# Britefury/cutmix-semisup-seg

Hardware: AMD Instinct MI355X
Metric: train images/sec (student+teacher step) (higher is better)
Workload: dtype bf16; 1 GPU; deeplab2-resnet101 cutmix mean-teacher step, 10x3x321x321, 21 classes (BASELINE configs[1]); per_gpu_batch=10, global_batch=10, classes=21, parallelism=dp1, fuse_batches=True, stream_overlap=True, deterministic_wgrad=False

## Files before the change

### cutmix-semisup-seg_amd/_lib.py

```python
import ctypes as C
import os

import torch

_HERE = os.path.dirname(os.path.abspath(__file__))
LIB_PATH = os.path.join(_HERE, 'csrc', 'libcutmixseg_hip.so')

if not os.path.exists(LIB_PATH):
    raise ImportError('libcutmixseg_hip.so not found at {} -- build it with '
                      '`python cutmix-semisup-seg_amd/build.py` (hipcc, gfx950); there is no CPU fallback'.format(LIB_PATH))

lib = C.CDLL(LIB_PATH)

F32, BF16 = 0, 1
(BN_REDUCE, BN_FINALIZE, BN_APPLY, BN_REDUCE_BWD, BN_BWD_APPLY, BN_COUNT, BN_STATS, BN_FINALIZE_TILES,
 BN_BWD_SUMS_TILES) = range(9)
LABEL_U8, LABEL_I64 = 0, 1
LOSS_IDS = {'var': 0, 'logits_var': 1, 'logits_smoothl1': 2, 'bce': 3, 'kld': 4}
MODE_MIX, MODE_CUT = 0, 1
OPT_CHUNK = 2048
AUG_PARAMS = 24

c_void_p, c_int, c_float, c_size_t = C.c_void_p, C.c_int, C.c_float, C.c_size_t

# ... 52 lines not shown
                ('stats_out', c_void_p), ('stats_rows_per_group', c_int), ('mask_gates_res', c_int),
                ('bstats_u', c_void_p), ('bstats_bits', c_void_p), ('bstats_mean', c_void_p), ('bstats_rstd', c_void_p)]


class WgradDesc(C.Structure):
    _fields_ = [('du', c_void_p), ('x', c_void_p), ('dw', c_void_p), ('scale', c_void_p),
                ('n', c_int), ('h', c_int), ('w_in', c_int), ('cin', c_int), ('ho', c_int), ('wo', c_int),
                ('cout', c_int), ('cout_real', c_int), ('ntaps', c_int), ('tap_dy', c_int * 18), ('tap_dx', c_int * 18),
                ('stride', c_int), ('ksplit', c_int), ('w', c_void_p), ('wdot', c_void_p), ('dbeta', c_void_p),
                ('dw_cout', c_int), ('workspace', c_void_p), ('workspace_bytes', C.c_longlong), ('wg_target', c_int)]


class BnOp(C.Structure):
    _fields_ = [('what', c_int), ('dtype', c_int), ('c', c_int), ('relu', c_int),
                ('x', c_void_p), ('res', c_void_p), ('y', c_void_p), ('dy', c_void_p), ('dx', c_void_p), ('dres', c_void_p),
                ('sums', c_void_p), ('gamma', c_void_p), ('beta', c_void_p), ('mean', c_void_p), ('rstd', c_void_p),
                ('scale', c_void_p), ('shift', c_void_p), ('running_mean', c_void_p), ('running_var', c_void_p),
                ('counter', c_void_p), ('clear_a', c_void_p), ('clear_b', c_void_p), ('ws', c_void_p), ('count', C.c_double), ('n_pixels', C.c_ulonglong), ('eps', c_float),
                ('momentum', c_float), ('groups', c_int), ('tile_rows', c_int), ('mask_bits', c_void_p)]


class AugmentDesc(C.Structure):
    _fields_ = [('src', c_void_p), ('src_labels', c_void_p), ('out0', c_void_p), ('out1', c_void_p),
                ('out_labels', c_void_p), ('out_mask', c_void_p), ('params', c_void_p),
                ('mean', c_float * 3), ('std_', c_float * 3),
                ('n', c_int), ('hs', c_int), ('ws', c_int), ('h', c_int), ('w', c_int), ('out_dtype', c_int)]


class StageEntry(C.Structure):
    _fields_ = [('img_off', C.c_longlong), ('lab_off', C.c_longlong), ('hs', c_int), ('ws', c_int)]


class StageDesc(C.Structure):
    _fields_ = [('pool_img', c_void_p), ('pool_labels', c_void_p), ('entries', c_void_p), ('index', c_void_p),
                ('out0', c_void_p), ('out1', c_void_p), ('out_labels', c_void_p), ('out_mask', c_void_p), ('params', c_void_p),
                ('mean', c_float * 3), ('std_', c_float * 3),
                ('n', c_int), ('n_entries', c_int), ('h', c_int), ('w', c_int), ('out_dtype', c_int)]


class PdPatch(C.Structure):
    _fields_ = [('img_off', C.c_longlong), ('hs', c_int), ('ws', c_int), ('cy', c_int), ('cx', c_int)]


TTA_MAX_VIEWS = 16


class TtaDesc(C.Structure):
    _fields_ = [('logits', c_void_p * TTA_MAX_VIEWS), ('h', c_int * TTA_MAX_VIEWS), ('w', c_int * TTA_MAX_VIEWS),
                ('flip', c_int * TTA_MAX_VIEWS),
                ('n', c_int), ('c', c_int), ('H', c_int), ('W', c_int), ('k', c_int), ('align_corners', c_int),
                ('labels', c_void_p), ('label_dtype', c_int), ('ignore_index', c_int), ('cm', c_void_p), ('pred_out', c_void_p)]


class ClassMixDesc(C.Structure):
    _fields_ = [('logits', c_void_p), ('valid', c_void_p), ('keys', c_void_p),
                ('n', c_int), ('c', c_int), ('h', c_int), ('w', c_int), ('H', c_int), ('W', c_int), ('align_corners', c_int),
                ('mask_out', c_void_p), ('pred_out', c_void_p), ('present_out', c_void_p), ('chosen_out', c_void_p),
                ('workspace', c_void_p), ('workspace_bytes', c_size_t)]


class CpsDesc(C.Structure):
    _fields_ = [('l0_a', c_void_p), ('l1_a', c_void_p), ('l0_b', c_void_p), ('l1_b', c_void_p),
                ('ranges', c_void_p), ('mask', c_void_p), ('um0', c_void_p), ('um1', c_void_p),
                ('n', c_int), ('c', c_int), ('h', c_int), ('w', c_int), ('H', c_int), ('W', c_int), ('align_corners', c_int),
                ('n_boxes', c_int), ('invert', c_int), ('conf_thresh', c_float),
                ('label_a', c_void_p), ('label_b', c_void_p), ('stats', c_void_p)]


class BoundaryDesc(C.Structure):
    _fields_ = [('truth', c_void_p), ('pred', c_void_p), ('widths', c_void_p),
                ('n', c_int), ('h', c_int), ('w', c_int), ('num_classes', c_int), ('ignore_index', c_int), ('k', c_int),
                ('bcm', c_void_p), ('tcm', c_void_p), ('dist_truth', c_void_p), ('dist_pred', c_void_p),
                ('workspace', c_void_p), ('workspace_bytes', c_size_t)]


class PackItem(C.Structure):
    _fields_ = [('src', c_void_p), ('dst', c_void_p), ('scale', c_void_p),
                ('ntaps', c_int), ('cout', c_int), ('cin', c_int), ('first_block', c_int)]


class WfinishItem(C.Structure):
    _fields_ = [('scratch', c_void_p), ('grad', c_void_p), ('w', c_void_p), ('scale', c_void_p), ('wdot', c_void_p),
                ('ntaps', c_int), ('cout', c_int), ('cin', c_int), ('first_block', c_int)]


_P = C.POINTER


def _proto(name, restype, argtypes):
    fn = getattr(lib, name)
    fn.restype = restype
    fn.argtypes = argtypes
    return fn


PROTOTYPES = {
    'cms_version': (c_int, []),
    'cms_last_error': (C.c_char_p, []),
    'cms_device_info': (c_int, [_P(c_int), C.c_char_p, c_size_t]),
    'cms_boxmask_rasterize': (c_int, [c_void_p, c_int, c_int, c_int, c_int, c_int, c_void_p, c_void_p]),
    'cms_cutmix_paste': (c_int, [c_void_p, c_void_p, c_void_p, c_int, c_void_p, c_int, c_int, c_int, c_int, c_int,
                                 c_int, c_void_p]),
    'cms_cutmix_paste_mask': (c_int, [c_void_p, c_void_p, c_void_p, c_int, c_void_p, c_int, c_int, c_int, c_int,
                                      c_void_p]),
    'cms_consistency_workspace_bytes': (c_size_t, [_P(ConsistencyDesc)]),
    'cms_consistency_fwd': (c_int, [_P(ConsistencyDesc), c_void_p, c_void_p, c_void_p]),
    'cms_consistency_finalize': (c_int, [c_void_p, c_void_p, c_float, c_int, c_float, c_float, c_void_p, c_void_p]),
    'cms_consistency_bwd': (c_int, [_P(ConsistencyDesc), c_void_p, c_void_p, c_void_p]),
    'cms_consistency_fused_supported': (c_int, [_P(ConsistencyDesc)]),
    'cms_consistency_fwd_bwd': (c_int, [_P(ConsistencyDesc), c_float, c_void_p, c_void_p, c_void_p, c_void_p]),
    'cms_scale_by_scalar': (c_int, [c_void_p, C.c_longlong, c_void_p, c_int, c_float, c_void_p]),
    'cms_ict_blend': (c_int, [c_void_p, c_void_p, c_void_p, c_int, c_void_p, c_int, C.c_longlong, c_void_p]),
    'cms_ict_workspace_bytes': (c_size_t, [_P(IctDesc)]),
    'cms_ict_fwd': (c_int, [_P(IctDesc), c_void_p, c_void_p, c_void_p]),
    'cms_ict_bwd': (c_int, [_P(IctDesc), c_void_p, c_void_p, c_void_p, c_void_p]),
    'cms_aug_workspace_bytes': (c_size_t, [_P(AugDesc)]),
    'cms_aug_fwd': (c_int, [_P(AugDesc), c_void_p, c_void_p, c_void_p]),
    'cms_aug_bwd': (c_int, [_P(AugDesc), c_void_p, c_void_p, c_void_p]),
    'cms_ce_workspace_bytes': (c_size_t, [_P(CeDesc)]),
    'cms_ce_fwd': (c_int, [_P(CeDesc), c_void_p, c_void_p, c_void_p]),
    'cms_ce_finalize': (c_int, [c_void_p, c_float, c_void_p, c_void_p]),
    'cms_ce_bwd': (c_int, [_P(CeDesc), c_void_p, c_void_p, c_void_p]),
    'cms_ce_fused_supported': (c_int, [_P(CeDesc)]),
    'cms_ce_fwd_bwd': (c_int, [_P(CeDesc), c_void_p, c_void_p, c_void_p, c_void_p]),
    'cms_upsample_bilinear_fwd': (c_int, [c_void_p, c_void_p, c_int, c_int, c_int, c_int, c_int, c_int, c_int,
                                          c_void_p]),
    'cms_upsample_bilinear_bwd': (c_int, [c_void_p, c_void_p, c_int, c_int, c_int, c_int, c_int, c_int, c_int,
                                          c_void_p]),
    'cms_ema_flat': (c_int, [c_void_p, c_void_p, c_size_t, c_float, c_float, c_void_p, c_void_p]),
    'cms_adam_ema_step': (c_int, [_P(OptimDesc), c_void_p]),
    'cms_sgd_ema_step': (c_int, [_P(OptimDesc), c_void_p]),
    'cms_increment_counter': (c_int, [c_void_p, c_void_p]),
    'cms_bn_fold': (c_int, [c_void_p, c_void_p, c_void_p, c_void_p, c_void_p, c_int, c_float, c_void_p, c_void_p, c_void_p]),
    'cms_argmax_confusion': (c_int, [c_void_p, c_void_p, c_int, c_int, c_int, c_int, c_int, c_int, c_int, c_int,
                                     c_int, c_void_p, c_void_p, c_void_p]),
    'cms_confusion': (c_int, [c_void_p, c_void_p, c_size_t, c_int, c_int, c_void_p, c_void_p]),
    'cms_fill_holes_workspace_bytes': (c_size_t, [c_int, c_int, c_int]),
    'cms_fill_holes': (c_int, [c_void_p, c_void_p, c_void_p, c_int, c_void_p, c_int, c_int, c_int, c_void_p, c_size_t,
                               c_void_p]),
    'cms_conv_igemm': (c_int, [_P(ConvDesc), c_void_p]),
    'cms_conv_igemm_route': (c_int, [_P(ConvDesc)]),
    'cms_conv_igemm_stats_tile_rows': (c_int, [_P(ConvDesc)]),
    'cms_frozen_bn_act_bwd': (c_int, [c_void_p, c_void_p, c_void_p, c_void_p, c_int, c_void_p, c_size_t, c_int, c_void_p]),
    'cms_conv_set_trace': (c_int, [c_void_p, c_int]),
    'cms_conv_set_wgrad8': (c_int, [c_int]),
    'cms_loss_set_deterministic': (c_int, [c_int]),
    'cms_conv_wgrad_uses_wgrad8': (c_int, [_P(WgradDesc)]),
    'cms_conv_wgrad': (c_int, [_P(WgradDesc), c_void_p]),
    'cms_conv_wgrad_workspace_bytes': (C.c_longlong, [_P(WgradDesc)]),
    'cms_conv_wgrad_group_kind': (c_int, [_P(WgradDesc)]),
    'cms_conv_wgrad_group_bytes': (C.c_longlong, [c_int]),
    'cms_conv_wgrad_group_pack': (c_int, [_P(WgradDesc), c_int, c_int, c_void_p, C.c_longlong, _P(c_int)]),
    'cms_conv_wgrad_group_run': (c_int, [c_void_p, c_int, c_int, c_int, c_void_p]),
    'cms_conv_pack_transpose': (c_int, [c_void_p, c_int, c_void_p, c_void_p, c_int, c_int, c_int, c_int, c_void_p]),
    'cms_conv_pack_transpose_batch': (c_int, [c_void_p, c_int, c_int, c_int, c_void_p]),
    'cms_conv_pack_transpose_batch64': (c_int, [c_void_p, c_int, c_int, c_void_p]),
    'cms_augment_batch': (c_int, [_P(AugmentDesc), c_void_p]),
    'cms_augment_luma': (c_int, [_P(AugmentDesc), c_void_p, c_void_p]),
    'cms_stage_batch': (c_int, [_P(StageDesc), c_void_p]),
    'cms_stage_luma': (c_int, [_P(StageDesc), c_void_p, c_void_p]),
    'cms_bn_workspace_bytes': (c_size_t, [c_size_t, c_int, c_int]),
    'cms_bn_run': (c_int, [_P(BnOp), c_void_p]),
    'cms_channel_copy': (c_int, [c_void_p, c_size_t, c_void_p, c_size_t, c_size_t, c_int, c_int, c_size_t, c_void_p]),
    'cms_add_n': (c_int, [c_void_p, c_int, c_void_p, c_size_t, c_int, c_void_p]),
    'cms_channel_sum': (c_int, [c_void_p, c_int, c_size_t, c_int, c_void_p, c_void_p]),
    'cms_wgrad_finish_pack': (c_int, [_P(WfinishItem), c_int]),
    'cms_wgrad_finish_run': (c_int, [c_void_p, c_int, c_int, c_void_p]),
    'cms_program_add_channel_sum': (c_int, [c_void_p, c_void_p, c_int, c_size_t, c_int, c_void_p, c_int, c_int]),
    'cms_program_add_wgrad_finish': (c_int, [c_void_p, c_void_p, c_int, c_int, c_int, c_int]),
    'cms_rows_reduce': (c_int, [c_void_p, c_size_t, c_int, c_size_t, c_int, c_int, c_void_p, c_float, c_void_p]),
    'cms_upsample_nhwc': (c_int, [c_void_p, c_void_p, c_size_t, c_int, c_int, c_int, c_int, c_int, c_int, c_int, c_int, c_int,
                                  c_void_p]),
    'cms_aspp_gather_fwd': (c_int, [c_void_p, c_void_p, c_void_p, _P(c_int), _P(c_int), c_int, c_int, c_int, c_int, c_int,
                                    c_int, c_void_p]),
    'cms_aspp_spread_bwd': (c_int, [c_void_p, c_void_p, c_int, _P(c_int), _P(c_int), c_int, c_int, c_int, c_int, c_int,
                                    c_int, c_void_p]),
    'cms_stem_pack_weights': (c_int, [c_void_p, c_int, c_void_p, c_void_p]),
    'cms_stem_out_hw': (c_int, [c_int, c_int, _P(c_int), _P(c_int), _P(c_int), _P(c_int)]),
    'cms_stem_fwd': (c_int, [c_void_p, c_int, c_void_p, c_int, c_void_p, c_void_p, c_void_p, c_int, c_int, c_int,
                             c_void_p]),
    'cms_maxpool3x3s2_fwd': (c_int, [c_void_p, c_void_p, c_void_p, c_int, c_int, c_int, c_int, c_int, c_int, c_void_p]),
    'cms_maxpool3x3s2_relu_bwd': (c_int, [c_void_p, c_void_p, c_void_p, c_void_p, c_int, c_int, c_int, c_int, c_int,
                                          c_int, c_void_p]),
    'cms_stem_wgrad': (c_int, [c_void_p, c_int, c_void_p, c_int, c_void_p, c_void_p, c_int, c_int, c_int, c_void_p]),
    'cms_stem_wgrad_workspace_bytes': (C.c_longlong, [c_int, c_int, c_int, c_int, c_int]),
    'cms_stem_wgrad_ws': (c_int, [c_void_p, c_int, c_void_p, c_int, c_void_p, c_void_p, c_int, c_int, c_int, c_void_p,
                          C.c_longlong, c_void_p]),
    'cms_stem_dgrad': (c_int, [c_void_p, c_int, c_void_p, c_void_p, c_void_p, c_int, c_int, c_int, c_void_p]),
    'cms_program_create': (c_int, [_P(c_void_p)]),
    'cms_program_destroy': (c_int, [c_void_p]),
    'cms_program_add_conv': (c_int, [c_void_p, _P(ConvDesc), c_int, c_int, c_int]),
    'cms_program_add_wgrad': (c_int, [c_void_p, _P(WgradDesc), c_int, c_int, c_int]),
    'cms_program_add_wgrad_group': (c_int, [c_void_p, c_void_p, c_int, c_int, c_int, c_int, c_int]),
    'cms_program_add_memset': (c_int, [c_void_p, c_void_p, c_size_t, c_int, c_int]),
# ... 66 lines not shown
```

### cutmix-semisup-seg_amd/backbone_hip.py

```python
import os
import torch

from . import ops
from .arena import ensure_arena


def executors_of(module):
    exs = getattr(module, '_hip_executors', None)
    if exs:
        return list(exs.values())
    ex = getattr(module, '_hip_executor', None)
    return [] if ex is None else [ex]


class _Conv(object):
    __slots__ = ('wkey', 'bn', 'taps', 'ntaps', 'neg_taps', 'stride', 'cin', 'cout', 'scale', 'bias', 'wT', 'ksize',
                 'pad', 'dil', 'wdot', 'dbeta', 'wT_raw')

    def __init__(self, wkey, bn, conv):
        self.wkey, self.bn = wkey, bn
        kh, kw = conv.kernel_size
        self.ksize, self.pad, self.dil = kh, conv.padding[0], conv.dilation[0]
        self.taps = ops.conv_taps(kh, kw, conv.dilation[0], conv.padding[0])
        self.neg_taps = [(-dy, -dx) for dy, dx in self.taps]
        self.stride = conv.stride[0]
        self.cin, self.cout = conv.in_channels, conv.out_channels
        self.scale = self.bias = self.wT = None
        self.wT_raw = None
        self.wdot = self.dbeta = None


class _Block(object):
    __slots__ = ('c1', 'c2', 'c3', 'cd')


class DeepLabHipExecutor(object):
    def __init__(self, net, dtype=torch.bfloat16):
        self._init_common(net, dtype)
        self.num_classes = net.num_classes
        self._add_blocks('', [getattr(net, 'layer{}'.format(li)) for li in range(1, 5)])
        self.stem_wkey, self.stem_bn, self.stem_ceil = 'conv1.weight', 'bn1', True
        self.stem_w147 = None
        self._stem_version = -1
        head = net.layer5.conv2d_list
        self.aspp_keys = ['layer5.conv2d_list.0', 'layer5.conv2d_list.1']
        self.aspp_taps = []
        for i in range(2):
            self.aspp_taps += ops.conv_taps(3, 3, head[i].dilation[0], head[i].padding[0])
        self.aspp_neg_taps = [(-dy, -dx) for dy, dx in self.aspp_taps]
        dev = self.arena.device
        C = self.num_classes
        if C > 32:
            raise NotImplementedError('ASPP head kernel is specialised for <= 32 classes')
        self.aspp_zc = (18 * C + 127) // 128 * 128
        self.aspp_wall = torch.zeros(1, self.aspp_zc, 2048, dtype=self.dtype, device=dev)
        self.aspp_wallT = torch.zeros(1, 2048, self.aspp_zc, dtype=self.dtype, device=dev)
        self._aspp_version = -1
        self.aspp_bias = torch.zeros(C, dtype=torch.float32, device=dev)

    def _init_common(self, net, dtype=torch.bfloat16):
        if dtype not in (torch.bfloat16, torch.float32):
            raise TypeError('executor dtype must be torch.bfloat16 or torch.float32')
        self.net = net
        self.dtype = dtype
        self.trainable = any(p.requires_grad for p in net.parameters())
        self.bn_trainable = any(p.requires_grad for m in net.modules() if 'BatchNorm' in type(m).__name__
                                for p in m.parameters())
        self.arena = ensure_arena(net, with_grad=self.trainable, with_bf16=(dtype == torch.bfloat16))
        self.blocks = []
        self._layer_first = []
        self._affine_ready = False
        self._bn_idx = None
        self._side = None
        self._pack_plan = None
        self._pack_plan_bn = None
        self._wT_raw_version = -1
        self._bn_modules = {}
        self._stem_param = None
        self._sentinel = None
        self._seen_shapes = {}
        self._wscratch_buf = None
        self._wfinish_pending = []
        self._wfinish_ok = {}
        self._pending_keep = None
        self.grad_hook = None
        self.data_grad_only = False
        self.overlap_wgrad = True
        self.wgrad_streams = 2 if os.environ.get('CMS_WGRAD8', '1') != '0' else 1
        self.defer_wgrad_join = False
        self._pending_join = None
        self._sides = []
        self.conv_tile = 0
        self.tile_rules = {}
        self._wT_version = -1
        self.version = 0
        self.use_programs = True
        self._programs = {}
        self._generation = 0
        self.issued = dict(flops=0.0, conv_launches=0, conv_bytes=0.0, head_launches=0, head_bytes=0.0, head_bytes_alg=0.0, floor_s=0.0)
        net.register_load_state_dict_post_hook(lambda module, incompatible: self.invalidate())

    def _add_blocks(self, prefix, layers):
        for li, layer in enumerate(layers):
            self._layer_first.append(len(self.blocks))
            for bi, blk in enumerate(layer):
                pre = '{}layer{}.{}'.format(prefix, li + 1, bi)
                b = _Block()
                b.c1 = _Conv(pre + '.conv1.weight', pre + '.bn1', blk.conv1)
                b.c2 = _Conv(pre + '.conv2.weight', pre + '.bn2', blk.conv2)
                b.c3 = _Conv(pre + '.conv3.weight', pre + '.bn3', blk.conv3)
                b.cd = None
                if blk.downsample is not None:
                    b.cd = _Conv(pre + '.downsample.0.weight', pre + '.downsample.1', blk.downsample[0])
                self.blocks.append(b)

    def invalidate(self):
        self.arena.refresh_bf16()
        self._affine_ready = False
        self.version += 1

    def weights_changed(self, bn_too=False):
        self.version += 1
        if bn_too or self.bn_trainable:
            self._affine_ready = False

    def block_grad_offsets(self):
        return [self.arena.by_key[b.c1.wkey].offset for b in self.blocks]

    def layer_first_blocks(self):
        return list(self._layer_first)

    def _all_convs(self):
        for b in self.blocks:
            for c in (b.c1, b.c2, b.c3, b.cd):
                if c is not None:
                    yield c

    def _build_affine_tables(self):
        a = self.arena
        idx = {k: [] for k in ('weight', 'bias', 'running_mean', 'running_var')}
        off = 0
        spans = []
        for c in self._all_convs():
            for k in idx:
                s = a.by_key[c.bn + '.' + k]
                idx[k].append(torch.arange(s.offset, s.offset + s.count, dtype=torch.int64))
            spans.append((c, off, off + c.cout))
            off += c.cout
        stem_span = None
        if getattr(self, 'stem_bn', None) is not None:
            for k in idx:
                s = a.by_key[self.stem_bn + '.' + k]
                idx[k].append(torch.arange(s.offset, s.offset + s.count, dtype=torch.int64))
            stem_span = (off, off + a.by_key[self.stem_bn + '.weight'].count)
            off = stem_span[1]
        dev = a.device
        self._bn_idx = {k: torch.cat(v).to(dev) for k, v in idx.items()}
        self._scale_all = torch.zeros(off, dtype=torch.float32, device=dev)
        self._bias_all = torch.zeros(off, dtype=torch.float32, device=dev)
        for c, lo, hi in spans:
            c.scale, c.bias = self._scale_all[lo:hi], self._bias_all[lo:hi]
        if stem_span is not None:
            self.stem_scale, self.stem_bias = self._scale_all[stem_span[0]:stem_span[1]], self._bias_all[stem_span[0]:stem_span[1]]
        if self.bn_trainable and self.trainable:
            self._wdot_all = torch.zeros(off, dtype=torch.float32, device=dev)
            self._dbeta_all = torch.zeros(off, dtype=torch.float32, device=dev)
            for c, lo, hi in spans:
                c.wdot, c.dbeta = self._wdot_all[lo:hi], self._dbeta_all[lo:hi]

    def _refresh_affine(self):
        if self._bn_idx is None:
            self._build_affine_tables()
# ... 134 lines not shown
                          sums=fsums[g * 2 * C:(g + 1) * 2 * C], gamma=a.view(c.bn + '.weight'), beta=a.view(c.bn + '.bias'),
                          mean=mean[sl], rstd=rstd[sl], scale=scale[sl], shift=shift[sl],
                          running_mean=a.view(c.bn + '.running_mean'), running_var=a.view(c.bn + '.running_var'),
                          counter=bn.num_batches_tracked)
        else:
            ops.bn_op('stats', c=C, dtype=self.dtype, n_pixels=npix, groups=G, eps=bn.eps, momentum=bn.momentum, x=u, ws=ws,
                      gamma=a.view(c.bn + '.weight'), beta=a.view(c.bn + '.bias'), mean=mean, rstd=rstd, scale=scale, shift=shift,
                      running_mean=a.view(c.bn + '.running_mean'), running_var=a.view(c.bn + '.running_var'),
                      counter=bn.num_batches_tracked)
        y = torch.empty_like(u)
        bits = torch.empty(npix * C // 8, dtype=torch.uint8, device=dev) if (relu and save) else None
        ops.bn_op('apply', c=C, dtype=self.dtype, n_pixels=npix, groups=G, relu=relu, x=u, res=res, y=y, scale=scale,
                  shift=shift, mask_bits=bits)
        return y, (u, bits, mean, rstd, bsums, ws, G)

    def _bstats(self, s3):
        if self.dtype != torch.bfloat16:
            return None
        u, bits, mean, rstd, _sums, _ws, G = s3
        return {'groups': G, 'u': u, 'mean': mean, 'rstd': rstd, 'bits': bits}

    def _bwd_unit_bn(self, dy, saved, c, want_res, dy_bits=None, tile_stats=None):
        u, bits, mean, rstd, sums, ws, G = saved
        C = c.cout
        npix = u.numel() // C
        if dy_bits is not None:
            assert bits is None
            bits = dy_bits
        if tile_stats is not None and tile_stats.get('tile_rows', 0) > 0:
            assert dy_bits is None
            ops.bn_op('sums_tiles', c=C, dtype=self.dtype, n_pixels=npix, groups=G, tile_rows=tile_stats['tile_rows'],
                      ws=tile_stats['tile_sums'], sums=sums)
        else:
            ops.bn_op('reduce_bwd', c=C, dtype=self.dtype, n_pixels=npix, groups=G, x=u, dy=dy, mean=mean, rstd=rstd, sums=sums,
                      ws=ws, mask_bits=bits)
        grp = self._dist_group()
        world = ops._world(grp)
        if world > 1:
            ops.host_call(lambda t=sums, g_=grp: ops._allreduce_sum(t, g_))
        du = torch.empty_like(u)
        dres = torch.empty_like(u) if want_res else None
        ops.bn_op('bwd_apply', c=C, dtype=self.dtype, n_pixels=npix, groups=G, count=(npix // G) * world, x=u, dy=dy, dx=du, dres=dres,
                  mask_bits=bits, mean=mean, rstd=rstd, gamma=self.arena.view(c.bn + '.weight'), sums=sums)
        return du, dres

    def _fwd_block_bn(self, st, bi):
        b, cur = self.blocks[bi], st['cur']
        save, G = st['saved'] is not None, st.get('groups', 1)
        a1, s1 = self._fwd_unit_bn(cur, b.c1, True, save=save, groups=G)
        a2, s2 = self._fwd_unit_bn(a1, b.c2, True, save=save, groups=G)
        sd = None
        if b.cd is None:
            res = cur
        else:
            res, sd = self._fwd_unit_bn(cur, b.cd, False, save=save, groups=G)
        out, s3 = self._fwd_unit_bn(a2, b.c3, True, res=res, save=save, groups=G)
        st['cur'] = out
        if st['saved'] is not None:
            st['saved'].append((cur, a1, a2, s1, s2, s3, sd))

    def _refresh_backward_weights_bn(self):
        if self._pack_plan_bn is None:
            triples = []
            for c in self._all_convs():
                w = self._w(c)
                c.wT_raw = torch.empty((w.shape[0], w.shape[2], w.shape[1]), dtype=self.dtype, device=w.device)
                triples.append((w, c.wT_raw, None))
            triples.append((self.aspp_wall, self.aspp_wallT, None))
            self._pack_plan_bn = ops.PackTransposePlan(triples)
        self._pack_plan_bn.run()

    def _dgrad_raw(self, du, c, res=None, in_hw=None, res_bits=None, bstats=None):
        n, ho, wo, _ = du.shape
        if c.stride == 1:
            return ops.conv_igemm(du, c.wT_raw, c.neg_taps, res=res, mode=1, tile=self._tile(c.cin), mask_bits=res_bits,
                                  mask_gates_res=res_bits is not None, stats=bstats)
        assert res_bits is None and bstats is None
        return ops.conv_igemm(du, c.wT_raw, c.neg_taps, res=res, mode=1, out_hw=(ho, wo), out_stride=c.stride,
                              out_full_hw=in_hw, tile=self._tile(c.cin))

    def _wgrad_raw(self, du, x, c):
        ops.conv_wgrad(du, x, c.taps, self.arena.packed(c.wkey, self.arena.grad), stride=c.stride, wg_target=self._wg_target())

    def _backward_chain_bn(self, saved, dlg, want_w, sides, hook, box=None):
        x4 = saved[-1]
        main = torch.cuda.current_stream()
        d = ops.aspp_spread_bwd(dlg, self.aspp_taps, self.aspp_zc, self.dtype)
        dwall = None
        if want_w:
            dwall = torch.empty((1, self.aspp_zc, 2048), dtype=torch.float32, device=d.device)
            ops.memset_zero(dwall)
            ops.conv_wgrad(d, x4, [(0, 0)], dwall)
            if box is not None:
                box['dwall'] = dwall
        pend = self._bstats(saved[len(self.blocks) - 1][5])
        dOut = ops.conv_igemm(d, self.aspp_wallT, [(0, 0)], mode=1, stats=pend)
        keep = []
        closes = set(self.bucket_starts())
        for bi in range(len(self.blocks) - 1, -1, -1):
            b = self.blocks[bi]
            xin, a1, a2, s1, s2, s3, sd = saved[bi]
            in_hw = (xin.shape[1], xin.shape[2])
            bits3 = s3[1] if (b.cd is not None or (b.c1.stride == 1 and self.dtype == torch.bfloat16)) else None
            du3, dres = self._bwd_unit_bn(dOut, s3, b.c3, bits3 is None, tile_stats=pend)
            da2 = self._dgrad_raw(du3, b.c3)
            du2, _ = self._bwd_unit_bn(da2, s2, b.c2, False)
            da1 = self._dgrad_raw(du2, b.c2)
            du1, _ = self._bwd_unit_bn(da1, s1, b.c1, False)
            dud = None
            if b.cd is not None:
                dud, _ = self._bwd_unit_bn(dres if bits3 is None else dOut, sd, b.cd, False, dy_bits=bits3)
            if want_w:
                self._issue_wgrads(self._block_jobs(b, du3, du2, dud, du1, xin, a1, a2), sides, main, keep, bi in closes,
                                   wgrad=self._wgrad_raw)
                with torch.cuda.stream(sides[0] if sides else main):
                    hook(bi)
            pend = self._bstats(saved[bi - 1][5]) if (bi > 0 and b.c1.stride == 1) else None
            if b.cd is None and bits3 is not None:
                dOut = self._dgrad_raw(du1, b.c1, res=dOut, in_hw=in_hw, res_bits=bits3, bstats=pend)
            else:
                dx = dres if b.cd is None else self._dgrad_raw(dud, b.cd, in_hw=in_hw)
                dOut = self._dgrad_raw(du1, b.c1, res=dx, in_hw=in_hw, bstats=pend)
        if not self.defer_wgrad_join:
            for sd_ in sides:
                ops.stream_wait(main, sd_)
        self._retire_keep(keep)
        return dOut, dwall

    def _stem_prepare(self):
        if not self._affine_ready:
            self._refresh_affine()
        if self._stem_version != self.version:
            self.stem_w147 = ops.stem_pack_weights(self.arena.packed(self.stem_wkey, self._wbuf()), out=self.stem_w147)
            self._stem_version = self.version

    def stem(self, x):
        if self._stem_param is None:
            self._stem_param = dict(self.net.named_parameters())[self.stem_wkey]
        save = (torch.is_grad_enabled() and (self.trainable or x.requires_grad)) if self.use_programs else None
        return _StemFn.apply(x.contiguous(), self._stem_param, self, save)

    def _stem_destination(self, shape, save):
        key = ('fwd', tuple(int(v) for v in shape), bool(save), self._tile_key(), self._bn_key())
        prog = self._programs.get(key)
        return None if prog is None else prog.x_in

    def _prepare_forward(self):
        if not self._affine_ready and not self.batch_statistics():
            self._refresh_affine()
        self._refresh_aspp_fwd()

    def _bn_key(self):
        return self.bn_groups() if self.batch_statistics() else 0

    def _tile_key(self):
        return (self.conv_tile, tuple(sorted(self.tile_rules.items())))

    MAX_PROGRAMS = 8

    def _program_lookup(self, key):
        prog = self._programs.get(key)
        if prog is not None:
            self._programs[key] = self._programs.pop(key)
            return prog
        if len(self._programs) >= self.MAX_PROGRAMS:
            torch.cuda.synchronize()
            self._programs.pop(next(iter(self._programs)))
        return None

    def _eager_this_time(self, kind, shape, save):
# ... 70 lines not shown
                self.fwd_block(st, bi)
            return self.fwd_end(st)
        prog = self.forward_program(x.shape, save)
        self._prepare_forward()
        if x.data_ptr() != prog.x_in.data_ptr():
            prog.x_in.copy_(x)
        prog.run([torch.cuda.current_stream()])
        self._stamp(prog)
        return prog.logits.clone(), ((prog, prog.generation) if save else None)

    def _wgrad(self, du, x, c):
        if c.wdot is not None and self.dtype == torch.float32:
            g = torch.zeros_like(self._w(c))
            ops.conv_wgrad(du, x, c.taps, g, stride=c.stride)
            self.arena.packed(c.wkey, self.arena.grad).add_(g * c.scale.view(1, -1, 1))
            c.wdot.add_((g * self._w(c)).sum(dim=(0, 2)))
            c.dbeta.add_(du.sum(dim=(0, 1, 2)))
        elif c.wdot is not None and self._wfinish_takes(du, x, c):
            ops.conv_wgrad(du, x, c.taps, self.arena.packed(c.wkey, self._wscratch()), stride=c.stride, scale=None,
                           wg_target=self._wg_target())
            ops.channel_sum(du, c.dbeta)
            if all(c is not p for p in self._wfinish_pending):
                self._wfinish_pending.append(c)
        elif c.wdot is not None:
            ops.conv_wgrad(du, x, c.taps, self.arena.packed(c.wkey, self.arena.grad), stride=c.stride, scale=c.scale,
                           w_bf16=self._w(c), wdot=c.wdot, dbeta=c.dbeta)
        else:
            ops.conv_wgrad(du, x, c.taps, self.arena.packed(c.wkey, self.arena.grad), stride=c.stride, scale=c.scale,
                           wg_target=self._wg_target())

    def _wscratch(self):
        if self._wscratch_buf is None:
            self._wscratch_buf = torch.zeros_like(self.arena.grad)
        return self._wscratch_buf

    def _wfinish_takes(self, du, x, c):
        if self.dtype != torch.bfloat16 or ops.deterministic_wgrad():
            return False
        key = (c.wkey, tuple(du.shape), tuple(x.shape))
        hit = self._wfinish_ok.get(key)
        if hit is None:
            hit = self._wfinish_ok[key] = bool(ops.conv_wgrad(du, x, c.taps, self.arena.packed(c.wkey, self._wscratch()),
                                                              stride=c.stride, scale=None, wg_target=self._wg_target(),
                                                              query_kernel=True))
        return hit

    def _wfinish_flush(self):
        pend = self._wfinish_pending
        if not pend:
            return
        a = self.arena
        ops.wgrad_finish([(a.packed(c.wkey, self._wscratch()), a.packed(c.wkey, a.grad), self._w(c), c.scale, c.wdot) for c in pend])
        del pend[:]

    def _wg_target(self):
        if not self.overlap_wgrad:
            return 0
        return 56 if self.wgrad_streams >= 2 else 112

    def _dgrad(self, du, c, res=None, mask=None, in_hw=None):
        n, ho, wo, _ = du.shape
        mb = getattr(mask, '_cms_relu_bits', None) if mask is not None else None
        if mb is not None:
            mask = None
        if c.stride == 1:
            return ops.conv_igemm(du, c.wT, c.neg_taps, res=res, mode=1, mask_src=mask, tile=self._tile(c.cin), mask_bits=mb)
        return ops.conv_igemm(du, c.wT, c.neg_taps, res=res, mode=1, mask_src=mask, out_hw=(ho, wo),
                              out_stride=c.stride, out_full_hw=in_hw, tile=self._tile(c.cin), mask_bits=mb)

    def _grad_sentinel(self):
        if self._sentinel is None:
            self._sentinel = dict(self.net.named_parameters())[self.blocks[-1].c3.wkey]
        return self._sentinel

    def _want_w(self):
        data_only = self.data_grad_only or getattr(self.net, '_data_grad_only', False)
        return self.trainable and not data_only and self.arena.grad is not None

    def _refresh_for_backward(self):
        if self._wT_version != self.version or self.blocks[0].c1.wT is None:
            self._refresh_backward_weights()
            self._wT_version = self.version

    def _head_bias_grads(self, dlogits, want_w, side=None):
        if want_w:
            if side is not None:
                side.wait_stream(torch.cuda.current_stream())
                dlogits.record_stream(side)
            with torch.cuda.stream(side if side is not None else torch.cuda.current_stream()):
                db = dlogits.sum(dim=(0, 2, 3))
                for k in self.aspp_keys:
                    self.arena.view(k + '.bias', self.arena.grad).add_(db)

    def _head_weight_grads(self, dwall, side=None):
        C = self.num_classes
        a = self.arena
        with torch.cuda.stream(side if side is not None else torch.cuda.current_stream()):
            for i, k in enumerate(self.aspp_keys):
                a.packed(k + '.weight', a.grad).add_(dwall[0, 9 * C * i:9 * C * (i + 1)].view(9, C, 2048))

    def _finish_head(self, dwall, side):
        self._head_weight_grads(dwall, side)
        if side is not None and not self.defer_wgrad_join:
            torch.cuda.current_stream().wait_stream(side)

    def bucket_starts(self):
        l2, l3, l4 = self._layer_first[1], self._layer_first[2], self._layer_first[3]
        return sorted(set([0, l2, l3, (l3 + l4 + 1) // 2, l4]))

    def _backward_chain(self, saved, dlg, want_w, sides, hook, box=None):
        x4 = saved[-1]
        main = torch.cuda.current_stream()
        d = ops.aspp_spread_bwd(dlg, self.aspp_taps, self.aspp_zc, self.dtype)
        dwall = None
        keep = []
        if want_w:
            dwall = torch.empty((1, self.aspp_zc, 2048), dtype=torch.float32, device=d.device)
            hs = sides[0] if sides else None
            if hs is not None:
                ops.stream_wait(hs, main)
                keep.append((d, dwall))
            with torch.cuda.stream(hs if hs is not None else main):
                ops.memset_zero(dwall)
                ops.conv_wgrad(d, x4, [(0, 0)], dwall)
            if box is not None:
                box['dwall'] = dwall
        x4b = getattr(x4, '_cms_relu_bits', None)
        dC = ops.conv_igemm(d, self.aspp_wallT, [(0, 0)], mode=1, mask_src=None if x4b is not None else x4, mask_bits=x4b)
        capture = getattr(self, 'debug_capture', None)
        closes = set(self.bucket_starts())
        for bi in range(len(self.blocks) - 1, -1, -1):
            if capture is not None:
                capture[bi] = dC
            b = self.blocks[bi]
            xin, a1, a2 = saved[bi]
            in_hw = (xin.shape[1], xin.shape[2])
            dU2 = self._dgrad(dC, b.c3, mask=a2)
            dU1 = self._dgrad(dU2, b.c2, mask=a1)
            if want_w:
                self._issue_wgrads(self._block_jobs(b, dC, dU2, dC, dU1, xin, a1, a2), sides, main, keep, bi in closes)
                with torch.cuda.stream(sides[0] if sides else main):
                    hook(bi)
            dres = dC if b.cd is None else self._dgrad(dC, b.cd, in_hw=in_hw)
            dC = self._dgrad(dU1, b.c1, res=dres, mask=None if bi == 0 else xin, in_hw=in_hw)
        if not self.defer_wgrad_join:
            for sd in sides:
                ops.stream_wait(main, sd)
        self._retire_keep(keep)
        return dC, dwall

    def backward(self, token, dlogits):
        bn = (token[0].bn if self.use_programs and isinstance(token, tuple) and isinstance(token[0], ops.Program)
              else len(token[0]) == 7)
        chain = self._backward_chain_bn if bn else self._backward_chain
        if bn:
            if self._wT_raw_version != self.version or self.blocks[0].c1.wT_raw is None:
                self._refresh_aspp_fwd()
                self._refresh_backward_weights_bn()
                self._wT_raw_version = self.version
        else:
            self._refresh_for_backward()
        want_w = self._want_w()
        if want_w and self._grad_sentinel().grad is None:
            self.arena.ensure_grads_attached()
        n, _, h, w = dlogits.shape
        main = torch.cuda.current_stream()
        sides = self._side_streams(self.wgrad_streams) if (self.overlap_wgrad and want_w) else []
        hside = sides[0] if (sides and not bn) else None
        if not self.use_programs:
            if self.defer_wgrad_join and sides:
                self._pending_join = list(sides)
            self._head_bias_grads(dlogits, want_w, hside)
            box = {}

            def hook(bi):
                if 'done' not in box and box.get('dwall') is not None:
                    self._head_weight_grads(box['dwall'])
                    box['done'] = True
                if self.grad_hook is not None:
                    self.grad_hook(bi)
            dx, dwall = chain(token, dlogits, want_w, sides, hook, box)
            if dwall is not None and 'done' not in box:
                self._finish_head(dwall, hside)
            return dx
        fprog, gen = token
        if fprog.generation != gen:
            raise RuntimeError('the activations of this forward pass were overwritten by a later forward pass of the '
                               'same shape through the same executor (programs keep ONE set of buffers per shape): '
                               'run backward before the next forward, or set executor.use_programs = False')
        key = (want_w, len(sides), bool(self.defer_wgrad_join))
        if self.defer_wgrad_join and sides:
            self._pending_join = list(sides)
        prog = fprog.bwd.get(key)
        if prog is None:
            prog = ops.Program()
            dlg = torch.empty(tuple(dlogits.shape), dtype=torch.float32, device=dlogits.device)
            streams = [main] + sides
            with ops.recording(prog, streams):
                dx, dwall = chain(fprog.saved, dlg, want_w, sides, prog.mark)
            prog.dlg, prog.dx, prog.dwall = dlg, dx, dwall
            fprog.bwd[key] = prog
        prog.dlg.copy_(dlogits)
        self._head_bias_grads(dlogits, want_w, hside)
        streams = [main] + sides
        if self.grad_hook is None or not want_w:
            prog.run(streams)
            if prog.dwall is not None:
                self._finish_head(prog.dwall, hside)
        else:
            first = 0
            hook_stream = sides[0] if sides else main
            head_done = False
            wanted = getattr(self.grad_hook, 'blocks', None)
            for idx, bi in prog.marks:
                if wanted is not None and bi not in wanted:
                    continue
                prog.run(streams, first, idx)
                first = idx
                with torch.cuda.stream(hook_stream):
                    if not head_done and prog.dwall is not None:
                        self._head_weight_grads(prog.dwall)
                        head_done = True
                    self.grad_hook(bi)
            prog.run(streams, first, -1)
            if prog.dwall is not None and not head_done:
                self._finish_head(prog.dwall, hside)
        self._account(prog)
        return prog.dx.clone()

    def _retire_keep(self, keep):
        if keep and self.defer_wgrad_join and ops._REC is None:
            self._pending_keep = (self._pending_keep or []) + [keep]

    def join_wgrad(self):
        sides, self._pending_join = self._pending_join, None
        if sides:
            main = torch.cuda.current_stream()
            for sd in sides:
                main.wait_stream(sd)
        self._pending_keep = None

    @staticmethod
    def _block_jobs(b, d3, d2, dd, d1, xin, a1, a2):
        return [(d3, a2, b.c3), (d2, a1, b.c2)] + ([(dd, xin, b.cd)] if b.cd is not None else []) + [(d1, xin, b.c1)]

    def _issue_wgrads(self, jobs, sides, main, keep, closes, first=0, wgrad=None):
        wgrad = wgrad or self._wgrad
        for sd in sides:
            ops.stream_wait(sd, main)
        if sides:
            keep.append(jobs)
        for ji, (du_, x_, c_) in enumerate(jobs, first):
            with torch.cuda.stream(sides[ji % len(sides)] if sides else main):
                wgrad(du_, x_, c_)
        if closes:
            for sd in sides[1:]:
                ops.stream_wait(sides[0], sd)
        return first + len(jobs)

    def _side_streams(self, k):
        k = max(1, min(int(k), 3))
        while len(self._sides) < k:
            self._sides.append(ops.pooled_stream(self.arena.device, 'wgrad{}'.format(len(self._sides))))
        return self._sides[:k]

    def _side_stream(self):
        if self._side is None:
            self._side = ops.pooled_stream(self.arena.device, 'side')
        return self._side


class DeepLabV3PlusBackboneExecutor(DeepLabHipExecutor):

    def __init__(self, wrapper, dtype=torch.bfloat16):
        self._init_common(wrapper, dtype)
        self.use_programs = not (dtype == torch.float32 and self.bn_trainable and self.trainable)
        self.stem_wkey, self.stem_bn, self.stem_ceil = 'deeplab.backbone.conv1.weight', 'deeplab.backbone.bn1', False
        self.stem_w147 = None
        self._stem_version = -1
        bb = wrapper.deeplab.backbone
        self._add_blocks('deeplab.backbone.', [bb['layer{}'.format(li)] for li in range(1, 5)])
        self.tap_low = self._layer_first[1] - 1
        self._phase_w = {}

    def _prepare_forward(self):
        if not self._affine_ready:
            self._refresh_affine()

    def _taps_pass(self, x, save):
        st = self.fwd_begin(x, save)
        low = None
        for bi in range(len(self.blocks)):
            if ops._REC is not None:
                ops._REC[0].group = bi
            self.fwd_block(st, bi)
            if bi == self.tap_low:
                low = st['cur']
        if save:
            st['saved'].append(st['cur'])
        return low, st['cur'], st['saved']

    def taps_program(self, shape, save):
        key = ('taps', tuple(int(v) for v in shape), bool(save), self._tile_key())
        prog = self._program_lookup(key)
        if prog is None:
            self._prepare_forward()
            prog = ops.Program()
            x_in = torch.empty(tuple(shape), dtype=self.dtype, device=self.arena.device)
            with ops.recording(prog, [torch.cuda.current_stream()]):
                low, out, saved = self._taps_pass(x_in, save)
            prog.x_in, prog.low, prog.out, prog.saved = x_in, low, out, saved
            prog.bwd = {}
            prog.generation = -1
            self._programs[key] = prog
        return prog

    def forward_taps(self, x, save=False):
        if not self.use_programs or self._eager_this_time('taps', x.shape, save):
            low, out, saved = self._taps_pass(x, save)
            return (low, out, saved) if save else (low, out)
        prog = self.taps_program(x.shape, save)
        self._prepare_forward()
        prog.x_in.copy_(x)
        prog.run([torch.cuda.current_stream()])
        self._stamp(prog)
        if save:
            return prog.low.detach(), prog.out.detach(), (prog, prog.generation)
        return prog.low.detach(), prog.out.detach()

    def _refresh_backward_weights(self):
        super()._refresh_backward_weights()
        for (cid, py, px), (c, idx, buf) in self._phase_w.items():
            torch.index_select(c.wT, 0, idx, out=buf)

    def _dgrad_strided(self, du, c, mask, in_hw):
        if not (c.stride == 2 and c.ksize == 3 and c.pad == 1 and c.dil == 1):
            raise NotImplementedError('phase decomposition is written for the 3x3 / stride 2 / pad 1 convolution')
        n = du.shape[0]
        H, W = int(in_hw[0]), int(in_hw[1])
        dx = torch.empty((n, H, W, c.cin), dtype=du.dtype, device=du.device)
        sel = {0: [1], 1: [0, 2]}
        for py in (0, 1):
            for px in (0, 1):
                ha, wb = (H - py + 1) // 2, (W - px + 1) // 2
                if ha <= 0 or wb <= 0:
                    continue
                ks = [(ky, kx) for ky in sel[py] for kx in sel[px]]
                ent = self._phase_w.get((id(c), py, px))
                if ent is None:
                    idx = _index_tensor(tuple(ky * 3 + kx for ky, kx in ks), du.device)
                    ent = (c, idx, c.wT[idx].contiguous())
                    self._phase_w[(id(c), py, px)] = ent
                taps = [((py + 1 - ky) // 2, (px + 1 - kx) // 2) for ky, kx in ks]
                ops.conv_igemm(du, ent[2], taps, mode=1, mask_src=mask, out=dx, out_hw=(ha, wb), out_stride=2,
                               out_full_hw=(H, W), out_pixel_offset=py * W + px)
# ... 350 lines not shown
        return p

    @staticmethod
    def backward(ctx, dp):
        x, s, idx = ctx.saved_tensors
        ex = ctx.executor
        ds = ops.maxpool3x3s2_relu_backward(dp.to(s.dtype), idx, s, ceil_mode=ex.stem_ceil)
        if ctx.w_grad and ex._want_w():
            if ex.bn_trainable:
                a = ex.arena
                g = torch.zeros((49, 64, 3), dtype=torch.float32, device=ds.device)
                ops.stem_wgrad(x, ds, g, None)
                a.packed(ex.stem_wkey, a.grad).add_(g * ex.stem_scale.view(1, -1, 1))
                wdot = (g * a.packed(ex.stem_wkey, ex._wbuf()).float()).sum(dim=(0, 2))
                dbeta = ds.float().sum(dim=(0, 1, 2))
                mean, var = a.view(ex.stem_bn + '.running_mean'), a.view(ex.stem_bn + '.running_var')
                a.view(ex.stem_bn + '.weight', a.grad).add_((wdot - mean * dbeta) * torch.rsqrt(var + 1e-5))
                a.view(ex.stem_bn + '.bias', a.grad).add_(dbeta)
            else:
                ops.stem_wgrad(x, ds, ex.arena.packed(ex.stem_wkey, ex.arena.grad), ex.stem_scale)
        dx = None
        if ctx.needs_input_grad[0]:
            dx = ops.stem_dgrad(ds, ex.stem_w147, ex.stem_scale, ctx.x_shape).to(ctx.x_dtype)
        return dx, None, None, None


class _BodyFn(torch.autograd.Function):

    @staticmethod
    def forward(ctx, x_nhwc, executor, need_grad):
        logits, token = executor.forward(x_nhwc, save=need_grad)
        ctx.executor = executor
        ctx.saved_acts = token
        return logits

    @staticmethod
    def backward(ctx, dlogits):
        dx = ctx.executor.backward(ctx.saved_acts, dlogits.contiguous().float())
        ctx.saved_acts = None
        return dx, None, None


class _BodyPairFn(torch.autograd.Function):

    @staticmethod
    def forward(ctx, x_stu, x_tea, ex_stu, ex_tea, side, need_grad):
        if ex_stu.use_programs and ex_tea.use_programs:
            main = torch.cuda.current_stream()
            ps = ex_stu.forward_program(x_stu.shape, need_grad)
            ex_stu._prepare_forward()
            if x_stu.data_ptr() != ps.x_in.data_ptr():
                ps.x_in.copy_(x_stu)
            with torch.cuda.stream(side):
                pt = ex_tea.forward_program(x_tea.shape, False)
                ex_tea._prepare_forward()
                if x_tea.data_ptr() != pt.x_in.data_ptr():
                    pt.x_in.copy_(x_tea)
            if ps.host_ops or pt.host_ops:
                with torch.cuda.stream(side):
                    pt.run([side])
                ps.run([main])
            else:
                ops.run_pair(ps, [main], pt, [side])
            ex_stu._stamp(ps)
            ex_tea._stamp(pt)
            logits_s = ps.logits.clone()
            with torch.cuda.stream(side):
                logits_t = pt.logits.clone()
            saved = (ps, ps.generation) if need_grad else None
        else:
            st_s = ex_stu.fwd_begin(x_stu, need_grad)
            with torch.cuda.stream(side):
                st_t = ex_tea.fwd_begin(x_tea, False)
            for bi in range(len(ex_stu.blocks)):
                ex_stu.fwd_block(st_s, bi)
                with torch.cuda.stream(side):
                    ex_tea.fwd_block(st_t, bi)
            logits_s, saved = ex_stu.fwd_end(st_s)
            with torch.cuda.stream(side):
                logits_t, _ = ex_tea.fwd_end(st_t)
        ctx.executor = ex_stu
        ctx.saved_acts = saved
        ctx.mark_non_differentiable(logits_t)
        return logits_s, logits_t

    @staticmethod
    def backward(ctx, dlogits, _unused):
        dx = ctx.executor.backward(ctx.saved_acts, dlogits.contiguous().float())
        ctx.saved_acts = None
        return dx, None, None, None, None, None


def run_body_pair(ex_stu, x_stu, ex_tea, x_tea, side):
    if len(ex_stu.blocks) != len(ex_tea.blocks):
        raise ValueError('student and teacher bodies differ')
    need_grad = torch.is_grad_enabled() and ex_stu.trainable
    if need_grad and not x_stu.requires_grad:
        x_stu = x_stu.detach().requires_grad_(True)
    return _BodyPairFn.apply(x_stu, x_tea, ex_stu, ex_tea, side, need_grad)


def run_body(executor, x_nhwc):
    need_grad = torch.is_grad_enabled() and (executor.trainable or x_nhwc.requires_grad)
    if need_grad and not x_nhwc.requires_grad:
        x_nhwc = x_nhwc.detach().requires_grad_(True)
    return _BodyFn.apply(x_nhwc, executor, need_grad)
```

### cutmix-semisup-seg_amd/csrc/aspp.hip

```cpp
#include "common.hpp"

namespace cms {

struct AsppTaps {
    int n_taps;
    short dy[CMS_CONV_MAX_TAPS], dx[CMS_CONV_MAX_TAPS];
};

__device__ __forceinline__ void taps_to_lds(const AsppTaps& tp, short* sdy, short* sdx) {
#pragma unroll
    for (int i = 0; i < CMS_CONV_MAX_TAPS; ++i)
        if ((int)threadIdx.x == i) {
            sdy[i] = tp.dy[i];
            sdx[i] = tp.dx[i];
        }
    __syncthreads();
}

__global__ __launch_bounds__(256) void aspp_gather_fwd_kernel(const float* __restrict__ z, const float* __restrict__ bias,
                                                              float* __restrict__ logits, AsppTaps tp, int N, int C, int ZC,
                                                              int H, int W) {
    __shared__ short sdy[CMS_CONV_MAX_TAPS], sdx[CMS_CONV_MAX_TAPS];
    taps_to_lds(tp, sdy, sdx);
    const int n_taps = tp.n_taps;
    const size_t total = (size_t)N * C * H * W;
    for (size_t i = (size_t)blockIdx.x * blockDim.x + threadIdx.x; i < total; i += (size_t)gridDim.x * blockDim.x) {
        const unsigned ii = (unsigned)i;
        const int x = (int)(ii % (unsigned)W);
        unsigned t = ii / (unsigned)W;
        const int y = (int)(t % (unsigned)H); t /= (unsigned)H;
        const int c = (int)(t % (unsigned)C);
        const int n = (int)(t / (unsigned)C);
        float acc = bias ? bias[c] : 0.0f;
        const float* zn = z + ((size_t)n * ZC + c) * H * W;
        const size_t tap_stride = (size_t)C * H * W;
        for (int k = 0; k < n_taps; ++k) {
            const int yy = y + sdy[k], xx = x + sdx[k];
            if ((unsigned)yy < (unsigned)H && (unsigned)xx < (unsigned)W) acc += zn[(size_t)k * tap_stride + (size_t)yy * W + xx];
        }
        logits[i] = acc;
    }
}

template <class T>
__global__ __launch_bounds__(256) void aspp_spread_bwd_kernel(const float* __restrict__ dl, T* __restrict__ d, AsppTaps tp,
                                                              int N, int C, int ZC, int H, int W) {
    __shared__ short sdy[CMS_CONV_MAX_TAPS], sdx[CMS_CONV_MAX_TAPS];
    taps_to_lds(tp, sdy, sdx);
    const int n_taps = tp.n_taps;
    const unsigned zc8 = (unsigned)ZC / 8u;
    const size_t total = (size_t)N * H * W * zc8;
    const size_t plane = (size_t)H * W;
    for (size_t i = (size_t)blockIdx.x * blockDim.x + threadIdx.x; i < total; i += (size_t)gridDim.x * blockDim.x) {
        const unsigned ii = (unsigned)i;
        const unsigned ch = ii % zc8;
        unsigned t = ii / zc8;
        const int x = (int)(t % (unsigned)W); t /= (unsigned)W;
        const int y = (int)(t % (unsigned)H);
        const int n = (int)(t / (unsigned)H);
        const float* dn = dl + (size_t)n * C * plane;
        float v[8];
        int k = (int)((ch * 8u) / (unsigned)C), c = (int)(ch * 8u) - k * C;
#pragma unroll
        for (int e = 0; e < 8; ++e) {
            float val = 0.0f;
            if (k < n_taps) {
                const int yy = y - sdy[k], xx = x - sdx[k];
                if ((unsigned)yy < (unsigned)H && (unsigned)xx < (unsigned)W) val = dn[(size_t)c * plane + (size_t)yy * W + xx];
            }
            v[e] = val;
            if (++c == C) { c = 0; ++k; }
        }
        if constexpr (sizeof(T) == 4) {
            float4* o = reinterpret_cast<float4*>(d + i * 8);
            o[0] = float4{v[0], v[1], v[2], v[3]};
            o[1] = float4{v[4], v[5], v[6], v[7]};
        } else {
            uint4 o;
            o.x = (uint32_t)f32_to_bf16(v[0]) | ((uint32_t)f32_to_bf16(v[1]) << 16);
            o.y = (uint32_t)f32_to_bf16(v[2]) | ((uint32_t)f32_to_bf16(v[3]) << 16);
            o.z = (uint32_t)f32_to_bf16(v[4]) | ((uint32_t)f32_to_bf16(v[5]) << 16);
            o.w = (uint32_t)f32_to_bf16(v[6]) | ((uint32_t)f32_to_bf16(v[7]) << 16);
            *reinterpret_cast<uint4*>(d + i * 8) = o;
        }
    }
}

}

using namespace cms;

static int fill_taps(AsppTaps& tp, const int* dy, const int* dx, int n_taps) {
    CMS_REQUIRE(dy && dx && n_taps > 0 && n_taps <= CMS_CONV_MAX_TAPS, "aspp: 1..%d taps", CMS_CONV_MAX_TAPS);
    tp.n_taps = n_taps;
    for (int i = 0; i < CMS_CONV_MAX_TAPS; ++i) {
        tp.dy[i] = (short)(i < n_taps ? dy[i] : 0);
        tp.dx[i] = (short)(i < n_taps ? dx[i] : 0);
    }
    return CMS_OK;
}

extern "C" int cms_aspp_gather_fwd(const float* z, const float* bias, float* logits, const int* tap_dy, const int* tap_dx,
                                   int n_taps, int n, int c, int zc, int h, int w, void* stream) {
    CMS_REQUIRE(z && logits, "aspp_gather_fwd: NULL pointer");
    CMS_REQUIRE(n > 0 && c > 0 && h > 0 && w > 0 && zc >= n_taps * c, "aspp_gather_fwd: bad geometry (zc >= taps * classes)");
    AsppTaps tp;
    const int rc = fill_taps(tp, tap_dy, tap_dx, n_taps);
    if (rc) return rc;
    const size_t total = (size_t)n * c * h * w;
    CMS_REQUIRE(total < (1ull << 32), "aspp_gather_fwd: more than 2^32 logits");
    hipLaunchKernelGGL(aspp_gather_fwd_kernel, dim3(grid_for(total, 256, 256 * 16)), dim3(256), 0, (hipStream_t)stream, z, bias,
                       logits, tp, n, c, zc, h, w);
    return launch_status("cms_aspp_gather_fwd");
}

extern "C" int cms_aspp_spread_bwd(const float* dlogits, void* d_nhwc, int d_dtype, const int* tap_dy, const int* tap_dx,
                                   int n_taps, int n, int c, int zc, int h, int w, void* stream) {
    CMS_REQUIRE(dlogits && d_nhwc, "aspp_spread_bwd: NULL pointer");
    CMS_REQUIRE(d_dtype == CMS_F32 || d_dtype == CMS_BF16, "aspp_spread_bwd: bad dtype");
    CMS_REQUIRE(n > 0 && c > 0 && h > 0 && w > 0 && zc >= n_taps * c, "aspp_spread_bwd: bad geometry (zc >= taps * classes)");
    AsppTaps tp;
    const int rc = fill_taps(tp, tap_dy, tap_dx, n_taps);
    if (rc) return rc;
    CMS_REQUIRE(zc % 8 == 0, "aspp_spread_bwd: the stacked tap x class axis (%d) must be a multiple of 8", zc);
    const size_t total = (size_t)n * h * w * (zc / 8);
    CMS_REQUIRE(total < (1ull << 32), "aspp_spread_bwd: more than 2^32 chunks");
    hipStream_t s = (hipStream_t)stream;
    if (d_dtype == CMS_F32)
        hipLaunchKernelGGL(aspp_spread_bwd_kernel<float>, dim3(grid_for(total, 256, 256 * 16)), dim3(256), 0, s, dlogits,
                           (float*)d_nhwc, tp, n, c, zc, h, w);
    else
        hipLaunchKernelGGL(aspp_spread_bwd_kernel<uint16_t>, dim3(grid_for(total, 256, 256 * 16)), dim3(256), 0, s, dlogits,
                           (uint16_t*)d_nhwc, tp, n, c, zc, h, w);
    return launch_status("cms_aspp_spread_bwd");
}
```

### cutmix-semisup-seg_amd/csrc/common.hpp

```cpp
#pragma once
#include <hip/hip_runtime.h>
#include <stdarg.h>
#include <stdio.h>
#include "../../include/cutmixseg.h"
#include "pixel_math.hpp"

namespace cms {

void set_error(const char* fmt, ...);

inline int launch_status(const char* what) {
    hipError_t e = hipGetLastError();
    if (e != hipSuccess) {
        set_error("%s: %s", what, hipGetErrorString(e));
        return CMS_ELAUNCH;
    }
    return CMS_OK;
}

#define CMS_REQUIRE(cond, ...)         \
    do {                               \
        if (!(cond)) {                 \
            cms::set_error(__VA_ARGS__); \
            return CMS_EINVAL;         \
        }                              \
    } while (0)

constexpr int kWave = 64;

__device__ __forceinline__ float wave_sum(float v) {
#pragma unroll
    for (int off = 32; off > 0; off >>= 1) v += __shfl_down(v, off, 64);
    return v;
}

template <int K>
__device__ __forceinline__ void block_sum(float (&v)[K], float* smem ) {
    const int lane = threadIdx.x & 63, wid = threadIdx.x >> 6, nw = blockDim.x >> 6;
#pragma unroll
    for (int k = 0; k < K; ++k) v[k] = wave_sum(v[k]);
    if (lane == 0) {
#pragma unroll
        for (int k = 0; k < K; ++k) smem[k * 16 + wid] = v[k];
    }
    __syncthreads();
    if (threadIdx.x == 0) {
#pragma unroll
        for (int k = 0; k < K; ++k) {
            float s = 0.0f;
            for (int i = 0; i < nw; ++i) s += smem[k * 16 + i];
            v[k] = s;
        }
    }
}

bool conv8_supported(const cms_conv_desc* d);
int conv8_launch(const cms_conv_desc* d, hipStream_t s, void* trace, int trace_wgs);
bool wgrad8_supported(const cms_wgrad_desc* d);
int wgrad8_plan(const cms_wgrad_desc* d, int* kt_per_slice);
int wgrad8_launch(const cms_wgrad_desc* d, hipStream_t s, void* trace, int trace_wgs);
void wgrad_reduce_launch(const float* slab, float* dw, int ksplit, size_t slice_elems, int ntaps, int cout, int cin, int cout_real,
                         int dw_cout, hipStream_t s);

inline int grid_for(size_t work_items, int block, int max_blocks = 256 * 8) {
    size_t b = (work_items + block - 1) / block;
    if (b > (size_t)max_blocks) b = max_blocks;
    if (b < 1) b = 1;
    return (int)b;
}

__device__ __forceinline__ float bf16_to_f32(uint16_t v) { return __uint_as_float(((uint32_t)v) << 16); }
__device__ __forceinline__ uint16_t f32_to_bf16(float f) {
    uint32_t u = __float_as_uint(f);
    if ((u & 0x7fffffffu) > 0x7f800000u) return (uint16_t)((u >> 16) | 0x40);
    u += 0x7fffu + ((u >> 16) & 1u);
    return (uint16_t)(u >> 16);
}

template <class T>
__device__ __forceinline__ void put_as(void* base, size_t idx, float v) {
    if constexpr (sizeof(T) == 4) reinterpret_cast<float*>(base)[idx] = v;
    else reinterpret_cast<uint16_t*>(base)[idx] = f32_to_bf16(v);
}

}
```

### cutmix-semisup-seg_amd/csrc/loss_tiles.hpp

```cpp
#pragma once
#include <algorithm>
#include <cstdlib>
#include "common.hpp"

namespace cms {

template <bool IDENT>
struct Gather {
    const float* base;
    size_t plane;
    int w_in;
    Tap ty, tx;
    size_t off;
    __device__ __forceinline__ float operator()(int c) const {
        if (IDENT) return base[c * plane + off];
        return bilin_gather(base + c * plane, w_in, ty, tx);
    }
};

template <int CT>
struct RegVec {
    float v[CT > 0 ? CT : 1];
    __device__ __forceinline__ float operator()(int c) const { return v[c]; }
};
// ... 96 lines not shown
        r.off = (size_t)y * g.w + x;
    } else {
        r.ty = bilin_tap(y, g.sy, g.h, g.align != 0);
        r.tx = bilin_tap(x, g.sx, g.w, g.align != 0);
    }
    return r;
}

__device__ __forceinline__ Gather<false> gather_staged(const float* base, const Patch& p, const Tap& ty, const Tap& tx) {
    Gather<false> r;
    r.base = base;
    r.plane = (size_t)p.n_rows * p.n_cols;
    r.w_in = p.n_cols;
    r.ty = ty;
    r.tx = tx;
    return r;
}

struct ScatterTile {
    int n, x0, y0, tw, th;
};

__device__ __forceinline__ ScatterTile fwd_tile(const Geo& g) {
    const int tiles_x = (g.W + TILE_W - 1) / TILE_W, tiles_y = (g.H + FWD_TILE_H - 1) / FWD_TILE_H;
    int b = blockIdx.x;
    const int tx_i = b % tiles_x;
    b /= tiles_x;
    const int ty_i = b % tiles_y;
    ScatterTile t;
    t.n = b / tiles_y;
    t.x0 = tx_i * TILE_W;
    t.y0 = ty_i * FWD_TILE_H;
    t.tw = min(TILE_W, g.W - t.x0);
    t.th = min(FWD_TILE_H, g.H - t.y0);
    return t;
}

template <bool UNROLL, class Stage, class Pixel>
__device__ __forceinline__ void fwd_tile_walk(const Geo& g, float* smem, Stage stage, Pixel pixel) {
    const ScatterTile t = fwd_tile(g);
    const Patch p = tile_patch(g, t.x0, t.y0, t.tw, t.th);
    stage(t.n, p, smem);
    __syncthreads();
    const int col = threadIdx.x & (TILE_W - 1);
    auto rows = [&](int rr) {
        const int row = (threadIdx.x >> 6) + rr * 4;
        if (col < t.tw && row < t.th) {
            const int y = t.y0 + row, x = t.x0 + col;
            Tap ty = bilin_tap(y, g.sy, g.h, g.align != 0), tx = bilin_tap(x, g.sx, g.w, g.align != 0);
            rebase(ty, tx, p);
            pixel(t.n, y, x, ty, tx, p);
        }
    };
    if (UNROLL) {
#pragma unroll
        for (int rr = 0; rr < FWD_TILE_H / 4; ++rr) rows(rr);
    } else {
#pragma unroll 1
        for (int rr = 0; rr < FWD_TILE_H / 4; ++rr) rows(rr);
    }
}

template <class F>
__device__ __forceinline__ void pixel_walk(const Geo& g, F f) {
    const size_t P = (size_t)g.n * g.H * g.W;
    for (size_t idx = (size_t)blockIdx.x * blockDim.x + threadIdx.x; idx < P; idx += (size_t)gridDim.x * blockDim.x) {
        const int x = (int)(idx % g.W);
        const size_t t = idx / g.W;
        const int y = (int)(t % g.H);
        const int n = (int)(t / g.H);
        f(idx, n, y, x);
    }
}

template <int K>
__device__ __forceinline__ void store_partials(float (&acc)[K], float* red, float* __restrict__ partials) {
    block_sum<K>(acc, red);
    if (threadIdx.x == 0) {
#pragma unroll
        for (int k = 0; k < K; ++k) partials[blockIdx.x * K + k] = acc[k];
    }
}

template <int K>
__global__ __launch_bounds__(256) void reduce_partials_kernel(const float* __restrict__ partials, int nblocks,
                                                              double* __restrict__ out, double extra, int extra_slot) {
    __shared__ double sm[K][256];
    double loc[K];
#pragma unroll
    for (int k = 0; k < K; ++k) loc[k] = 0.0;
    for (int i = threadIdx.x; i < nblocks; i += 256) {
#pragma unroll
        for (int k = 0; k < K; ++k) loc[k] += (double)partials[i * K + k];
    }
#pragma unroll
    for (int k = 0; k < K; ++k) sm[k][threadIdx.x] = loc[k];
    __syncthreads();
    for (int s = 128; s > 0; s >>= 1) {
        if ((int)threadIdx.x < s) {
#pragma unroll
            for (int k = 0; k < K; ++k) sm[k][threadIdx.x] += sm[k][threadIdx.x + s];
        }
        __syncthreads();
    }
    if (threadIdx.x == 0) {
#pragma unroll
        for (int k = 0; k < K; ++k) out[k] = sm[k][0];
        if (extra_slot >= 0) out[extra_slot] = extra;
    }
}

#ifndef CMS_LOSS_TILE_H
#define CMS_LOSS_TILE_H 4
#endif
constexpr int TILE_H = CMS_LOSS_TILE_H;
constexpr int G_LD = TILE_W + 1;

struct TileTables {
    int xi0[TILE_W], xi1[TILE_W];
    float xw1[TILE_W];
    int yi0[TILE_H], yi1[TILE_H];
    float yw1[TILE_H];
    int xbeg[TILE_W + 2], xend[TILE_W + 2];
};

inline int tile_max_rows(float sy) { return tile_max_rows_of(sy, TILE_H); }

inline size_t tile_lds_bytes(int C, float sy, float sx, int n_patches) {
    size_t g = (size_t)TILE_H * C * G_LD;
    size_t r = (size_t)TILE_H * C * tile_max_cols(sx);
    return (g + r + (size_t)n_patches * patch_floats(C, sy, sx, TILE_H)) * sizeof(float);
}

__device__ __forceinline__ ScatterTile scatter_tile(const Geo& g) {
    const int tiles_x = (g.W + TILE_W - 1) / TILE_W;
    const int tiles_y = (g.H + TILE_H - 1) / TILE_H;
    const int ctx = (tiles_x - g.col_x + g.col_kx - 1) / g.col_kx;
    const int cty = (tiles_y - g.col_y + g.col_ky - 1) / g.col_ky;
    int b = blockIdx.x;
    const int tx_i = g.col_x + (b % ctx) * g.col_kx;
    b /= ctx;
    const int ty_i = g.col_y + (b % cty) * g.col_ky;
    ScatterTile t;
    t.n = b / cty;
    t.x0 = tx_i * TILE_W;
    t.y0 = ty_i * TILE_H;
    t.tw = min(TILE_W, g.W - t.x0);
    t.th = min(TILE_H, g.H - t.y0);
    return t;
}

template <class Stage, class PixelGrad>
__device__ __forceinline__ void tiled_scatter(const Geo& g, Stage stage, PixelGrad pixel_grad, float* __restrict__ grad_lo,
                                              float* smem) {
    __shared__ TileTables tb;
    const ScatterTile tile = scatter_tile(g);
    const int n = tile.n, x0 = tile.x0, y0 = tile.y0, tw = tile.tw, th = tile.th;
    const int C = g.c;
    const int tid = threadIdx.x;

    if (tid < TILE_W) {
        Tap t = bilin_tap(min(x0 + tid, g.W - 1), g.sx, g.w, g.align != 0);
        tb.xi0[tid] = t.i0;
        tb.xi1[tid] = t.i1;
        tb.xw1[tid] = t.w1;
    } else if (tid < TILE_W + TILE_H) {
        const int r = tid - TILE_W;
        Tap t = bilin_tap(min(y0 + r, g.H - 1), g.sy, g.h, g.align != 0);
        tb.yi0[r] = t.i0;
        tb.yi1[r] = t.i1;
        tb.yw1[r] = t.w1;
    }
    __syncthreads();
    const int r_x_lo = tb.xi0[0], r_n_cols = tb.xi1[tw - 1] - r_x_lo + 1;
    const int r_y_lo = tb.yi0[0], r_n_rows = tb.yi1[th - 1] - r_y_lo + 1;
    if (tid < r_n_cols) {
        tb.xbeg[tid] = tw;
        tb.xend[tid] = 0;
    }
    __syncthreads();
    if (tid < tw) {
        const int j0 = tb.xi0[tid] - r_x_lo, j1 = tb.xi1[tid] - r_x_lo;
        atomicMin(&tb.xbeg[j0], tid);
        atomicMax(&tb.xend[j0], tid + 1);
        atomicMin(&tb.xbeg[j1], tid);
        atomicMax(&tb.xend[j1], tid + 1);
    }

    float* G = smem;
    float* R = smem + (size_t)TILE_H * C * G_LD;
    Patch patch;
    patch.x_lo = r_x_lo; patch.n_cols = r_n_cols; patch.y_lo = r_y_lo; patch.n_rows = r_n_rows;
// ... 194 lines not shown
```

### cutmix-semisup-seg_amd/csrc/losses.hip

```cpp
#include "loss_tiles.hpp"

namespace cms {

struct ConsArgs {
    cms_consistency_desc d;
    Geo g;
    float tau, inv_root_c;
};

struct ConsPixel {
    bool m;
    float um;
    const float* tea;
    int which;
};

__device__ __forceinline__ ConsPixel cons_pixel_inputs(const ConsArgs& a, int n, int y, int x) {
    const cms_consistency_desc& d = a.d;
    const size_t pix = ((size_t)n * d.H + y) * d.W + x;
    ConsPixel p;
    if (d.mask) {
        p.m = d.mask[pix] >= 0.5f;
    } else {
        p.m = box_mask_bit(d.ranges + (size_t)n * d.n_boxes * 4, d.n_boxes, y, x, d.invert != 0);
    }
    const size_t sample = (size_t)n * d.c * d.h * d.w;
    if (d.mode == MODE_MIX) {
        p.tea = (p.m ? d.l_tea1 : d.l_tea0) + sample;
        p.which = p.m ? 1 : 0;
        const float* um = p.m ? d.um1 : d.um0;
        p.um = um ? um[pix] : 1.0f;
    } else {
        p.tea = d.l_tea0 + sample;
        p.which = 0;
        p.um = p.m ? (d.um0 ? d.um0[pix] : 1.0f) : 0.0f;
    }
    return p;
}

__device__ __forceinline__ void cons_stage(const ConsArgs& a, int n, const Patch& p, float* P, int pstride) {
    const Geo& g = a.g;
    const size_t plane = (size_t)g.h * g.w, sample = (size_t)n * g.c * plane;
    stage_patch(P, a.d.l_stu + sample, g.c, plane, g.w, p);
    stage_patch(P + pstride, a.d.l_tea0 + sample, g.c, plane, g.w, p);
    if (a.d.mode == MODE_MIX) stage_patch(P + 2 * pstride, a.d.l_tea1 + sample, g.c, plane, g.w, p);
}

template <int CT, bool IDENT>
__device__ __forceinline__ void cons_fwd_pixel(const ConsArgs& a, const ConsPixel& px, const Gather<IDENT>& gs, const Gather<IDENT>& gt,
                                               float (&acc)[3]) {
    const Geo& g = a.g;
    PixelFwd r;
    if (CT > 0) {
        RegVec<CT> rs, rt;
        fill<CT, IDENT>(rs, gs);
        fill<CT, IDENT>(rt, gt);
        r = consistency_pixel_fwd<CT>(rs, rt, g.c, a.d.loss_fn, a.inv_root_c);
    } else {
        r = consistency_pixel_fwd<0>(gs, gt, g.c, a.d.loss_fn, a.inv_root_c);
    }
    const float lm = r.loss * px.um;
    const float cf = (a.tau > 0.0f && r.conf >= a.tau) ? 1.0f : 0.0f;
    acc[0] += lm;
    acc[1] += lm * cf;
    acc[2] += cf;
}

template <int CT>
__global__ __launch_bounds__(256) void cons_fwd_tiled_kernel(ConsArgs a, float* __restrict__ partials, int patch_stride) {
    extern __shared__ __attribute__((aligned(16))) float smem[];
    float acc[3] = {0.0f, 0.0f, 0.0f};
    fwd_tile_walk<false>(
        a.g, smem, [&](int n, const Patch& p, float* P) { cons_stage(a, n, p, P, patch_stride); },
        [&](int n, int y, int x, const Tap& ty, const Tap& tx, const Patch& p) {
            const ConsPixel px = cons_pixel_inputs(a, n, y, x);
            const Gather<false> gs = gather_staged(smem, p, ty, tx);
            const Gather<false> gt = gather_staged(smem + (px.which ? 2 : 1) * patch_stride, p, ty, tx);
            cons_fwd_pixel<CT, false>(a, px, gs, gt, acc);
        });
    __shared__ float red[3 * 16];
    store_partials<3>(acc, red, partials);
}

template <int CT, bool IDENT>
__global__ __launch_bounds__(256) void cons_fwd_kernel(ConsArgs a, float* __restrict__ partials) {
    const Geo& g = a.g;
    float acc[3] = {0.0f, 0.0f, 0.0f};
    pixel_walk(g, [&](size_t, int n, int y, int x) {
        const ConsPixel px = cons_pixel_inputs(a, n, y, x);
        const Gather<IDENT> gs = gather_at<IDENT>(a.d.l_stu + (size_t)n * g.c * ((size_t)g.h * g.w), g, y, x);
        Gather<IDENT> gt = gs;
        gt.base = px.tea;
        cons_fwd_pixel<CT, IDENT>(a, px, gs, gt, acc);
    });
    __shared__ float red[3 * 16];
    store_partials<3>(acc, red, partials);
}

__global__ void cons_finalize_kernel(const double* __restrict__ sl, const double* __restrict__ sg, float tau,
                                     int per_pixel, float ramp, float weight, float* __restrict__ out) {
    if (threadIdx.x != 0 || blockIdx.x != 0) return;
    const double Pl = sl[3];
    double closs, gs, rate;
    if (tau > 0.0f) {
        rate = sg[2] / sg[3];
        if (per_pixel) {
            closs = sl[1] / Pl;
            gs = 1.0 / Pl;
        } else {
            closs = rate * (sl[0] / Pl);
            gs = rate / Pl;
        }
    } else {
        rate = NAN;
        closs = sl[0] / Pl;
        gs = 1.0 / Pl;
    }
    closs *= (double)ramp;
    out[0] = (float)closs;
    out[1] = (float)rate;
    out[2] = (float)(gs * (double)ramp * (double)weight);
    out[3] = (float)(closs * (double)weight);
}

template <int CT>
__global__ __launch_bounds__(256) void cons_bwd_ident_kernel(ConsArgs a, const float* __restrict__ scalars,
                                                             float* __restrict__ grad) {
    const Geo& g = a.g;
    const size_t plane = (size_t)g.h * g.w;
    const float gscale = scalars[2];
    pixel_walk(g, [&](size_t, int n, int y, int x) {
        const ConsPixel px = cons_pixel_inputs(a, n, y, x);
        const Gather<true> gs = gather_at<true>(a.d.l_stu + (size_t)n * g.c * plane, g, y, x);
        Gather<true> gt = gs;
        gt.base = px.tea;
        float* gp = grad + (size_t)n * g.c * plane + gs.off;
        const float base_f = gscale * px.um;
        const bool pp = a.tau > 0.0f && a.d.conf_per_pixel;
        if (CT > 0) {
            RegVec<CT> rs, rt;
            fill<CT, true>(rs, gs);
            fill<CT, true>(rt, gt);
            float gv[CT > 0 ? CT : 1];
            const float conf = consistency_pixel_bwd<CT>(rs, rt, g.c, a.d.loss_fn, a.inv_root_c,
                                                        [&](int k, float v) { gv[k] = v; });
            const float f = (pp && !(conf >= a.tau)) ? 0.0f : base_f;
#pragma unroll
            for (int k = 0; k < CT; ++k) gp[k * plane] += f * gv[k];
        } else {
            float ms, zs, mt, zt;
            softmax_stats<0>(gt, g.c, mt, zt);
            (void)ms; (void)zs;
            const float conf = 1.0f / zt;
            const float f = (pp && !(conf >= a.tau)) ? 0.0f : base_f;
            consistency_pixel_bwd<0>(gs, gt, g.c, a.d.loss_fn, a.inv_root_c,
                                     [&](int k, float v) { gp[k * plane] += f * v; });
        }
    });
}

template <int CT>
__global__ __launch_bounds__(256) void cons_bwd_tiled_kernel(ConsArgs a, const float* __restrict__ scalars,
                                                             float* __restrict__ grad, int patch_stride) {
    extern __shared__ __attribute__((aligned(16))) float smem[];
    const Geo& g = a.g;
    const float gscale = scalars[2];
    const bool pp = a.tau > 0.0f && a.d.conf_per_pixel;
    const int pstride = patch_stride;
    auto stage = [&](int n, const Patch& p, float* P) { cons_stage(a, n, p, P, pstride); };
    auto pixel_grad = [&](int n, int y, int x, const Tap& ty, const Tap& tx, const Patch& p, const float* P, auto emit) -> bool {
        const ConsPixel px = cons_pixel_inputs(a, n, y, x);
        const float base_f = gscale * px.um;
        const Gather<false> gs = gather_staged(P, p, ty, tx);
        const Gather<false> gt = gather_staged(P + (px.which ? 2 * pstride : pstride), p, ty, tx);
        if (CT > 0) {
            RegVec<CT> rs, rt;
            fill<CT, false>(rs, gs);
            fill<CT, false>(rt, gt);
            float gv[CT > 0 ? CT : 1];
            const float conf = consistency_pixel_bwd<CT>(rs, rt, g.c, a.d.loss_fn, a.inv_root_c,
                                                        [&](int k, float v) { gv[k] = v; });
            const float f = (pp && !(conf >= a.tau)) ? 0.0f : base_f;
#pragma unroll
            for (int k = 0; k < CT; ++k) emit(k, f * gv[k]);
        } else {
            float mt, zt;
            softmax_stats<0>(gt, g.c, mt, zt);
            const float conf = 1.0f / zt;
            const float f = (pp && !(conf >= a.tau)) ? 0.0f : base_f;
            consistency_pixel_bwd<0>(gs, gt, g.c, a.d.loss_fn, a.inv_root_c, [&](int k, float v) { emit(k, f * v); });
        }
        return true;
    };
    tiled_scatter(g, stage, pixel_grad, grad, smem);
}

template <int CT, int LF>
__global__ __launch_bounds__(256, (LF >= 0 && CT > 0) ? 4 : 1) void cons_fused_tiled_kernel(ConsArgs a, float grad_unit, float* __restrict__ grad,
                                                               int patch_stride, float* __restrict__ partials) {
    extern __shared__ __attribute__((aligned(16))) float smem[];
    const Geo& g = a.g;
    const bool pp = a.tau > 0.0f && a.d.conf_per_pixel;
    const int pstride = patch_stride;
    float acc[3] = {0.0f, 0.0f, 0.0f};
    auto stage = [&](int n, const Patch& p, float* P) { cons_stage(a, n, p, P, pstride); };
    auto pixel_grad = [&](int n, int y, int x, const Tap& ty, const Tap& tx, const Patch& p, const float* P, auto emit) -> bool {
        const ConsPixel px = cons_pixel_inputs(a, n, y, x);
        const float base_f = grad_unit * px.um;
        const Gather<false> gs = gather_staged(P, p, ty, tx);
        const Gather<false> gt = gather_staged(P + (px.which ? 2 * pstride : pstride), p, ty, tx);
        PixelFwd r;
        if (CT > 0) {
            RegVec<CT> rs, rt;
            fill<CT, false>(rs, gs);
            fill<CT, false>(rt, gt);
            r = consistency_pixel_fwd_bwd<(CT > 0 ? CT : 1), LF>(
                rs, rt, a.d.loss_fn, a.inv_root_c,
                [&](float conf) -> float { return (pp && !(conf >= a.tau)) ? 0.0f : base_f; },
                [&](int k, float v) { emit(k, v); });
        } else {
            r = consistency_pixel_fwd<0>(gs, gt, g.c, a.d.loss_fn, a.inv_root_c);
            const float f = (pp && !(r.conf >= a.tau)) ? 0.0f : base_f;
            consistency_pixel_bwd<0>(gs, gt, g.c, a.d.loss_fn, a.inv_root_c, [&](int k, float v) { emit(k, f * v); });
        }
        const float lm = r.loss * px.um;
        const float cf = (a.tau > 0.0f && r.conf >= a.tau) ? 1.0f : 0.0f;
        acc[0] += lm;
        acc[1] += lm * cf;
        acc[2] += cf;
        return true;
    };
    tiled_scatter(g, stage, pixel_grad, grad, smem);
    __shared__ float red[3 * 16];
    store_partials<3>(acc, red, partials);
}

__global__ __launch_bounds__(256) void scale_by_scalar_kernel(float* __restrict__ x, size_t n, const float* __restrict__ scalars,
                                                              int idx, float factor) {
    const float f = scalars[idx] * factor;
    for (size_t i = (size_t)blockIdx.x * blockDim.x + threadIdx.x; i < n; i += (size_t)gridDim.x * blockDim.x) x[i] *= f;
}

struct CeArgs {
    cms_ce_desc d;
    Geo g;
};

__device__ __forceinline__ int load_label(const CeArgs& a, size_t pix) {
    if (a.d.label_dtype == CMS_LABEL_U8) return (int)((const uint8_t*)a.d.labels)[pix];
    const int64_t v = ((const int64_t*)a.d.labels)[pix];
    return (v < 0 || v > 0x7fffffff) ? -1 : (int)v;
}

__device__ __forceinline__ bool ce_ignored(const CeArgs& a, int label) {
    return label == a.d.ignore_index || label < 0 || label >= a.g.c;
}

__device__ __forceinline__ void ce_stage(const CeArgs& a, int n, const Patch& p, float* P) {
    const Geo& g = a.g;
    const size_t plane = (size_t)g.h * g.w;
    stage_patch(P, a.d.logits + (size_t)n * g.c * plane, g.c, plane, g.w, p);
}

template <int CT, bool IDENT>
__device__ __forceinline__ void ce_fwd_pixel(const CeArgs& a, const Gather<IDENT>& gl, int label, float (&acc)[2]) {
    float v;
    if (CT > 0) {
        RegVec<CT> r;
        fill<CT, IDENT>(r, gl);
        float mx, z;
        softmax_stats<CT>(r, a.g.c, mx, z);
        v = -((gl(label) - mx) - logf(z));
    } else {
        v = ce_pixel_fwd<0>(gl, a.g.c, label);
    }
    acc[0] += v;
    acc[1] += 1.0f;
}

template <int CT, bool IDENT>
__global__ __launch_bounds__(256) void ce_fwd_kernel(CeArgs a, float* __restrict__ partials) {
    const Geo& g = a.g;
    float acc[2] = {0.0f, 0.0f};
    pixel_walk(g, [&](size_t pix, int n, int y, int x) {
        const int label = load_label(a, pix);
        if (ce_ignored(a, label)) return;
        ce_fwd_pixel<CT, IDENT>(a, gather_at<IDENT>(a.d.logits + (size_t)n * g.c * ((size_t)g.h * g.w), g, y, x), label, acc);
    });
    __shared__ float red[2 * 16];
    store_partials<2>(acc, red, partials);
}

template <int CT>
__global__ __launch_bounds__(256) void ce_fwd_tiled_kernel(CeArgs a, float* __restrict__ partials) {
    extern __shared__ __attribute__((aligned(16))) float smem[];
    const Geo& g = a.g;
    float acc[2] = {0.0f, 0.0f};
    fwd_tile_walk<true>(
        g, smem, [&](int n, const Patch& p, float* P) { ce_stage(a, n, p, P); },
        [&](int n, int y, int x, const Tap& ty, const Tap& tx, const Patch& p) {
            const int label = load_label(a, ((size_t)n * g.H + y) * g.W + x);
            if (ce_ignored(a, label)) return;
            ce_fwd_pixel<CT, false>(a, gather_staged(smem, p, ty, tx), label, acc);
        });
    __shared__ float red[2 * 16];
    store_partials<2>(acc, red, partials);
}

__global__ void ce_finalize_kernel(const double* __restrict__ stats, float weight, float* __restrict__ out) {
    if (threadIdx.x != 0 || blockIdx.x != 0) return;
    out[0] = (float)(stats[0] / stats[1]);
    out[1] = stats[1] > 0.0 ? (float)((double)weight / stats[1]) : 0.0f;
}

template <int CT>
__global__ __launch_bounds__(256) void ce_bwd_ident_kernel(CeArgs a, const float* __restrict__ scalars,
                                                           float* __restrict__ grad) {
    const Geo& g = a.g;
    const size_t plane = (size_t)g.h * g.w;
    const float gscale = scalars[1];
    pixel_walk(g, [&](size_t pix, int n, int y, int x) {
        const int label = load_label(a, pix);
        if (ce_ignored(a, label)) return;
        const Gather<true> gl = gather_at<true>(a.d.logits + (size_t)n * g.c * plane, g, y, x);
        float* gp = grad + (size_t)n * g.c * plane + gl.off;
        if (CT > 0) {
            RegVec<CT> r;
            fill<CT, true>(r, gl);
            ce_pixel_bwd<CT>(r, g.c, label, [&](int k, float v) { gp[k * plane] += gscale * v; });
        } else {
            ce_pixel_bwd<0>(gl, g.c, label, [&](int k, float v) { gp[k * plane] += gscale * v; });
        }
    });
}

template <int CT>
__global__ __launch_bounds__(256) void ce_bwd_tiled_kernel(CeArgs a, const float* __restrict__ scalars,
                                                           float* __restrict__ grad) {
    extern __shared__ __attribute__((aligned(16))) float smem[];
    const Geo& g = a.g;
    const float gscale = scalars[1];
    auto stage = [&](int n, const Patch& p, float* P) { ce_stage(a, n, p, P); };
    auto pixel_grad = [&](int n, int y, int x, const Tap& ty, const Tap& tx, const Patch& p, const float* P, auto emit) -> bool {
        const size_t pix = ((size_t)n * g.H + y) * g.W + x;
        const int label = load_label(a, pix);
        if (ce_ignored(a, label)) return false;
        const Gather<false> gl = gather_staged(P, p, ty, tx);
        if (CT > 0) {
            RegVec<CT> r;
            fill<CT, false>(r, gl);
            ce_pixel_bwd<CT>(r, g.c, label, [&](int k, float v) { emit(k, gscale * v); });
        } else {
            ce_pixel_bwd<0>(gl, g.c, label, [&](int k, float v) { emit(k, gscale * v); });
        }
        return true;
    };
    tiled_scatter(g, stage, pixel_grad, grad, smem);
}

template <int CT>
__global__ __launch_bounds__(256) void ce_fused_tiled_kernel(CeArgs a, float* __restrict__ grad, float* __restrict__ partials) {
    extern __shared__ __attribute__((aligned(16))) float smem[];
    const Geo& g = a.g;
    float acc[2] = {0.0f, 0.0f};
    auto stage = [&](int n, const Patch& p, float* P) { ce_stage(a, n, p, P); };
    auto pixel_grad = [&](int n, int y, int x, const Tap& ty, const Tap& tx, const Patch& p, const float* P, auto emit) -> bool {
        const size_t pix = ((size_t)n * g.H + y) * g.W + x;
        const int label = load_label(a, pix);
        if (ce_ignored(a, label)) return false;
        const Gather<false> gl = gather_staged(P, p, ty, tx);
        float v;
        if (CT > 0) {
            RegVec<CT> r;
            fill<CT, false>(r, gl);
            v = ce_pixel_fwd_bwd<(CT > 0 ? CT : 1)>(r, gl(label), label, [&](int k, float gv) { emit(k, gv); });
        } else {
            v = ce_pixel_fwd<0>(gl, g.c, label);
            ce_pixel_bwd<0>(gl, g.c, label, [&](int k, float gv) { emit(k, gv); });
        }
        acc[0] += v;
        acc[1] += 1.0f;
        return true;
    };
    tiled_scatter(g, stage, pixel_grad, grad, smem);
    __shared__ float red[2 * 16];
    store_partials<2>(acc, red, partials);
}

static int g_loss_deterministic = -1;
bool loss_deterministic() {
    if (g_loss_deterministic < 0) {
        const char* e = getenv("CMS_LOSS_DETERMINISTIC");
        g_loss_deterministic = e ? (atoi(e) != 0) : 0;
    }
    return g_loss_deterministic != 0;
}

int fwd_tiles(const Geo& g, int n_patches, size_t* lds_out, int* stride_out) {
    if (is_ident(g)) return 0;
    static int on = -1;
    if (on < 0) {
        const char* e = getenv("CMS_LOSS_FWD_TILED");
        on = e ? (atoi(e) != 0) : 1;
    }
    if (!on) return 0;
    const size_t pf = patch_floats(g.c, g.sy, g.sx, FWD_TILE_H);
    const size_t lds = pf * n_patches * sizeof(float);
    if (lds > FWD_PATCH_LDS_MAX) return 0;
    if (lds_out) *lds_out = lds;
    if (stride_out) *stride_out = (int)pf;
    return ((g.W + TILE_W - 1) / TILE_W) * ((g.H + FWD_TILE_H - 1) / FWD_TILE_H) * g.n;
}

int fused_tiles(const Geo& g, int n_patches) {
    if (is_ident(g)) return 0;
    if (loss_deterministic()) return 0;
    static int on = -1;
    if (on < 0) {
        const char* e = getenv("CMS_LOSS_FUSED");
        on = e ? (atoi(e) != 0) : 1;
    }
    if (!on) return 0;
    if (tile_lds_bytes(g.c, g.sy, g.sx, n_patches) > TILE_LDS_MAX) return 0;
    return ((g.W + TILE_W - 1) / TILE_W) * ((g.H + TILE_H - 1) / TILE_H) * g.n;
}

static int check_cons(const cms_consistency_desc* d) {
    CMS_REQUIRE(d != nullptr, "consistency: null descriptor");
    CMS_REQUIRE(d->l_stu && d->l_tea0, "consistency: l_stu / l_tea0 must not be NULL");
    CMS_REQUIRE(d->mode == CMS_MODE_MIX || d->mode == CMS_MODE_CUT, "consistency: unknown mode %d", d->mode);
    CMS_REQUIRE(d->mode != CMS_MODE_MIX || d->l_tea1, "consistency: mix mode needs l_tea1");
    CMS_REQUIRE((d->ranges != nullptr) != (d->mask != nullptr), "consistency: give exactly one of ranges / mask");
    CMS_REQUIRE(d->ranges == nullptr || d->n_boxes >= 0, "consistency: n_boxes < 0");
    int rc = check_geometry(d, "consistency");
    return rc ? rc : check_loss_fn(d);
}

static ConsArgs make_cons_args(const cms_consistency_desc* d) {
    ConsArgs a;
    a.d = *d;
    a.g = geo_of(d);
    a.tau = d->conf_thresh;
    a.inv_root_c = (float)(1.0 / sqrt((double)d->c));
    return a;
}

static int check_ce(const cms_ce_desc* d) {
    CMS_REQUIRE(d != nullptr, "ce: null descriptor");
    CMS_REQUIRE(d->logits && d->labels, "ce: logits / labels NULL");
    CMS_REQUIRE(d->label_dtype == CMS_LABEL_U8 || d->label_dtype == CMS_LABEL_I64, "ce: bad label dtype");
    return check_geometry(d, "ce", "label");
}

static CeArgs make_ce_args(const cms_ce_desc* d) {
    CeArgs a;
    a.d = *d;
    a.g = geo_of(d);
    return a;
}

template <int K, class Kern, class... Args>
static void launch_fused(Kern kern, int tiles, size_t lds, hipStream_t s, float* partials, double* stats_out, double extra, int extra_slot,
                         Args... args) {
    allow_lds(kern, lds);
    hipLaunchKernelGGL(kern, dim3(tiles), dim3(256), lds, s, args..., partials);
    hipLaunchKernelGGL((reduce_partials_kernel<K>), dim3(1), dim3(256), 0, s, partials, tiles, stats_out, extra, extra_slot);
}

}

using namespace cms;

extern "C" size_t cms_consistency_workspace_bytes(const cms_consistency_desc* d) {
    if (!d) return 0;
    const Geo g = geo_of(d);
    return (size_t)std::max(fwd_blocks(g, 3), fused_tiles(g, 3)) * 3 * sizeof(float);
}

extern "C" int cms_consistency_fused_supported(const cms_consistency_desc* d) {
    if (check_cons(d)) return 0;
    return fused_tiles(geo_of(d), 3) > 0 ? 1 : 0;
}

extern "C" int cms_consistency_fwd_bwd(const cms_consistency_desc* d, float grad_unit, void* workspace, double* stats_out,
                                       float* grad_l_stu, void* stream) {
    int rc = check_cons(d);
    if (rc) return rc;
    CMS_REQUIRE(workspace && stats_out && grad_l_stu, "consistency_fwd_bwd: workspace / stats_out / grad NULL");
    ConsArgs a = make_cons_args(d);
    const int tiles = fused_tiles(a.g, 3);
    CMS_REQUIRE(tiles > 0, "consistency_fwd_bwd: not available for this geometry / mode (ask cms_consistency_fused_supported)");
    hipStream_t s = (hipStream_t)stream;
    const int pstride = (int)patch_floats(d->c, a.g.sy, a.g.sx, TILE_H);
    CMS_DISPATCH_C(d->c, {
        auto kern = d->loss_fn == CMS_LOSS_VAR ? cons_fused_tiled_kernel<CT, LOSS_VAR> : cons_fused_tiled_kernel<CT, -1>;
        launch_fused<3>(kern, tiles, tile_lds_bytes(d->c, a.g.sy, a.g.sx, 3), s, (float*)workspace, stats_out,
                        (double)((size_t)d->n * d->H * d->W), 3, a, grad_unit, grad_l_stu, pstride);
    });
    return launch_status("cms_consistency_fwd_bwd");
}

extern "C" int cms_scale_by_scalar(float* x, long long n, const float* scalars, int index, float factor, void* stream) {
    CMS_REQUIRE(x && scalars && n >= 0 && index >= 0, "scale_by_scalar: bad argument");
    if (n == 0) return CMS_OK;
    const int grid = (int)std::min<long long>((n + 255) / 256, 1024);
    hipLaunchKernelGGL(scale_by_scalar_kernel, dim3(grid), dim3(256), 0, (hipStream_t)stream, x, (size_t)n, scalars, index, factor);
    return launch_status("cms_scale_by_scalar");
}

extern "C" int cms_consistency_fwd(const cms_consistency_desc* d, void* workspace, double* stats_out, void* stream) {
    int rc = check_cons(d);
    if (rc) return rc;
    CMS_REQUIRE(workspace && stats_out, "consistency_fwd: workspace / stats_out NULL");
    ConsArgs a = make_cons_args(d);
    const FwdPlan p = fwd_plan(a.g, 3);
    CMS_DISPATCH_C(d->c, launch_fwd<3>(cons_fwd_tiled_kernel<CT>, cons_fwd_kernel<CT, true>, cons_fwd_kernel<CT, false>, a, p,
                                       (float*)workspace, stats_out, (double)((size_t)d->n * d->H * d->W), 3,
                                       (hipStream_t)stream, p.pstride));
    return launch_status("cms_consistency_fwd");
}

extern "C" int cms_consistency_finalize(const double* stats_local, const double* stats_global, float conf_thresh,
                                        int conf_per_pixel, float ramp_val, float cons_weight, float* scalars_out,
                                        void* stream) {
    CMS_REQUIRE(stats_local && stats_global && scalars_out, "consistency_finalize: NULL argument");
    hipLaunchKernelGGL(cons_finalize_kernel, dim3(1), dim3(64), 0, (hipStream_t)stream, stats_local, stats_global,
                       conf_thresh, conf_per_pixel, ramp_val, cons_weight, scalars_out);
    return launch_status("cms_consistency_finalize");
}

extern "C" int cms_loss_set_deterministic(int on) {
    cms::g_loss_deterministic = on ? 1 : 0;
    return CMS_OK;
}

extern "C" int cms_consistency_bwd(const cms_consistency_desc* d, const float* scalars, float* grad_l_stu,
                                   void* stream) {
    int rc = check_cons(d);
    if (rc) return rc;
    CMS_REQUIRE(scalars && grad_l_stu, "consistency_bwd: scalars / grad NULL");
    ConsArgs a = make_cons_args(d);
    const int pstride = (int)patch_floats(d->c, a.g.sy, a.g.sx, TILE_H);
    CMS_DISPATCH_C(d->c, rc = launch_bwd("consistency_bwd", cons_bwd_ident_kernel<CT>, cons_bwd_tiled_kernel<CT>, a, 3, 0, scalars,
                                         grad_l_stu, (hipStream_t)stream, pstride));
    return rc ? rc : launch_status("cms_consistency_bwd");
}

extern "C" size_t cms_ce_workspace_bytes(const cms_ce_desc* d) {
    if (!d) return 0;
    const Geo g = geo_of(d);
    return (size_t)std::max(fwd_blocks(g, 1), fused_tiles(g, 1)) * 2 * sizeof(float);
}

extern "C" int cms_ce_fused_supported(const cms_ce_desc* d) {
    if (check_ce(d)) return 0;
    return fused_tiles(geo_of(d), 1) > 0 ? 1 : 0;
}

extern "C" int cms_ce_fwd_bwd(const cms_ce_desc* d, void* workspace, double* stats_out, float* grad_logits, void* stream) {
    int rc = check_ce(d);
    if (rc) return rc;
    CMS_REQUIRE(workspace && stats_out && grad_logits, "ce_fwd_bwd: workspace / stats_out / grad NULL");
    const CeArgs a = make_ce_args(d);
    const int tiles = fused_tiles(a.g, 1);
    CMS_REQUIRE(tiles > 0, "ce_fwd_bwd: not available for this geometry / mode (ask cms_ce_fused_supported)");
    CMS_DISPATCH_C(d->c, launch_fused<2>(ce_fused_tiled_kernel<CT>, tiles, tile_lds_bytes(d->c, a.g.sy, a.g.sx, 1), (hipStream_t)stream,
                                         (float*)workspace, stats_out, 0.0, -1, a, grad_logits));
    return launch_status("cms_ce_fwd_bwd");
}

extern "C" int cms_ce_fwd(const cms_ce_desc* d, void* workspace, double* stats_out, void* stream) {
    int rc = check_ce(d);
    if (rc) return rc;
    CMS_REQUIRE(workspace && stats_out, "ce_fwd: workspace / stats_out NULL");
    const CeArgs a = make_ce_args(d);
    const FwdPlan p = fwd_plan(a.g, 1);
    CMS_DISPATCH_C(d->c, launch_fwd<2>(ce_fwd_tiled_kernel<CT>, ce_fwd_kernel<CT, true>, ce_fwd_kernel<CT, false>, a, p,
                                       (float*)workspace, stats_out, 0.0, -1, (hipStream_t)stream));
    return launch_status("cms_ce_fwd");
}

extern "C" int cms_ce_finalize(const double* stats, float loss_weight, float* scalars_out, void* stream) {
    CMS_REQUIRE(stats && scalars_out, "ce_finalize: NULL argument");
    hipLaunchKernelGGL(ce_finalize_kernel, dim3(1), dim3(64), 0, (hipStream_t)stream, stats, loss_weight, scalars_out);
    return launch_status("cms_ce_finalize");
}

extern "C" int cms_ce_bwd(const cms_ce_desc* d, const float* scalars, float* grad_logits, void* stream) {
    int rc = check_ce(d);
    if (rc) return rc;
    CMS_REQUIRE(scalars && grad_logits, "ce_bwd: scalars / grad NULL");
    const CeArgs a = make_ce_args(d);
    CMS_DISPATCH_C(d->c, rc = launch_bwd("ce_bwd", ce_bwd_ident_kernel<CT>, ce_bwd_tiled_kernel<CT>, a, 1, 0, scalars, grad_logits,
                                         (hipStream_t)stream));
    return rc ? rc : launch_status("cms_ce_bwd");
}
```

### cutmix-semisup-seg_amd/ops.py

```python
import ctypes as C

import numpy as np
import torch

from . import _lib
from ._lib import fn, check


def _stream():
    return C.c_void_p(torch.cuda.current_stream().cuda_stream)


def _ptr(t):
    return None if t is None else C.c_void_p(t.data_ptr())


def _need_cuda(*tensors):
    for t in tensors:
        if t is not None and not t.is_cuda:
            raise RuntimeError('cutmix-semisup-seg_amd ops run on the GPU only (got a {} tensor); there is no CPU '
                               'fallback'.format(t.device))


def _f32c(t):
# ... 69 lines not shown
        d.loss_fn = _lib.LOSS_IDS[self.loss_fn]
        d.conf_thresh = self.conf_thresh
        d.conf_per_pixel = int(self.conf_per_pixel)


class ConsistencyConfig(_LossConfig):

    def __init__(self, mode='mix', loss_fn='var', conf_thresh=0.97, conf_per_pixel=False, align_corners=True,
                 invert=True):
        if mode not in ('mix', 'cut'):
            raise ValueError('Unknown mask_mode {}'.format(mode))
        _LossConfig.__init__(self, loss_fn, conf_thresh, conf_per_pixel, align_corners)
        self.mode = mode
        self.invert = bool(invert)


def _nonempty_ranges(ranges):
    if ranges is not None and ranges.dim() == 3 and ranges.shape[1] == 0:
        return torch.zeros((int(ranges.shape[0]), 1, 4), dtype=torch.int32, device=ranges.device)
    return ranges


def _cons_desc(cfg, l_stu, l_tea0, l_tea1, ranges, mask, um0, um1, out_size):
    n, c, h, w = (int(s) for s in l_stu.shape)
    d = _lib.ConsistencyDesc()
    d.l_stu, d.l_tea0, d.l_tea1 = l_stu.data_ptr(), l_tea0.data_ptr(), (l_tea1.data_ptr() if l_tea1 is not None else None)
    d.ranges = ranges.data_ptr() if ranges is not None else None
    d.mask = mask.data_ptr() if mask is not None else None
    d.um0 = um0.data_ptr() if um0 is not None else None
    d.um1 = um1.data_ptr() if um1 is not None else None
    d.n, d.c, d.h, d.w = n, c, h, w
    d.H, d.W = int(out_size[0]), int(out_size[1])
    cfg.fill(d)
    d.n_boxes = int(ranges.shape[1]) if ranges is not None else 0
    d.invert = int(cfg.invert)
    d.mode = _lib.MODE_MIX if cfg.mode == 'mix' else _lib.MODE_CUT
    return d


def _workspace(name, d, device):
    return _workspace_bytes(int(fn['cms_{}_workspace_bytes'.format(name)](C.byref(d))), device)


def _workspace_bytes(nbytes, device):
    return torch.empty(max(int(nbytes), 16), dtype=torch.uint8, device=device)


def _check_grad_out(who, grad_out, like):
    if grad_out.dtype != torch.float32 or tuple(grad_out.shape) != tuple(like.shape) or not grad_out.is_contiguous():
        raise ValueError('{}: grad_out must be a contiguous f32 tensor of the logits\' shape'.format(who))


def _finalized_scalars(stats, stats_g, cfg, ramp_val, cons_weight):
    scalars = torch.empty(4, dtype=torch.float32, device=stats.device)
    check(fn['cms_consistency_finalize'](_ptr(stats), _ptr(stats_g), cfg.conf_thresh, int(cfg.conf_per_pixel),
                                         float(ramp_val), float(cons_weight), _ptr(scalars), _stream()),
          'cms_consistency_finalize')
    return scalars


def _allreduce_sum(t, group):
    import torch.distributed as dist
    if dist.is_available() and dist.is_initialized() and dist.get_world_size(group) > 1:
        dist.all_reduce(t, op=dist.ReduceOp.SUM, group=group)
        return True
    return False


def _cons_prepare(who, cfg, l_stu, l_tea0, l_tea1, out_size, ranges, mask, um0, um1, grad_out=None):
    _need_cuda(l_stu, l_tea0, l_tea1, ranges, mask, um0, um1, grad_out)
    l_stu, l_tea0, l_tea1 = _f32c(l_stu), _f32c(l_tea0), _f32c(l_tea1)
    mask, um0, um1 = _f32c(mask), _f32c(um0), _f32c(um1)
    ranges = _nonempty_ranges(ranges)
    if l_tea0.shape != l_stu.shape or (l_tea1 is not None and l_tea1.shape != l_stu.shape):
        raise ValueError('consistency: student / teacher logits shapes differ')
    if grad_out is not None:
        _check_grad_out(who, grad_out, l_stu)
    d = _cons_desc(cfg, l_stu, l_tea0, l_tea1, ranges, mask, um0, um1, out_size)
    return d, (l_stu, l_tea0, l_tea1, ranges, mask, um0, um1, cfg, tuple(int(v) for v in out_size))


def _cons_scalars(stats, cfg, ramp_val, cons_weight, group, sync_conf_rate):
    stats_g = stats
    if sync_conf_rate and cfg.conf_thresh > 0.0:
        g = stats.clone()
        if _allreduce_sum(g, group):
            stats_g = g
    return _finalized_scalars(stats, stats_g, cfg, ramp_val, cons_weight)


def consistency_forward(cfg, l_stu, l_tea0, l_tea1, out_size, ranges=None, mask=None, um0=None, um1=None,
                        ramp_val=1.0, cons_weight=1.0, group=None, sync_conf_rate=True):
    d, keep = _cons_prepare('consistency_forward', cfg, l_stu, l_tea0, l_tea1, out_size, ranges, mask, um0, um1)
    dev = keep[0].device
    ws = _workspace('consistency', d, dev)
    stats = torch.empty(4, dtype=torch.float64, device=dev)
    check(fn['cms_consistency_fwd'](C.byref(d), _ptr(ws), _ptr(stats), _stream()), 'cms_consistency_fwd')
    return _cons_scalars(stats, cfg, ramp_val, cons_weight, group, sync_conf_rate), (d, keep, stats)


def consistency_backward(ctx, scalars, grad_out=None, samples=None):
    d, keep, _ = ctx
    l_stu = keep[0]
    if grad_out is None:
        grad_out = torch.zeros_like(l_stu)
    if samples is not None:
        s0, s1 = int(samples[0]), int(samples[1])
        if not (0 <= s0 < s1 <= int(l_stu.shape[0])):
            raise ValueError('consistency_backward: bad sample range')
        sl = lambda t: None if t is None else t[s0:s1]
        l_s, l_t0, l_t1, ranges, mask, um0, um1, cfg, out_size = keep
        d = _cons_desc(cfg, sl(l_s), sl(l_t0), sl(l_t1), sl(ranges), sl(mask), sl(um0), sl(um1), out_size)
        check(fn['cms_consistency_bwd'](C.byref(d), _ptr(scalars), _ptr(grad_out[s0:s1]), _stream()), 'cms_consistency_bwd')
        return grad_out
    check(fn['cms_consistency_bwd'](C.byref(d), _ptr(scalars), _ptr(grad_out), _stream()), 'cms_consistency_bwd')
    return grad_out


def consistency_fused(cfg, l_stu, l_tea0, l_tea1, out_size, grad_out, ranges=None, mask=None, um0=None, um1=None,
                      ramp_val=1.0, cons_weight=1.0, group=None, sync_conf_rate=True):
    d, keep = _cons_prepare('consistency_fused', cfg, l_stu, l_tea0, l_tea1, out_size, ranges, mask, um0, um1, grad_out)
    l_stu, l_tea0, l_tea1, ranges, mask, um0, um1 = keep[:7]
    if not fn['cms_consistency_fused_supported'](C.byref(d)):
        sc, cctx = consistency_forward(cfg, l_stu, l_tea0, l_tea1, out_size, ranges, mask, um0, um1, ramp_val, cons_weight, group,
                                       sync_conf_rate)
        consistency_backward(cctx, sc, grad_out)
        return sc
    dev = l_stu.device
    ws = _workspace('consistency', d, dev)
    stats = torch.empty(4, dtype=torch.float64, device=dev)
    P = float(d.n) * float(d.H) * float(d.W)
    grad_unit = float(ramp_val) * float(cons_weight) / P
    check(fn['cms_consistency_fwd_bwd'](C.byref(d), grad_unit, _ptr(ws), _ptr(stats), _ptr(grad_out), _stream()),
          'cms_consistency_fwd_bwd')
    scalars = _cons_scalars(stats, cfg, ramp_val, cons_weight, group, sync_conf_rate)
    if cfg.conf_thresh > 0.0 and not cfg.conf_per_pixel:
        check(fn['cms_scale_by_scalar'](_ptr(grad_out), grad_out.numel(), _ptr(scalars), 1, 1.0, _stream()), 'cms_scale_by_scalar')
    return scalars


class _ConsistencyFn(torch.autograd.Function):
    @staticmethod
    def forward(ctx, l_stu, l_tea0, l_tea1, ranges, mask, um0, um1, cfg, out_size, ramp_val, cons_weight, group):
        scalars, c = consistency_forward(cfg, l_stu.detach(), l_tea0, l_tea1, out_size, ranges, mask, um0, um1,
                                         ramp_val, cons_weight, group)
        ctx.c = c
        ctx.scalars = scalars
        ctx.in_dtype = l_stu.dtype
        closs, rate, unsup = scalars[0], scalars[1], scalars[3]
        ctx.mark_non_differentiable(closs, rate)
        return unsup, closs, rate

    @staticmethod
    def backward(ctx, g_unsup, g_closs, g_rate):
        sc = ctx.scalars.clone()
        sc[2] = sc[2] * g_unsup
        grad = consistency_backward(ctx.c, sc)
        return (grad.to(ctx.in_dtype),) + (None,) * 11


def consistency_loss(l_stu, l_tea0, l_tea1, out_size, cfg, ranges=None, mask=None, um0=None, um1=None, ramp_val=1.0,
                     cons_weight=1.0, group=None):
    return _ConsistencyFn.apply(l_stu, l_tea0, l_tea1, ranges, mask, um0, um1, cfg, tuple(out_size), ramp_val,
                                cons_weight, group)


def _lam_vector(lam, n):
    lam = _f32c(lam).reshape(-1)
    if int(lam.numel()) != int(n):
        raise ValueError('ict: {} mix factors for {} samples'.format(int(lam.numel()), int(n)))
    return lam


def ict_blend(x0, x1, lam, out=None):
    _need_cuda(x0, x1, lam, out)
    if x0.shape != x1.shape or x0.dtype != x1.dtype:
        raise ValueError('ict_blend: x0/x1 shape or dtype mismatch')
    x0, x1 = x0.contiguous(), x1.contiguous()
    n = int(x0.shape[0])
    lam = _lam_vector(lam, n)
    if out is None:
        out = torch.empty_like(x0)
    elif out.shape != x0.shape or out.dtype != x0.dtype or not out.is_contiguous():
        raise ValueError('ict_blend: out must be a contiguous tensor of the inputs\' shape and dtype')
    if x0.numel() == 0:
        return out
    check(fn['cms_ict_blend'](_ptr(x0), _ptr(x1), _ptr(out), _dtype_code(x0), _ptr(lam), n, int(x0.numel()) // n, _stream()),
          'cms_ict_blend')
    return out


class ICTConsistencyConfig(_LossConfig):

    def __init__(self, loss_fn='var', conf_thresh=0.97, conf_per_pixel=False, align_corners=True):
        _LossConfig.__init__(self, loss_fn, conf_thresh, conf_per_pixel, align_corners)


def ict_consistency_forward(cfg, l_stu, l_tea0, l_tea1, lam, out_size, um0=None, um1=None, ramp_val=1.0, cons_weight=1.0):
    _need_cuda(l_stu, l_tea0, l_tea1, lam, um0, um1)
    l_stu, l_tea0, l_tea1 = _f32c(l_stu), _f32c(l_tea0), _f32c(l_tea1)
    um0, um1 = _f32c(um0), _f32c(um1)
    if l_tea0.shape != l_stu.shape or l_tea1.shape != l_stu.shape:
        raise ValueError('ict: student / teacher logits shapes differ')
    n, c, h, w = (int(s) for s in l_stu.shape)
    H, W = int(out_size[0]), int(out_size[1])
    for um in (um0, um1):
        if um is not None and int(um.numel()) != n * H * W:
            raise ValueError('ict: validity masks must be (N,1,H,W) of the loss geometry')
    lam = _lam_vector(lam, n)
    d = _lib.IctDesc()
    d.l_stu, d.l_tea0, d.l_tea1, d.lam = l_stu.data_ptr(), l_tea0.data_ptr(), l_tea1.data_ptr(), lam.data_ptr()
    d.um0 = um0.data_ptr() if um0 is not None else None
    d.um1 = um1.data_ptr() if um1 is not None else None
    d.n, d.c, d.h, d.w, d.H, d.W = n, c, h, w, H, W
    cfg.fill(d)
    dev = l_stu.device
    ws = _workspace('ict', d, dev)
    stats = torch.empty(4, dtype=torch.float64, device=dev)
    check(fn['cms_ict_fwd'](C.byref(d), _ptr(ws), _ptr(stats), _stream()), 'cms_ict_fwd')
    keep = (l_stu, l_tea0, l_tea1, lam, um0, um1)
    return _finalized_scalars(stats, stats, cfg, ramp_val, cons_weight), (d, keep, ws, stats)
# ... 51 lines not shown
    xf = aug_pixel_matrices(xf0_to_1, (H, W), l_stu.device)
    if int(xf.shape[0]) != n:
        raise ValueError('aug: {} warp matrices for {} samples'.format(int(xf.shape[0]), n))
    d = _lib.AugDesc()
    d.l_stu, d.l_tea, d.xf = l_stu.data_ptr(), l_tea.data_ptr(), xf.data_ptr()
    d.um0 = um0.data_ptr() if um0 is not None else None
    d.um1 = um1.data_ptr() if um1 is not None else None
    d.n, d.c, d.h, d.w, d.H, d.W = n, c, h, w, H, W
    cfg.fill(d)
    d.force_global = int(cfg.force_global)
    dev = l_stu.device
    ws = _workspace('aug', d, dev)
    stats = torch.empty(4, dtype=torch.float64, device=dev)
    check(fn['cms_aug_fwd'](C.byref(d), _ptr(ws), _ptr(stats), _stream()), 'cms_aug_fwd')
    keep = (l_stu, l_tea, xf, um0, um1)
    return _finalized_scalars(stats, stats, cfg, ramp_val, cons_weight), (d, keep, ws, stats)


def aug_consistency_backward(ctx, scalars, grad_out=None):
    d, keep, _, _ = ctx
    if grad_out is None:
        grad_out = torch.zeros_like(keep[0])
    else:
        _check_grad_out('aug_consistency_backward', grad_out, keep[0])
    check(fn['cms_aug_bwd'](C.byref(d), _ptr(scalars), _ptr(grad_out), _stream()), 'cms_aug_bwd')
    return grad_out


def _ce_desc(logits, labels, ignore_index, out_size, align_corners):
    n, c, h, w = (int(s) for s in logits.shape)
    d = _lib.CeDesc()
    d.logits, d.labels = logits.data_ptr(), labels.data_ptr()
    if labels.dtype == torch.uint8:
        d.label_dtype = _lib.LABEL_U8
    elif labels.dtype == torch.int64:
        d.label_dtype = _lib.LABEL_I64
    else:
        raise TypeError('labels must be uint8 or int64, got {}'.format(labels.dtype))
    d.ignore_index = int(ignore_index)
    d.n, d.c, d.h, d.w = n, c, h, w
    d.H, d.W = int(out_size[0]), int(out_size[1])
    d.align_corners = int(bool(align_corners))
    return d


def _ce_prepare(logits, labels, out_size, ignore_index, align_corners, grad_out=None):
    _need_cuda(logits, labels, grad_out)
    logits = _f32c(logits)
    labels = labels.contiguous()
    if labels.dim() == 4:
        labels = labels[:, 0].contiguous()
    if out_size is None:
        out_size = labels.shape[1:3]
    if tuple(labels.shape) != (logits.shape[0], int(out_size[0]), int(out_size[1])):
        raise ValueError('ce: labels shape {} does not match (N,H,W)=({}, {}, {})'.format(
            tuple(labels.shape), logits.shape[0], out_size[0], out_size[1]))
    if grad_out is not None:
        _check_grad_out('ce_fused', grad_out, logits)
    return _ce_desc(logits, labels, ignore_index, out_size, align_corners), logits, labels


def _ce_scalars(stats, loss_weight, group, sync_count):
    if sync_count:
        import torch.distributed as dist
        cnt = stats[1:2].clone()
        if _allreduce_sum(cnt, group):
            stats = torch.stack([stats[0], cnt[0] / dist.get_world_size(group)])
    scalars = torch.empty(2, dtype=torch.float32, device=stats.device)
    check(fn['cms_ce_finalize'](_ptr(stats), float(loss_weight), _ptr(scalars), _stream()), 'cms_ce_finalize')
    return scalars, stats


def ce_forward(logits, labels, out_size=None, ignore_index=255, align_corners=True, loss_weight=1.0, group=None,
               sync_count=False):
    d, logits, labels = _ce_prepare(logits, labels, out_size, ignore_index, align_corners)
    ws = _workspace('ce', d, logits.device)
    stats = torch.empty(2, dtype=torch.float64, device=logits.device)
    check(fn['cms_ce_fwd'](C.byref(d), _ptr(ws), _ptr(stats), _stream()), 'cms_ce_fwd')
    scalars, stats = _ce_scalars(stats, loss_weight, group, sync_count)
    return scalars, (d, (logits, labels), stats)


def ce_fused(logits, labels, grad_out, out_size=None, ignore_index=255, align_corners=True, loss_weight=1.0, group=None,
             sync_count=False):
    d, logits, labels = _ce_prepare(logits, labels, out_size, ignore_index, align_corners, grad_out)
    if not fn['cms_ce_fused_supported'](C.byref(d)):
        sc, cctx = ce_forward(logits, labels, out_size, ignore_index, align_corners, loss_weight, group, sync_count)
        ce_backward(cctx, sc, grad_out)
        return sc
    ws = _workspace('ce', d, logits.device)
    stats = torch.empty(2, dtype=torch.float64, device=logits.device)
    check(fn['cms_ce_fwd_bwd'](C.byref(d), _ptr(ws), _ptr(stats), _ptr(grad_out), _stream()), 'cms_ce_fwd_bwd')
    scalars, _ = _ce_scalars(stats, loss_weight, group, sync_count)
    check(fn['cms_scale_by_scalar'](_ptr(grad_out), grad_out.numel(), _ptr(scalars), 1, 1.0, _stream()), 'cms_scale_by_scalar')
    return scalars


def ce_backward(ctx, scalars, grad_out=None):
    d, keep, _ = ctx
    if grad_out is None:
        grad_out = torch.zeros_like(keep[0])
    check(fn['cms_ce_bwd'](C.byref(d), _ptr(scalars), _ptr(grad_out), _stream()), 'cms_ce_bwd')
    return grad_out


class _CeFn(torch.autograd.Function):
    @staticmethod
    def forward(ctx, logits, labels, out_size, ignore_index, align_corners):
        scalars, c = ce_forward(logits.detach(), labels, out_size, ignore_index, align_corners)
        ctx.c = c
        ctx.scalars = scalars
        ctx.in_dtype = logits.dtype
        return scalars[0]

    @staticmethod
    def backward(ctx, g):
        sc = ctx.scalars.clone()
        sc[1] = sc[1] * g
        return ce_backward(ctx.c, sc).to(ctx.in_dtype), None, None, None, None


def cross_entropy(logits, labels, out_size=None, ignore_index=255, align_corners=True):
    return _CeFn.apply(logits, labels, None if out_size is None else tuple(out_size), ignore_index, align_corners)


class _UpsampleFn(torch.autograd.Function):
    @staticmethod
    def forward(ctx, x, size, align_corners):
        _need_cuda(x)
        xin = _f32c(x)
        n, c, h, w = (int(s) for s in xin.shape)
        H, W = int(size[0]), int(size[1])
        out = torch.empty((n, c, H, W), dtype=torch.float32, device=x.device)
        check(fn['cms_upsample_bilinear_fwd'](_ptr(xin), _ptr(out), n, c, h, w, H, W, int(bool(align_corners)),
                                              _stream()), 'cms_upsample_bilinear_fwd')
        ctx.geo = (n, c, h, w, H, W, int(bool(align_corners)))
        ctx.in_dtype = x.dtype
        return out

    @staticmethod
    def backward(ctx, g):
        n, c, h, w, H, W, ac = ctx.geo
        g = _f32c(g)
        gi = torch.empty((n, c, h, w), dtype=torch.float32, device=g.device)
        check(fn['cms_upsample_bilinear_bwd'](_ptr(g), _ptr(gi), n, c, h, w, H, W, ac, _stream()),
              'cms_upsample_bilinear_bwd')
        return gi.to(ctx.in_dtype), None, None


def upsample_bilinear(x, size, align_corners=True):
    return _UpsampleFn.apply(x, tuple(size), align_corners)


_STREAM_POOL = {}


_ROLE_ALIASES = {'optimizer': 'wgrad1'}
_GOOD_STREAMS = {}
_STREAM_PROBE_LOG = []


def _probe_side_streams(dev):
    good = _GOOD_STREAMS.get(dev.index)
    if good is not None:
        return good
    n_cand = 6
    cands = [torch.cuda.Stream(device=dev) for _ in range(n_cand)]
    if _os.environ.get('CMS_STREAM_PROBE', '1') == '0' or not hasattr(torch.cuda, '_sleep'):
        good = _GOOD_STREAMS[dev.index] = cands
        return good
    cur = torch.cuda.current_stream(dev)
    spin = 200000
    streams = [cur] + cands

    def pair_ms(a, b):
        torch.cuda.synchronize(dev)
        e0, e1 = torch.cuda.Event(enable_timing=True), torch.cuda.Event(enable_timing=True)
        e0.record(a)
# ... 1283 lines not shown


def host_call(call):
    if _REC is None:
        call()
        return
    prog = _REC[0]
    prog.host_ops.append((prog.size(), _rec_stream_index(), call))


def memset_zero(t):
    _need_cuda(t)
    if _REC is None:
        t.zero_()
        return t
    if not t.is_contiguous():
        raise TypeError('memset_zero: contiguous tensor required')
    prog = _REC[0]
    idx = fn['cms_program_add_memset'](prog.h, _ptr(t), t.numel() * t.element_size(), _rec_stream_index(), prog.group)
    if idx < 0:
        check(idx, 'cms_program_add_memset')
    prog.keep.append(t)
    return t


def stream_wait(waiter, waited):
    if _REC is None:
        waiter.wait_stream(waited)
        return
    prog = _REC[0]
    idx = fn['cms_program_add_sync'](prog.h, _rec_stream_index(waited), _rec_stream_index(waiter), prog.group)
    if idx < 0:
        check(idx, 'cms_program_add_sync')


def _tap_arrays(taps):
    n = len(taps)
    dy = (C.c_int * n)(*[int(t[0]) for t in taps])
    dx = (C.c_int * n)(*[int(t[1]) for t in taps])
    return dy, dx, n


def aspp_gather_fwd(z, bias, taps, num_classes, out=None):
    _need_cuda(z, bias, out)
    if z.dtype != torch.float32 or not z.is_contiguous():
        raise TypeError('aspp_gather_fwd: contiguous fp32 (N, ZC, h, w) input required')
    n, zc, h, w = (int(v) for v in z.shape)
    if out is None:
        out = torch.empty((n, int(num_classes), h, w), dtype=torch.float32, device=z.device)
    dy, dx, nt = _tap_arrays(taps)
    if _REC is not None:
        prog = _REC[0]
        idx = fn['cms_program_add_aspp_gather'](prog.h, _ptr(z), _ptr(bias), _ptr(out), dy, dx, nt, n, int(num_classes), zc,
                                                h, w, _rec_stream_index(), prog.group)
        if idx < 0:
            check(idx, 'cms_program_add_aspp_gather')
        prog.keep += [t for t in (z, bias, out) if t is not None]
        prog.head_bytes += 4.0 * nt * int(num_classes) * n * h * w + 4.0 * out.numel()
        prog.head_bytes_alg += 4.0 * out.numel()
        return out
    check(fn['cms_aspp_gather_fwd'](_ptr(z), _ptr(bias), _ptr(out), dy, dx, nt, n, int(num_classes), zc, h, w, _stream()),
          'cms_aspp_gather_fwd')
    return out


def aspp_spread_bwd(dlogits, taps, zc, dtype, out=None):
    _need_cuda(dlogits, out)
    if dlogits.dtype != torch.float32 or not dlogits.is_contiguous():
        raise TypeError('aspp_spread_bwd: contiguous fp32 (N, C, h, w) gradient required')
    n, c, h, w = (int(v) for v in dlogits.shape)
    if out is None:
        out = torch.empty((n, h, w, int(zc)), dtype=dtype, device=dlogits.device)
    dy, dx, nt = _tap_arrays(taps)
    if _REC is not None:
        prog = _REC[0]
        idx = fn['cms_program_add_aspp_spread'](prog.h, _ptr(dlogits), _ptr(out), _dtype_code(out), dy, dx, nt, n, c,
                                                int(zc), h, w, _rec_stream_index(), prog.group)
        if idx < 0:
            check(idx, 'cms_program_add_aspp_spread')
        prog.keep += [dlogits, out]
        return out
    check(fn['cms_aspp_spread_bwd'](_ptr(dlogits), _ptr(out), _dtype_code(out), dy, dx, nt, n, c, int(zc), h, w, _stream()),
          'cms_aspp_spread_bwd')
    return out


_ZERO_PAGES = {}


def _zero_page(device):
    z = _ZERO_PAGES.get(device)
    if z is None:
        z = torch.zeros(32768, dtype=torch.bfloat16, device=device)
        _ZERO_PAGES[device] = z
    return z


_ROUTE_NAMES = {8: 'conv8_kernel', 2: 'conv_igemm_mixed_kernel', 1: 'conv_igemm_kernel<2, 2, 2, 2', 3: 'conv_igemm_kernel<1, 4, 2, 1',
                4: 'conv_igemm_kernel<1, 4, 1, 1', 0: 'other'}


def conv_taps(kh, kw, dilation, padding):
    return [(ky * dilation - padding, kx * dilation - padding) for ky in range(kh) for kx in range(kw)]


def conv_igemm(x, w_packed, taps, stride=1, out_hw=None, scale=None, bias=None, res=None, relu=False, mode=0,
               mask_src=None, out=None, out_f32_nchw=None, cout_real=None, out_stride=1, out_full_hw=None, tile=0,
               ksplit=1, variant=0, out_pixel_offset=0, mask_bits_out=None, mask_bits=None, stats=None,
               mask_gates_res=False):
    _need_cuda(x, w_packed, scale, bias, res, mask_src, out, out_f32_nchw, mask_bits_out, mask_bits)
    for t in (mask_bits_out, mask_bits):
        if t is not None and (t.dtype != torch.uint8 or not t.is_contiguous() or x.dtype != torch.bfloat16):
            raise TypeError('conv_igemm: ReLU mask bits are contiguous uint8 tensors of the bf16 entry point')
    if mask_bits is not None and mask_src is not None:
        raise ValueError('conv_igemm: mask_bits replaces mask_src')
    if mask_gates_res and (mask_bits is None or res is None or int(mode) != 1):
        raise ValueError('conv_igemm: mask_gates_res needs a data-gradient launch with res and mask_bits')
    if x.dtype not in (torch.bfloat16, torch.float32) or w_packed.dtype != x.dtype or not x.is_contiguous() \
            or not w_packed.is_contiguous():
        raise TypeError('conv_igemm: contiguous NHWC input and packed weights of one dtype (bf16 or fp32) required')
    for t in (res, mask_src, out):
        if t is not None and (t.dtype != x.dtype or not t.is_contiguous()):
            raise TypeError('conv_igemm: residual / mask / output tensors must be contiguous and of the input dtype')
    f32 = x.dtype == torch.float32
    n, h, w_in, cin = (int(s) for s in x.shape)
    ntaps, cout, cin_w = (int(s) for s in w_packed.shape)
    if cin_w != cin or ntaps != len(taps):
        raise ValueError('conv_igemm: weight / tap table does not match the input')
    ho, wo = (int(out_hw[0]), int(out_hw[1])) if out_hw is not None else (h, w_in)
    oh, ow = (int(out_full_hw[0]), int(out_full_hw[1])) if out_full_hw is not None else (ho, wo)
    d = _lib.ConvDesc()
    d.x, d.w = x.data_ptr(), w_packed.data_ptr()
    if out_f32_nchw is None:
        if out is None:
            out = torch.empty((n, oh, ow, cout), dtype=x.dtype, device=x.device)
            if out_stride > 1:
                memset_zero(out)
        shift = int(out_pixel_offset) * cout * x.element_size()
        if shift and (out_stride <= 1 or out is None):
            raise ValueError('conv_igemm: out_pixel_offset needs a caller-owned `out` and out_stride > 1')
        d.y, d.y32 = out.data_ptr() + shift, None
    else:
        d.y, d.y32 = None, out_f32_nchw.data_ptr()
    d.scale = scale.data_ptr() if scale is not None else None
    d.bias = bias.data_ptr() if bias is not None else None
    shift = int(out_pixel_offset) * cout * x.element_size() if out_f32_nchw is None else 0
    d.res = res.data_ptr() + shift if res is not None else None
    d.mask_src = mask_src.data_ptr() + shift if mask_src is not None else None
    d.n, d.h, d.w_in, d.cin = n, h, w_in, cin
    bshift = int(out_pixel_offset) * (int(w_packed.shape[1]) // 8) if out_f32_nchw is None else 0
    d.mask_bits_out = mask_bits_out.data_ptr() + bshift if mask_bits_out is not None else None
    d.mask_bits = mask_bits.data_ptr() + bshift if mask_bits is not None else None
    d.mask_gates_res = int(bool(mask_gates_res))
    d.ho, d.wo, d.cout = ho, wo, cout
    d.cout_real = cout if cout_real is None else int(cout_real)
    d.ntaps = ntaps
    for i, (dy, dx) in enumerate(taps):
        d.tap_dy[i], d.tap_dx[i] = int(dy), int(dx)
    d.stride = int(stride)
    d.out_h, d.out_w, d.out_stride = oh, ow, int(out_stride)
    d.relu, d.mode, d.tile = int(bool(relu)), int(mode), int(tile)
    d.ksplit = int(ksplit)
    zp = _zero_page(x.device)
    d.zeros, d.zeros_bytes = zp.data_ptr(), zp.numel() * 2
    d.variant = int(variant)
    tile_sums = None
# ... 331 lines not shown
```

### cutmix-semisup-seg_amd/step.py

```python
import os
import torch

from . import ops
from .graph_replay import GraphReplay


class StepConfig(object):
    def __init__(self, mask_mode='mix', cons_loss_fn='var', cons_weight=1.0, conf_thresh=0.97, conf_per_pixel=False,
                 rampup=-1, unsup_batch_ratio=1, invert=True, fuse_batches=True, compute_dtype=torch.bfloat16,
                 overlap_teacher=True, bucketed_allreduce=True, allreduce_dtype='fp32', deterministic=False,
                 early_optimizer=False):
        if mask_mode not in ('mix', 'zero', 'cut'):
            raise ValueError('Unknown mask_mode {}'.format(mask_mode))
        self.mix = mask_mode == 'mix'
        self.cons_weight = float(cons_weight)
        self.rampup = rampup
        self.unsup_batch_ratio = int(unsup_batch_ratio)
        self.fuse_batches = bool(fuse_batches)
        self.overlap_teacher = bool(overlap_teacher)
        self.bucketed_allreduce = bool(bucketed_allreduce)
        if allreduce_dtype not in ('fp32', 'bf16'):
            raise ValueError('allreduce_dtype must be fp32 or bf16')
        self.allreduce_dtype = allreduce_dtype
        self.deterministic = bool(deterministic)
# ... 286 lines not shown
            for bi, ub in enumerate(unsup_batches):
                x_stu = self._student_inputs(ub)
                if overlap:
                    l0, l1 = tea_out[bi]
                else:
                    with torch.no_grad():
                        l0 = self.teacher.forward_lowres(ub.x0_tea)
                        l1 = self.teacher.forward_lowres(ub.x1_tea) if cfg.mix else None
                ls = self.student.forward_lowres(x_stu)
                if overlap and bi == 0:
                    main.wait_stream(side)
                sc, cctx = ops.consistency_forward(cfg.cons, ls.detach(), l0, l1, out_size, ranges=ub.ranges, mask=ub.mask,
                                                   um0=ub.um0, um1=ub.um1, ramp_val=ramp,
                                                   cons_weight=cfg.cons_weight, group=self.group)
                ls.backward(ops.consistency_backward(cctx, sc).to(ls.dtype))
                cons_vals.append(sc)
        return ce_sc, cons_vals

    def _graph_wanted(self):
        env = os.environ.get('CMS_STEP_GRAPH', 'auto')
        if env in ('0', '1'):
            return env == '1' and self.world == 1
        layerwise = not any(hasattr(n, a) for n in (self.student, self.teacher) for a in ('_use_hip_body', '_use_hip_backbone'))
        return layerwise and self.world == 1

    def _separate_or_graphed(self, sup_x, sup_y, unsup_batches, ramp, out_size, use_unsup):
        cfg = self.cfg
        if not (sup_x.is_cuda and self._graph_wanted() and (cfg.rampup <= 0 or float(ramp) >= 1.0)):
            return self._separate_passes(sup_x, sup_y, unsup_batches, ramp, out_size, use_unsup)
        flat = [sup_x, sup_y]
        for u in (unsup_batches if use_unsup else ()):
            flat += [u.x0_tea, u.x1_tea, u.x0_stu, u.x1_stu, u.ranges, u.um0, u.um1, u.mask]
        extra = (float(ramp), tuple(out_size), bool(use_unsup), self.student.training, self.teacher.training,
                 getattr(self.student, 'compute_dtype', None), getattr(self.teacher, 'compute_dtype', None))

        def passes(ts, capturing):
            ubs = [UnsupBatch(x0t, rg, um0=m0, x1_tea=x1t, um1=m1, x0_stu=x0s, x1_stu=x1s, mask=mk)
                   for x0t, x1t, x0s, x1s, rg, m0, m1, mk in (ts[i:i + 8] for i in range(2, len(ts), 8))]
            overlap = not capturing or os.environ.get('CMS_STEP_GRAPH_OVERLAP', '1') != '0'
            return self._separate_passes(ts[0], ts[1], ubs, ramp, out_size, use_unsup, allow_overlap=overlap)

        return self._graphs.run(flat, extra, passes, nets=(self.student, self.teacher), device=sup_x.device)

    def _fused_passes(self, sup_x, sup_y, unsup_batches, ramp, out_size, use_unsup, independent, groups):
        cfg = self.cfg
        n_sup = sup_x.shape[0]
        stu_in = [sup_x]
        tea_in = []
        zev = None
        if use_unsup:
            main = torch.cuda.current_stream()
            side = self._teacher_stream() if (cfg.overlap_teacher and self.teacher is not self.student) else main
            if side is not main:
                side.wait_stream(main)
            zev = self._zero_grad(main)
            for ub in unsup_batches:
                tea_in.append(ub.x0_tea)
                if cfg.mix:
                    tea_in.append(ub.x1_tea)
            with torch.cuda.stream(side):
                x_tea = torch.cat(tea_in, dim=0) if len(tea_in) > 1 else tea_in[0]
            for ub in unsup_batches:
                stu_in.append(self._student_inputs(ub))
        else:
            self.student_optim.zero_grad()
        x_stu = torch.cat(stu_in, dim=0) if len(stu_in) > 1 else stu_in[0]
        if use_unsup and side is not main and self._both_on_executor():
            from .backbone_hip import run_body_pair
            with torch.cuda.stream(side), torch.no_grad():
                xt = self.teacher.stem_nhwc(x_tea)
            xs = self.student.stem_nhwc(x_stu)
            stu_lo, tea_lo = run_body_pair(self.student.hip_executor(), xs, self.teacher.hip_executor(), xt, side)
        else:
            if use_unsup:
                with torch.cuda.stream(side), torch.no_grad():
                    tea_lo = self.teacher.forward_lowres(x_tea)
            stu_lo = self.student.forward_lowres(x_stu)
        grad_lo = torch.zeros(stu_lo.shape, dtype=torch.float32, device=stu_lo.device)
        lo_det = stu_lo.detach()
        split = use_unsup and side is not main
        if split:
            side.wait_stream(main)
        cons_vals = []

        def consistency_branch():
            s_off, t_off = n_sup, 0
            for ub in unsup_batches:
                n = ub.x0_tea.shape[0]
                l0 = tea_lo[t_off:t_off + n]
                l1 = tea_lo[t_off + n:t_off + 2 * n] if cfg.mix else None
                t_off += 2 * n if cfg.mix else n
                sc = ops.consistency_fused(cfg.cons, lo_det[s_off:s_off + n], l0, l1, out_size, grad_lo[s_off:s_off + n],
                                           ranges=ub.ranges, mask=ub.mask, um0=ub.um0, um1=ub.um1, ramp_val=ramp,
                                           cons_weight=cfg.cons_weight, group=self.group)
                s_off += n
                if split and isinstance(sc, torch.Tensor):
                    sc.record_stream(main)
                cons_vals.append(sc)
        if split:
            with torch.cuda.stream(side):
                consistency_branch()
        ce_sc = ops.ce_fused(lo_det[:n_sup], sup_y, grad_lo[:n_sup], out_size, 255, self.align_corners, group=self.group)
        sex = self._student_executor()
        if split:
            if independent and groups is None and sex is not None and hasattr(sex, '_refresh_for_backward'):
                sex._refresh_for_backward()
            main.wait_stream(side)
        elif use_unsup:
            consistency_branch()
        ex = self._arm_buckets() or self._arm_early_optimizer()
        dex = sex if sex is not None and hasattr(sex, 'join_wgrad') else None
        if dex is not None:
            dex.defer_wgrad_join = True
        if zev is not None:
            main.wait_event(zev)
        try:
            stu_lo.backward(grad_lo.to(stu_lo.dtype))
        finally:
            if ex is not None:
                ex.grad_hook = None
            if dex is not None:
                dex.defer_wgrad_join = False
                dex.join_wgrad()
        return ce_sc, cons_vals

    def __call__(self, sup_x, sup_y, unsup_batches, ramp_val=1.0):
        cfg = self.cfg
        out_size = sup_x.shape[2:4]
        use_unsup = cfg.cons_weight > 0.0 and len(unsup_batches) > 0
        ramp = ramp_val if cfg.rampup > 0 else 1.0

        independent = self._samples_independent()
        groups = None if (independent or not cfg.fuse_batches) else self._sample_groups(sup_x.shape[0], unsup_batches, use_unsup)
        if groups is not None:
            self.student.set_sample_groups(groups[0])
            if use_unsup:
                self.teacher.set_sample_groups(groups[1])
        try:
            if cfg.fuse_batches and (independent or groups is not None):
                ce_sc, cons_vals = self._fused_passes(sup_x, sup_y, unsup_batches, ramp, out_size, use_unsup, independent, groups)
            else:
                ce_sc, cons_vals = self._separate_or_graphed(sup_x, sup_y, unsup_batches, ramp, out_size, use_unsup)

            ops.join_side_streams()
            self._allreduce_grads()
            if self._early_armed:
                self._early_armed = False
                torch.cuda.current_stream().wait_stream(self._opt_stream)
            self.student_optim.step()
            if self.teacher_optim is not None:
                self.teacher_optim.step()
            self._post_nan_probe(ce_sc[0])
            return step_result(ce_sc, cons_vals)
        finally:
            if groups is not None:
                self.student.set_sample_groups(1)
                self.teacher.set_sample_groups(1)
```

### include/cutmixseg.h

```cpp
#ifndef CUTMIXSEG_H
#define CUTMIXSEG_H

#include <stddef.h>
#include <stdint.h>

#ifdef __cplusplus
extern "C" {
#endif

#define CMS_VERSION 101

#define CMS_OK 0
#define CMS_EINVAL (-1)
#define CMS_ELAUNCH (-2)
#define CMS_EUNSUPPORTED (-3)

#define CMS_F32 0
#define CMS_BF16 1

#define CMS_LABEL_U8 0
#define CMS_LABEL_I64 1

#define CMS_LOSS_VAR 0
#define CMS_LOSS_LOGITS_VAR 1
#define CMS_LOSS_LOGITS_SMOOTHL1 2
#define CMS_LOSS_BCE 3
#define CMS_LOSS_KLD 4

#define CMS_MODE_MIX 0
#define CMS_MODE_CUT 1

int cms_version(void);
const char* cms_last_error(void);
int cms_device_info(int* n_cu, char* name_out, size_t name_cap);


int cms_boxmask_rasterize(const int32_t* ranges, int n, int n_boxes, int h, int w, int invert,
                          float* mask_out, void* stream);

int cms_cutmix_paste(const void* x0, const void* x1, void* out, int dtype, const int32_t* ranges, int n,
                     int n_boxes, int c, int h, int w, int invert, void* stream);

int cms_cutmix_paste_mask(const void* x0, const void* x1, void* out, int dtype, const float* mask, int n, int c,
                          int h, int w, void* stream);

typedef struct cms_consistency_desc {
    const float* l_stu;
    const float* l_tea0;
    const float* l_tea1;
    const int32_t* ranges;
    const float* mask;
    const float* um0;
    const float* um1;
    int n, c, h, w;
    int H, W;
    int align_corners;
    int n_boxes, invert;
    int mode;
    int loss_fn;
    float conf_thresh;
    int conf_per_pixel;
} cms_consistency_desc;

size_t cms_consistency_workspace_bytes(const cms_consistency_desc* d);

int cms_consistency_fwd(const cms_consistency_desc* d, void* workspace, double* stats_out, void* stream);

int cms_consistency_finalize(const double* stats_local, const double* stats_global, float conf_thresh,
                             int conf_per_pixel, float ramp_val, float cons_weight, float* scalars_out,
                             void* stream);

int cms_consistency_bwd(const cms_consistency_desc* d, const float* scalars, float* grad_l_stu, void* stream);

int cms_consistency_fused_supported(const cms_consistency_desc* d);
int cms_consistency_fwd_bwd(const cms_consistency_desc* d, float grad_unit, void* workspace, double* stats_out,
                            float* grad_l_stu, void* stream);
int cms_scale_by_scalar(float* x, long long n, const float* scalars, int index, float factor, void* stream);

typedef struct cms_ce_desc {
    const float* logits;
    const void* labels;
    int label_dtype;
    int ignore_index;
    int n, c, h, w, H, W, align_corners;
} cms_ce_desc;

size_t cms_ce_workspace_bytes(const cms_ce_desc* d);
int cms_ce_fwd(const cms_ce_desc* d, void* workspace, double* stats_out, void* stream);
int cms_ce_finalize(const double* stats, float loss_weight, float* scalars_out, void* stream);
int cms_ce_bwd(const cms_ce_desc* d, const float* scalars, float* grad_logits, void* stream);
int cms_ce_fused_supported(const cms_ce_desc* d);
int cms_ce_fwd_bwd(const cms_ce_desc* d, void* workspace, double* stats_out, float* grad_logits, void* stream);
int cms_loss_set_deterministic(int on);


int cms_ict_blend(const void* x0, const void* x1, void* out, int dtype, const float* lam, int n, long long chw, void* stream);

typedef struct cms_ict_desc {
    const float* l_stu;
    const float* l_tea0;
    const float* l_tea1;
    const float* lam;
    const float* um0;
    const float* um1;
    int n, c, h, w;
    int H, W;
    int align_corners;
    int loss_fn;
    float conf_thresh;
    int conf_per_pixel;
} cms_ict_desc;

size_t cms_ict_workspace_bytes(const cms_ict_desc* d);

int cms_ict_fwd(const cms_ict_desc* d, void* workspace, double* stats_out, void* stream);

int cms_ict_bwd(const cms_ict_desc* d, const void* workspace, const float* scalars, float* grad_l_stu, void* stream);


typedef struct cms_aug_desc {
    const float* l_stu;
    const float* l_tea;
    const float* xf;
    const float* um0;
    const float* um1;
    int n, c, h, w;
    int H, W;
    int align_corners;
    int loss_fn;
    float conf_thresh;
    int conf_per_pixel;
    int force_global;
} cms_aug_desc;

size_t cms_aug_workspace_bytes(const cms_aug_desc* d);

int cms_aug_fwd(const cms_aug_desc* d, void* workspace, double* stats_out, void* stream);

int cms_aug_bwd(const cms_aug_desc* d, const float* scalars, float* grad_l_stu, void* stream);

int cms_upsample_bilinear_fwd(const float* lo, float* hi, int n, int c, int h, int w, int H, int W,
                              int align_corners, void* stream);
int cms_upsample_bilinear_bwd(const float* grad_hi, float* grad_lo, int n, int c, int h, int w, int H, int W,
                              int align_corners, void* stream);


int cms_ema_flat(float* tgt, const float* src, size_t count, float alpha, float one_minus_alpha,
                 uint16_t* tgt_bf16_out, void* stream);

typedef struct cms_param_segment {
    uint64_t offset;
    uint64_t count;
    int32_t k_updates;
    int32_t lr_group;
} cms_param_segment;

typedef struct cms_optim_desc {
    float* param;
    const float* grad;
    float* slot0;
    float* slot1;
    float* ema_param;
    uint16_t* param_bf16;
    uint16_t* ema_bf16;
    const cms_param_segment* segments;
    const uint32_t* chunk_seg;
    const uint32_t* chunk_off;
    uint32_t n_chunks;
    const double* lrs;
    const int64_t* step_count;
    float grad_scale;
    float ema_alpha;
    float ema_one_minus_alpha;
    double beta1, beta2, eps;
    float momentum, weight_decay;
// ... 127 lines not shown
    void* out1;
    uint8_t* out_labels;
    float* out_mask;
    const float* params;
    float mean[3], std_[3];
    int n, hs, ws, h, w;
    int out_dtype;
} cms_augment_desc;
int cms_augment_batch(const cms_augment_desc* d, void* stream);
int cms_augment_luma(const cms_augment_desc* d, float* luma, void* stream);

typedef struct cms_stage_entry {
    long long img_off;
    long long lab_off;
    int hs, ws;
} cms_stage_entry;
typedef struct cms_stage_desc {
    const uint8_t* pool_img;
    const uint8_t* pool_labels;
    const cms_stage_entry* entries;
    const int* index;
    void* out0;
    void* out1;
    uint8_t* out_labels;
    float* out_mask;
    const float* params;
    float mean[3], std_[3];
    int n, n_entries, h, w;
    int out_dtype;
} cms_stage_desc;
int cms_stage_batch(const cms_stage_desc* d, void* stream);
int cms_stage_luma(const cms_stage_desc* d, float* luma, void* stream);

enum cms_bn_what { CMS_BN_REDUCE = 0, CMS_BN_FINALIZE, CMS_BN_APPLY, CMS_BN_REDUCE_BWD, CMS_BN_BWD_APPLY, CMS_BN_COUNT,
                   CMS_BN_STATS, CMS_BN_FINALIZE_TILES, CMS_BN_BWD_SUMS_TILES };

typedef struct cms_bn_op {
    int what;
    int dtype, c, relu;
    const void* x;
    const void* res;
    void* y;
    const void* dy;
    void* dx;
    void* dres;
    double* sums;
    const float* gamma;
    const float* beta;
    float* mean;
    float* rstd;
    float* scale;
    float* shift;
    float* running_mean;
    float* running_var;
    long long* counter;
    double* clear_a;
    double* clear_b;
    void* ws;
    double count;
    unsigned long long n_pixels;
    float eps, momentum;
    int groups;
    int tile_rows;
    void* mask_bits;
} cms_bn_op;

size_t cms_bn_workspace_bytes(size_t n_pixels, int c, int groups);
int cms_bn_run(const cms_bn_op* op, void* stream);
int cms_frozen_bn_act_bwd(const void* dy, const void* y, void* dx, void* dres, int dtype, const float* scale, size_t n_pixels, int c,
                          void* stream);

int cms_channel_copy(const void* src, size_t src_pitch, void* dst, size_t dst_pitch, size_t rows, int channels, int dtype,
                     size_t row_div, void* stream);
int cms_add_n(const void* const* srcs, int k, void* dst, size_t n, int dtype, void* stream);
int cms_rows_reduce(const void* src, size_t pitch, int n, size_t rows_per_sample, int channels, int dtype, float* dst,
                    float scale, void* stream);
int cms_upsample_nhwc(const void* src, void* dst, size_t dst_pitch, int n, int h, int w, int H, int W, int channels, int dtype,
                      int align_corners, int backward, void* stream);

int cms_aspp_gather_fwd(const float* z, const float* bias, float* logits, const int* tap_dy, const int* tap_dx, int n_taps,
                        int n, int c, int zc, int h, int w, void* stream);
int cms_aspp_spread_bwd(const float* dlogits, void* d_nhwc, int d_dtype, const int* tap_dy, const int* tap_dx, int n_taps,
                        int n, int c, int zc, int h, int w, void* stream);

int cms_stem_pack_weights(const void* w_khkwcoci, int w_dtype, float* w_packed, void* stream);
int cms_stem_out_hw(int h, int w, int* ho, int* wo, int* hp, int* wp);
int cms_stem_fwd(const void* x_nchw, int x_dtype, void* y_nhwc, int y_dtype, const float* w_packed, const float* scale,
                 const float* bias, int n, int h, int w, void* stream);
int cms_maxpool3x3s2_fwd(const void* s_nhwc, void* p_nhwc, uint8_t* argmax, int dtype, int n, int hs, int ws, int c,
                         int ceil_mode, void* stream);
int cms_maxpool3x3s2_relu_bwd(const void* dp_nhwc, const uint8_t* argmax, const void* s_nhwc, void* ds_nhwc, int dtype,
                              int n, int hs, int ws, int c, int ceil_mode, void* stream);
int cms_stem_wgrad(const void* x_nchw, int x_dtype, const void* ds_nhwc, int ds_dtype, float* dw_khkwcoci,
                   const float* scale, int n, int h, int w, void* stream);
long long cms_stem_wgrad_workspace_bytes(int x_dtype, int ds_dtype, int n, int h, int w);
int cms_stem_wgrad_ws(const void* x_nchw, int x_dtype, const void* ds_nhwc, int ds_dtype, float* dw_khkwcoci,
                      const float* scale, int n, int h, int w, void* workspace, long long workspace_bytes, void* stream);
int cms_stem_dgrad(const void* ds_nhwc, int ds_dtype, const float* w_packed, const float* scale, float* dx_nchw, int n,
                   int h, int w, void* stream);

#define CMS_PROGRAM_MAX_STREAMS 4
typedef struct cms_program cms_program;
int cms_program_create(cms_program** out);
int cms_program_destroy(cms_program* p);
int cms_program_add_conv(cms_program* p, const cms_conv_desc* d, int f32, int stream_idx, int group);
int cms_program_add_wgrad(cms_program* p, const cms_wgrad_desc* d, int f32, int stream_idx, int group);
int cms_program_add_wgrad_group(cms_program* p, const void* table_dev, int n_items, int total_blocks, int kind, int stream_idx,
                                int group);
int cms_program_add_memset(cms_program* p, void* ptr, size_t bytes, int stream_idx, int group);
int cms_program_add_aspp_gather(cms_program* p, const float* z, const float* bias, float* logits, const int* tap_dy,
                                const int* tap_dx, int n_taps, int n, int c, int zc, int h, int w, int stream_idx, int group);
int cms_program_add_aspp_spread(cms_program* p, const float* dlogits, void* d_nhwc, int d_dtype, const int* tap_dy,
                                const int* tap_dx, int n_taps, int n, int c, int zc, int h, int w, int stream_idx, int group);
int cms_program_add_sync(cms_program* p, int from_stream, int to_stream, int group);
typedef struct cms_wfinish_item {
    float* scratch;
    float* grad;
    const uint16_t* w;
    const float* scale;
    float* wdot;
    int ntaps, cout, cin;
    int first_block;
} cms_wfinish_item;
int cms_channel_sum(const void* src, int dtype, size_t rows, int channels, float* dst, void* stream);
int cms_wgrad_finish_pack(cms_wfinish_item* items, int n_items);
int cms_wgrad_finish_run(const void* items_dev, int n_items, int total_blocks, void* stream);
int cms_program_add_channel_sum(cms_program* p, const void* src, int dtype, size_t rows, int channels, float* dst, int stream_idx,
                                int group);
int cms_program_add_wgrad_finish(cms_program* p, const void* items_dev, int n_items, int total_blocks, int stream_idx, int group);

int cms_program_add_bn(cms_program* p, const cms_bn_op* op, int stream_idx, int group);
int cms_program_size(const cms_program* p);
int cms_program_run(cms_program* p, int first, int last, void* const* streams, int n_streams);
int cms_program_run_pair(cms_program* a, void* const* streams_a, int na, cms_program* b, void* const* streams_b, int nb);
int cms_program_set_timing(cms_program* p, int every_k);
int cms_program_read_timing(cms_program* p, double* sum_ms, double* sum_flops, long* launches, double* head_ms,
                            long* head_launches);

int cms_fft2(void* data, int batch, int fh, int fw, int inverse, const void* tw_h, const void* tw_w, void* stream);

typedef struct cms_pd_patch {
    long long img_off;
    int hs, ws;
    int cy, cx;
} cms_pd_patch;
int cms_pd_load_image(const uint8_t* pool_img, const cms_stage_entry* entry_host, int ph, int pw, int fh, int fw, void* planes,
                      int64_t* sq, void* stream);
int cms_pd_load_patches(const uint8_t* pool_img, const cms_pd_patch* patches, int n, int ph, int pw, int fh, int fw, void* planes,
                        void* stream);
int cms_pd_patch_sqdiff(const uint8_t* pool_img, const cms_pd_patch* a, const cms_pd_patch* b, int n, int ph, int pw, int64_t* out,
                        void* stream);
int cms_pd_spectrum_product(const void* f_img, const void* f_pairs, int n_pairs, int fh, int fw, void* out, void* stream);
int cms_pd_finish(const void* corr, const int64_t* p2, const int64_t* q2, int n, int h, int w, int fh, int fw, int64_t* d2,
                  int64_t* keys, uint64_t* residual_bits, void* stream);
size_t cms_select_workspace_bytes(int n);
int cms_select_k_smallest(const int64_t* keys, const uint8_t* mask, const uint8_t* labels, const int32_t* cls, int mode, int n,
                          long long m, int k, int64_t* out, int32_t* count, void* workspace, size_t workspace_bytes, void* stream);

int cms_pd_box_sum(const void* in, int in_is_int64, int hp, int wp, int ph, int pw, void* work, int64_t* out, void* stream);
size_t cms_pd_neighbour_workspace_bytes(int hs, int ws, int ph, int pw);
int cms_pd_neighbour_maps(const uint8_t* pool_img, const cms_stage_entry* entry_host, int ph, int pw, void* work, int64_t* out_d2,
                          void* stream);

int cms_downsample_image_u8(const uint8_t* src, int n, int h, int w, int d, uint8_t* dst, void* stream);
int cms_downsample_labels_u8(const uint8_t* src, int n, int h, int w, int d, uint8_t* dst, void* stream);

// ... 73 lines not shown
```

Baseline: 641.7 images/sec.

## Defer loss-gradient scaling into ASPP spread and reorder head wgrad behind dgrad

The CE and consistency fused losses no longer launch a separate scale-by-scalar pass over the logit gradient. A per-sample scale table is passed down so the ASPP spread-backward kernel, and the bias-gradient reduction via scale_by_table, apply the loss scalars inline. The backward program now records from the spread output instead of copying dlogits into a program buffer. The head weight-gradient is launched after the head dgrad so the dgrad chain starts sooner. This adds new kernels, ticket-based finalisation and more stream bookkeeping, and applies only to single-GPU runs with fp32 logits.

```diff
diff --git a/cutmix-semisup-seg_amd/_lib.py b/cutmix-semisup-seg_amd/_lib.py
--- a/cutmix-semisup-seg_amd/_lib.py
+++ b/cutmix-semisup-seg_amd/_lib.py
@@ -158,6 +158,17 @@
 class WfinishItem(C.Structure):
     _fields_ = [('scratch', c_void_p), ('grad', c_void_p), ('w', c_void_p), ('scale', c_void_p), ('wdot', c_void_p),
                 ('ntaps', c_int), ('cout', c_int), ('cin', c_int), ('first_block', c_int)]
+
+
+SCALE_ENTRIES = 4
+
+
+class ScaleEntry(C.Structure):
+    _fields_ = [('first_sample', c_int), ('index', c_int), ('scalars', c_void_p)]
+
+
+class ScaleTable(C.Structure):
+    _fields_ = [('n', c_int), ('e', ScaleEntry * SCALE_ENTRIES)]
 
 
 _P = C.POINTER
@@ -186,6 +197,12 @@
     'cms_consistency_fused_supported': (c_int, [_P(ConsistencyDesc)]),
     'cms_consistency_fwd_bwd': (c_int, [_P(ConsistencyDesc), c_float, c_void_p, c_void_p, c_void_p, c_void_p]),
     'cms_scale_by_scalar': (c_int, [c_void_p, C.c_longlong, c_void_p, c_int, c_float, c_void_p]),
+    'cms_consistency_fwd_bwd_final': (c_int, [_P(ConsistencyDesc), c_float, c_float, c_float, c_void_p, c_void_p, c_void_p, c_void_p,
+                                              c_void_p, c_void_p]),
+    'cms_scale_by_table': (c_int, [c_void_p, c_void_p, c_int, C.c_longlong, _P(ScaleTable), c_void_p]),
+    'cms_ce_fwd_bwd_final': (c_int, [_P(CeDesc), c_float, c_void_p, c_void_p, c_void_p, c_void_p, c_void_p, c_void_p]),
+    'cms_aspp_spread_bwd_scaled': (c_int, [c_void_p, _P(ScaleTable), c_void_p, c_int, _P(c_int), _P(c_int), c_int, c_int, c_int, c_int,
+                                           c_int, c_int, c_void_p]),
     'cms_ict_blend': (c_int, [c_void_p, c_void_p, c_void_p, c_int, c_void_p, c_int, C.c_longlong, c_void_p]),
     'cms_ict_workspace_bytes': (c_size_t, [_P(IctDesc)]),
     'cms_ict_fwd': (c_int, [_P(IctDesc), c_void_p, c_void_p, c_void_p]),
diff --git a/cutmix-semisup-seg_amd/backbone_hip.py b/cutmix-semisup-seg_amd/backbone_hip.py
--- a/cutmix-semisup-seg_amd/backbone_hip.py
+++ b/cutmix-semisup-seg_amd/backbone_hip.py
@@ -35,6 +35,8 @@
 
 
 class DeepLabHipExecutor(object):
+    takes_dlogits_scale = True
+
     def __init__(self, net, dtype=torch.bfloat16):
         self._init_common(net, dtype)
         self.num_classes = net.num_classes
@@ -88,6 +90,8 @@
         self.overlap_wgrad = True
         self.wgrad_streams = 2 if os.environ.get('CMS_WGRAD8', '1') != '0' else 1
         self.defer_wgrad_join = False
+        self.head_wgrad_behind_dgrad = True
+        self.dlogits_scale = None
         self._pending_join = None
         self._sides = []
         self.conv_tile = 0
@@ -388,10 +392,11 @@
     def _wgrad_raw(self, du, x, c):
         ops.conv_wgrad(du, x, c.taps, self.arena.packed(c.wkey, self.arena.grad), stride=c.stride, wg_target=self._wg_target())
 
-    def _backward_chain_bn(self, saved, dlg, want_w, sides, hook, box=None):
+    def _backward_chain_bn(self, saved, dlg, want_w, sides, hook, box=None, d=None, scale=None):
         x4 = saved[-1]
         main = torch.cuda.current_stream()
-        d = ops.aspp_spread_bwd(dlg, self.aspp_taps, self.aspp_zc, self.dtype)
+        if d is None:
+            d = self._spread(dlg, scale)
         dwall = None
         if want_w:
             dwall = torch.empty((1, self.aspp_zc, 2048), dtype=torch.float32, device=d.device)
@@ -628,15 +633,21 @@
             self._refresh_backward_weights()
             self._wT_version = self.version
 
-    def _head_bias_grads(self, dlogits, want_w, side=None):
-        if want_w:
-            if side is not None:
-                side.wait_stream(torch.cuda.current_stream())
-                dlogits.record_stream(side)
-            with torch.cuda.stream(side if side is not None else torch.cuda.current_stream()):
-                db = dlogits.sum(dim=(0, 2, 3))
-                for k in self.aspp_keys:
-                    self.arena.view(k + '.bias', self.arena.grad).add_(db)
+    def _head_bias_grads(self, dlogits, want_w, side=None, scale=None):
+        if not want_w:
+            return dlogits if not scale else None
+        if side is not None:
+            side.wait_stream(torch.cuda.current_stream())
+            dlogits.record_stream(side)
+            for _, sc, _ in (scale or ()):
+                if sc is not None:
+                    sc.record_stream(side)
+        with torch.cuda.stream(side if side is not None else torch.cuda.current_stream()):
+            src = ops.scale_by_table(dlogits, ops.scale_table(scale)) if scale else dlogits
+            db = src.sum(dim=(0, 2, 3))
+            for k in self.aspp_keys:
+                self.arena.view(k + '.bias', self.arena.grad).add_(db)
+        return src
 
     def _head_weight_grads(self, dwall, side=None):
         C = self.num_classes
@@ -654,25 +665,40 @@
         l2, l3, l4 = self._layer_first[1], self._layer_first[2], self._layer_first[3]
         return sorted(set([0, l2, l3, (l3 + l4 + 1) // 2, l4]))
 
-    def _backward_chain(self, saved, dlg, want_w, sides, hook, box=None):
+    def _spread(self, dlg, scale, out=None):
+        if scale:
+            return ops.aspp_spread_bwd_scaled(dlg, ops.scale_table(scale), self.aspp_taps, self.aspp_zc, self.dtype, out=out)
+        return ops.aspp_spread_bwd(dlg, self.aspp_taps, self.aspp_zc, self.dtype, out=out)
+
+    def _backward_chain(self, saved, dlg, want_w, sides, hook, box=None, d=None, scale=None):
         x4 = saved[-1]
         main = torch.cuda.current_stream()
-        d = ops.aspp_spread_bwd(dlg, self.aspp_taps, self.aspp_zc, self.dtype)
+        if d is None:
+            d = self._spread(dlg, scale)
         dwall = None
         keep = []
-        if want_w:
-            dwall = torch.empty((1, self.aspp_zc, 2048), dtype=torch.float32, device=d.device)
+
+        def head_wgrad():
+            dw = torch.empty((1, self.aspp_zc, 2048), dtype=torch.float32, device=d.device)
             hs = sides[0] if sides else None
             if hs is not None:
                 ops.stream_wait(hs, main)
-                keep.append((d, dwall))
+                keep.append((d, dw))
             with torch.cuda.stream(hs if hs is not None else main):
-                ops.memset_zero(dwall)
-                ops.conv_wgrad(d, x4, [(0, 0)], dwall)
+                ops.memset_zero(dw)
+                ops.conv_wgrad(d, x4, [(0, 0)], dw)
             if box is not None:
-                box['dwall'] = dwall
+                box['dwall'] = dw
+            return dw
+        behind = self.head_wgrad_behind_dgrad and bool(sides)
+        if want_w and not behind:
+            dwall = head_wgrad()
         x4b = getattr(x4, '_cms_relu_bits', None)
         dC = ops.conv_igemm(d, self.aspp_wallT, [(0, 0)], mode=1, mask_src=None if x4b is not None else x4, mask_bits=x4b)
+        if ops._REC is not None:
+            ops._REC[0].head_end = ops._REC[0].size()
+        if want_w and behind:
+            dwall = head_wgrad()
         capture = getattr(self, 'debug_capture', None)
         closes = set(self.bucket_starts())
         for bi in range(len(self.blocks) - 1, -1, -1):
@@ -713,10 +739,11 @@
         main = torch.cuda.current_stream()
         sides = self._side_streams(self.wgrad_streams) if (self.overlap_wgrad and want_w) else []
         hside = sides[0] if (sides and not bn) else None
+        scale, self.dlogits_scale = self.dlogits_scale, None
         if not self.use_programs:
             if self.defer_wgrad_join and sides:
                 self._pending_join = list(sides)
-            self._head_bias_grads(dlogits, want_w, hside)
+            self._head_bias_grads(dlogits, want_w, hside, scale)
             box = {}
 
             def hook(bi):
@@ -725,7 +752,7 @@
                     box['done'] = True
                 if self.grad_hook is not None:
                     self.grad_hook(bi)
-            dx, dwall = chain(token, dlogits, want_w, sides, hook, box)
+            dx, dwall = chain(token, dlogits, want_w, sides, hook, box, scale=scale)
             if dwall is not None and 'done' not in box:
                 self._finish_head(dwall, hside)
             return dx
@@ -734,27 +761,31 @@
             raise RuntimeError('the activations of this forward pass were overwritten by a later forward pass of the '
                                'same shape through the same executor (programs keep ONE set of buffers per shape): '
                                'run backward before the next forward, or set executor.use_programs = False')
-        key = (want_w, len(sides), bool(self.defer_wgrad_join))
+        key = (want_w, len(sides), bool(self.defer_wgrad_join), bool(self.head_wgrad_behind_dgrad))
         if self.defer_wgrad_join and sides:
             self._pending_join = list(sides)
         prog = fprog.bwd.get(key)
         if prog is None:
             prog = ops.Program()
-            dlg = torch.empty(tuple(dlogits.shape), dtype=torch.float32, device=dlogits.device)
+            d_in = torch.empty((n, h, w, self.aspp_zc), dtype=self.dtype, device=dlogits.device)
             streams = [main] + sides
+            prog.head_end = None
             with ops.recording(prog, streams):
-                dx, dwall = chain(fprog.saved, dlg, want_w, sides, prog.mark)
-            prog.dlg, prog.dx, prog.dwall = dlg, dx, dwall
+                dx, dwall = chain(fprog.saved, None, want_w, sides, prog.mark, d=d_in)
+            prog.d_in, prog.dx, prog.dwall = d_in, dx, dwall
             fprog.bwd[key] = prog
-        prog.dlg.copy_(dlogits)
-        self._head_bias_grads(dlogits, want_w, hside)
+        self._spread(dlogits, scale, out=prog.d_in)
         streams = [main] + sides
+        first = 0
+        if hside is not None and want_w and self.head_wgrad_behind_dgrad and prog.head_end:
+            prog.run(streams, 0, prog.head_end)
+            first = prog.head_end
+        prog.dlg = self._head_bias_grads(dlogits, want_w, hside, scale)
         if self.grad_hook is None or not want_w:
-            prog.run(streams)
+            prog.run(streams, first, -1)
             if prog.dwall is not None:
                 self._finish_head(prog.dwall, hside)
         else:
-            first = 0
             hook_stream = sides[0] if sides else main
             head_done = False
             wanted = getattr(self.grad_hook, 'blocks', None)
@@ -817,6 +848,7 @@
 
 
 class DeepLabV3PlusBackboneExecutor(DeepLabHipExecutor):
+    takes_dlogits_scale = False
 
     def __init__(self, wrapper, dtype=torch.bfloat16):
         self._init_common(wrapper, dtype)
@@ -1333,10 +1365,13 @@
         ctx.executor = ex_stu
         ctx.saved_acts = saved
         ctx.mark_non_differentiable(logits_t)
+        ctx.set_materialize_grads(False)
         return logits_s, logits_t
 
     @staticmethod
     def backward(ctx, dlogits, _unused):
+        if dlogits is None:
+            return None, None, None, None, None, None
         dx = ctx.executor.backward(ctx.saved_acts, dlogits.contiguous().float())
         ctx.saved_acts = None
         return dx, None, None, None, None, None
diff --git a/cutmix-semisup-seg_amd/csrc/aspp.hip b/cutmix-semisup-seg_amd/csrc/aspp.hip
--- a/cutmix-semisup-seg_amd/csrc/aspp.hip
+++ b/cutmix-semisup-seg_amd/csrc/aspp.hip
@@ -42,12 +42,12 @@
     }
 }
 
-template <class T>
-__global__ __launch_bounds__(256) void aspp_spread_bwd_kernel(const float* __restrict__ dl, T* __restrict__ d, AsppTaps tp,
-                                                              int N, int C, int ZC, int H, int W) {
-    __shared__ short sdy[CMS_CONV_MAX_TAPS], sdx[CMS_CONV_MAX_TAPS];
-    taps_to_lds(tp, sdy, sdx);
+template <class T, bool SCALED>
+__device__ __forceinline__ void aspp_spread_body(const float* __restrict__ dl, T* __restrict__ d, const AsppTaps& tp, const short* sdy,
+                                                 const short* sdx, int N, int C, int ZC, int H, int W, const cms_scale_table& tb) {
     const int n_taps = tp.n_taps;
+    ScaleFactors sf;
+    if constexpr (SCALED) sf = scale_table_load(tb);
     const unsigned zc8 = (unsigned)ZC / 8u;
     const size_t total = (size_t)N * H * W * zc8;
     const size_t plane = (size_t)H * W;
@@ -59,6 +59,9 @@
         const int y = (int)(t % (unsigned)H);
         const int n = (int)(t / (unsigned)H);
         const float* dn = dl + (size_t)n * C * plane;
+        float f = 1.0f;
+        bool scaled = false;
+        if constexpr (SCALED) scaled = scale_table_pick(tb, sf, n, f);
         float v[8];
         int k = (int)((ch * 8u) / (unsigned)C), c = (int)(ch * 8u) - k * C;
 #pragma unroll
@@ -66,7 +69,10 @@
             float val = 0.0f;
             if (k < n_taps) {
                 const int yy = y - sdy[k], xx = x - sdx[k];
-                if ((unsigned)yy < (unsigned)H && (unsigned)xx < (unsigned)W) val = dn[(size_t)c * plane + (size_t)yy * W + xx];
+                if ((unsigned)yy < (unsigned)H && (unsigned)xx < (unsigned)W) {
+                    val = dn[(size_t)c * plane + (size_t)yy * W + xx];
+                    if (SCALED && scaled) val *= f;
+                }
             }
             v[e] = val;
             if (++c == C) { c = 0; ++k; }
@@ -84,6 +90,22 @@
             *reinterpret_cast<uint4*>(d + i * 8) = o;
         }
     }
+}
+
+template <class T>
+__global__ __launch_bounds__(256) void aspp_spread_bwd_kernel(const float* __restrict__ dl, T* __restrict__ d, AsppTaps tp,
+                                                              int N, int C, int ZC, int H, int W) {
+    __shared__ short sdy[CMS_CONV_MAX_TAPS], sdx[CMS_CONV_MAX_TAPS];
+    taps_to_lds(tp, sdy, sdx);
+    aspp_spread_body<T, false>(dl, d, tp, sdy, sdx, N, C, ZC, H, W, cms_scale_table{});
+}
+
+template <class T>
+__global__ __launch_bounds__(256) void aspp_spread_bwd_scaled_kernel(const float* __restrict__ dl, T* __restrict__ d, AsppTaps tp,
+                                                                     int N, int C, int ZC, int H, int W, cms_scale_table tb) {
+    __shared__ short sdy[CMS_CONV_MAX_TAPS], sdx[CMS_CONV_MAX_TAPS];
+    taps_to_lds(tp, sdy, sdx);
+    aspp_spread_body<T, true>(dl, d, tp, sdy, sdx, N, C, ZC, H, W, tb);
 }
 
 }
@@ -114,8 +136,8 @@
     return launch_status("cms_aspp_gather_fwd");
 }
 
-extern "C" int cms_aspp_spread_bwd(const float* dlogits, void* d_nhwc, int d_dtype, const int* tap_dy, const int* tap_dx,
-                                   int n_taps, int n, int c, int zc, int h, int w, void* stream) {
+static int spread_launch(const float* dlogits, void* d_nhwc, int d_dtype, const int* tap_dy, const int* tap_dx, int n_taps, int n,
+                         int c, int zc, int h, int w, const cms_scale_table* table, void* stream) {
     CMS_REQUIRE(dlogits && d_nhwc, "aspp_spread_bwd: NULL pointer");
     CMS_REQUIRE(d_dtype == CMS_F32 || d_dtype == CMS_BF16, "aspp_spread_bwd: bad dtype");
     CMS_REQUIRE(n > 0 && c > 0 && h > 0 && w > 0 && zc >= n_taps * c, "aspp_spread_bwd: bad geometry (zc >= taps * classes)");
@@ -126,11 +148,32 @@
     const size_t total = (size_t)n * h * w * (zc / 8);
     CMS_REQUIRE(total < (1ull << 32), "aspp_spread_bwd: more than 2^32 chunks");
     hipStream_t s = (hipStream_t)stream;
+    const dim3 grid(grid_for(total, 256, 256 * 16));
+    if (table) {
+        if (d_dtype == CMS_F32)
+            hipLaunchKernelGGL(aspp_spread_bwd_scaled_kernel<float>, grid, dim3(256), 0, s, dlogits, (float*)d_nhwc, tp, n, c, zc, h, w,
+                               *table);
+        else
+            hipLaunchKernelGGL(aspp_spread_bwd_scaled_kernel<uint16_t>, grid, dim3(256), 0, s, dlogits, (uint16_t*)d_nhwc, tp, n, c, zc,
+                               h, w, *table);
+        return launch_status("cms_aspp_spread_bwd_scaled");
+    }
     if (d_dtype == CMS_F32)
-        hipLaunchKernelGGL(aspp_spread_bwd_kernel<float>, dim3(grid_for(total, 256, 256 * 16)), dim3(256), 0, s, dlogits,
-                           (float*)d_nhwc, tp, n, c, zc, h, w);
+        hipLaunchKernelGGL(aspp_spread_bwd_kernel<float>, grid, dim3(256), 0, s, dlogits, (float*)d_nhwc, tp, n, c, zc, h, w);
     else
-        hipLaunchKernelGGL(aspp_spread_bwd_kernel<uint16_t>, dim3(grid_for(total, 256, 256 * 16)), dim3(256), 0, s, dlogits,
-                           (uint16_t*)d_nhwc, tp, n, c, zc, h, w);
+        hipLaunchKernelGGL(aspp_spread_bwd_kernel<uint16_t>, grid, dim3(256), 0, s, dlogits, (uint16_t*)d_nhwc, tp, n, c, zc, h, w);
     return launch_status("cms_aspp_spread_bwd");
 }
+
+extern "C" int cms_aspp_spread_bwd(const float* dlogits, void* d_nhwc, int d_dtype, const int* tap_dy, const int* tap_dx,
+                                   int n_taps, int n, int c, int zc, int h, int w, void* stream) {
+    return spread_launch(dlogits, d_nhwc, d_dtype, tap_dy, tap_dx, n_taps, n, c, zc, h, w, nullptr, stream);
+}
+
+extern "C" int cms_aspp_spread_bwd_scaled(const float* dlogits, const cms_scale_table* table, void* d_nhwc, int d_dtype,
+                                          const int* tap_dy, const int* tap_dx, int n_taps, int n, int c, int zc, int h, int w,
+                                          void* stream) {
+    const int rc = check_scale_table(table, "aspp_spread_bwd_scaled");
+    if (rc) return rc;
+    return spread_launch(dlogits, d_nhwc, d_dtype, tap_dy, tap_dx, n_taps, n, c, zc, h, w, table, stream);
+}
diff --git a/cutmix-semisup-seg_amd/csrc/common.hpp b/cutmix-semisup-seg_amd/csrc/common.hpp
--- a/cutmix-semisup-seg_amd/csrc/common.hpp
+++ b/cutmix-semisup-seg_amd/csrc/common.hpp
@@ -54,6 +54,35 @@
     }
 }
 
+struct ScaleFactors {
+    float f[CMS_SCALE_ENTRIES];
+    bool has[CMS_SCALE_ENTRIES];
+};
+
+__device__ __forceinline__ ScaleFactors scale_table_load(const cms_scale_table& tb) {
+    ScaleFactors s;
+#pragma unroll
+    for (int e = 0; e < CMS_SCALE_ENTRIES; ++e) {
+        s.has[e] = e < tb.n && tb.e[e].scalars != nullptr;
+        s.f[e] = s.has[e] ? tb.e[e].scalars[tb.e[e].index] : 1.0f;
+    }
+    return s;
+}
+
+__device__ __forceinline__ bool scale_table_pick(const cms_scale_table& tb, const ScaleFactors& s, int sample, float& f) {
+    bool has = false;
+    f = 1.0f;
+#pragma unroll
+    for (int e = 0; e < CMS_SCALE_ENTRIES; ++e)
+        if (e < tb.n && sample >= tb.e[e].first_sample) {
+            has = s.has[e];
+            f = s.f[e];
+        }
+    return has;
+}
+
+int check_scale_table(const cms_scale_table* tb, const char* who);
+
 bool conv8_supported(const cms_conv_desc* d);
 int conv8_launch(const cms_conv_desc* d, hipStream_t s, void* trace, int trace_wgs);
 bool wgrad8_supported(const cms_wgrad_desc* d);
diff --git a/cutmix-semisup-seg_amd/csrc/loss_tiles.hpp b/cutmix-semisup-seg_amd/csrc/loss_tiles.hpp
--- a/cutmix-semisup-seg_amd/csrc/loss_tiles.hpp
+++ b/cutmix-semisup-seg_amd/csrc/loss_tiles.hpp
@@ -202,32 +202,68 @@
     }
 }
 
+template <int K, bool IN_LAUNCH>
+__device__ __forceinline__ void reduce_partials_block(const float* partials, int nblocks, double* sm, double (&res)[K]) {
+    double loc[K];
+#pragma unroll
+    for (int k = 0; k < K; ++k) loc[k] = 0.0;
+    for (int i = threadIdx.x; i < nblocks; i += 256) {
+#pragma unroll
+        for (int k = 0; k < K; ++k) {
+            float v;
+            if constexpr (IN_LAUNCH) v = __hip_atomic_load(partials + i * K + k, __ATOMIC_RELAXED, __HIP_MEMORY_SCOPE_AGENT);
+            else v = partials[i * K + k];
+            loc[k] += (double)v;
+        }
+    }
+#pragma unroll
+    for (int k = 0; k < K; ++k) sm[k * 256 + threadIdx.x] = loc[k];
+    __syncthreads();
+    for (int s = 128; s > 0; s >>= 1) {
+        if ((int)threadIdx.x < s) {
+#pragma unroll
+            for (int k = 0; k < K; ++k) sm[k * 256 + threadIdx.x] += sm[k * 256 + threadIdx.x + s];
+        }
+        __syncthreads();
+    }
+#pragma unroll
+    for (int k = 0; k < K; ++k) res[k] = sm[k * 256];
+}
+
 template <int K>
 __global__ __launch_bounds__(256) void reduce_partials_kernel(const float* __restrict__ partials, int nblocks,
                                                               double* __restrict__ out, double extra, int extra_slot) {
-    __shared__ double sm[K][256];
-    double loc[K];
-#pragma unroll
-    for (int k = 0; k < K; ++k) loc[k] = 0.0;
-    for (int i = threadIdx.x; i < nblocks; i += 256) {
-#pragma unroll
-        for (int k = 0; k < K; ++k) loc[k] += (double)partials[i * K + k];
-    }
-#pragma unroll
-    for (int k = 0; k < K; ++k) sm[k][threadIdx.x] = loc[k];
-    __syncthreads();
-    for (int s = 128; s > 0; s >>= 1) {
-        if ((int)threadIdx.x < s) {
-#pragma unroll
-            for (int k = 0; k < K; ++k) sm[k][threadIdx.x] += sm[k][threadIdx.x + s];
-        }
-        __syncthreads();
-    }
+    __shared__ double sm[K * 256];
+    double res[K];
+    reduce_partials_block<K, false>(partials, nblocks, sm, res);
     if (threadIdx.x == 0) {
 #pragma unroll
-        for (int k = 0; k < K; ++k) out[k] = sm[k][0];
+        for (int k = 0; k < K; ++k) out[k] = res[k];
         if (extra_slot >= 0) out[extra_slot] = extra;
     }
+}
+
+template <int K>
+__device__ __forceinline__ bool store_partials_ticket(float (&acc)[K], float* red, float* partials, unsigned* ticket) {
+    block_sum<K>(acc, red);
+    if (threadIdx.x == 0) {
+#pragma unroll
+        for (int k = 0; k < K; ++k) __hip_atomic_store(partials + blockIdx.x * K + k, acc[k], __ATOMIC_RELAXED, __HIP_MEMORY_SCOPE_AGENT);
+        asm volatile("s_waitcnt vmcnt(0)" ::: "memory");
+        const unsigned prev = __hip_atomic_fetch_add(ticket, 1u, __ATOMIC_RELAXED, __HIP_MEMORY_SCOPE_AGENT);
+        const bool last = prev == gridDim.x - 1;
+        if (last) {
+            __builtin_amdgcn_fence(__ATOMIC_ACQUIRE, "agent");
+            asm volatile("s_waitcnt vmcnt(0)" ::: "memory");
+        }
+        red[15] = last ? 1.0f : 0.0f;
+    }
+    __syncthreads();
+    return red[15] != 0.0f;
+}
+
+__device__ __forceinline__ void ticket_reset(unsigned* ticket) {
+    __hip_atomic_store(ticket, 0u, __ATOMIC_RELAXED, __HIP_MEMORY_SCOPE_AGENT);
 }
 
 #ifndef CMS_LOSS_TILE_H
diff --git a/cutmix-semisup-seg_amd/csrc/losses.hip b/cutmix-semisup-seg_amd/csrc/losses.hip
--- a/cutmix-semisup-seg_amd/csrc/losses.hip
+++ b/cutmix-semisup-seg_amd/csrc/losses.hip
@@ -97,9 +97,8 @@
     store_partials<3>(acc, red, partials);
 }
 
-__global__ void cons_finalize_kernel(const double* __restrict__ sl, const double* __restrict__ sg, float tau,
-                                     int per_pixel, float ramp, float weight, float* __restrict__ out) {
-    if (threadIdx.x != 0 || blockIdx.x != 0) return;
+__device__ __forceinline__ void cons_finalize(const double* sl, const double* sg, float tau, int per_pixel, float ramp, float weight,
+                                              float* out) {
     const double Pl = sl[3];
     double closs, gs, rate;
     if (tau > 0.0f) {
@@ -121,6 +120,12 @@
     out[1] = (float)rate;
     out[2] = (float)(gs * (double)ramp * (double)weight);
     out[3] = (float)(closs * (double)weight);
+}
+
+__global__ void cons_finalize_kernel(const double* __restrict__ sl, const double* __restrict__ sg, float tau,
+                                     int per_pixel, float ramp, float weight, float* __restrict__ out) {
+    if (threadIdx.x != 0 || blockIdx.x != 0) return;
+    cons_finalize(sl, sg, tau, per_pixel, ramp, weight, out);
 }
 
 template <int CT>
@@ -196,13 +201,11 @@
 }
 
 template <int CT, int LF>
-__global__ __launch_bounds__(256, (LF >= 0 && CT > 0) ? 4 : 1) void cons_fused_tiled_kernel(ConsArgs a, float grad_unit, float* __restrict__ grad,
-                                                               int patch_stride, float* __restrict__ partials) {
-    extern __shared__ __attribute__((aligned(16))) float smem[];
+__device__ __forceinline__ void cons_fused_tile(const ConsArgs& a, float grad_unit, float* __restrict__ grad, int patch_stride, float* smem,
+                                                float (&acc)[3]) {
     const Geo& g = a.g;
     const bool pp = a.tau > 0.0f && a.d.conf_per_pixel;
     const int pstride = patch_stride;
-    float acc[3] = {0.0f, 0.0f, 0.0f};
     auto stage = [&](int n, const Patch& p, float* P) { cons_stage(a, n, p, P, pstride); };
     auto pixel_grad = [&](int n, int y, int x, const Tap& ty, const Tap& tx, const Patch& p, const float* P, auto emit) -> bool {
         const ConsPixel px = cons_pixel_inputs(a, n, y, x);
@@ -231,14 +234,61 @@
         return true;
     };
     tiled_scatter(g, stage, pixel_grad, grad, smem);
+}
+
+template <int CT, int LF>
+__global__ __launch_bounds__(256, (LF >= 0 && CT > 0) ? 4 : 1) void cons_fused_tiled_kernel(ConsArgs a, float grad_unit, float* __restrict__ grad,
+                                                               int patch_stride, float* __restrict__ partials) {
+    extern __shared__ __attribute__((aligned(16))) float smem[];
+    float acc[3] = {0.0f, 0.0f, 0.0f};
+    cons_fused_tile<CT, LF>(a, grad_unit, grad, patch_stride, smem, acc);
     __shared__ float red[3 * 16];
     store_partials<3>(acc, red, partials);
 }
+
+struct ConsFin {
+    unsigned* ticket;
+    double* stats;
+    float* scalars;
+    double pixels;
+    float ramp, weight;
+};
+
+template <int CT, int LF>
+__global__ __launch_bounds__(256, (LF >= 0 && CT > 0) ? 4 : 1) void cons_fused_final_kernel(ConsArgs a, float grad_unit, float* __restrict__ grad,
+                                                               int patch_stride, float* partials, ConsFin fin) {
+    extern __shared__ __attribute__((aligned(16))) float smem[];
+    float acc[3] = {0.0f, 0.0f, 0.0f};
+    cons_fused_tile<CT, LF>(a, grad_unit, grad, patch_stride, smem, acc);
+    __shared__ float red[3 * 16];
+    if (!store_partials_ticket<3>(acc, red, partials, fin.ticket)) return;
+    double sums[3];
+    reduce_partials_block<3, true>(partials, (int)gridDim.x, reinterpret_cast<double*>(smem), sums);
+    if (threadIdx.x == 0) {
+        const double st[4] = {sums[0], sums[1], sums[2], fin.pixels};
+#pragma unroll
+        for (int k = 0; k < 4; ++k) fin.stats[k] = st[k];
+        cons_finalize(st, st, a.tau, a.d.conf_per_pixel, fin.ramp, fin.weight, fin.scalars);
+        ticket_reset(fin.ticket);
+    }
+}
+
 
 __global__ __launch_bounds__(256) void scale_by_scalar_kernel(float* __restrict__ x, size_t n, const float* __restrict__ scalars,
                                                               int idx, float factor) {
     const float f = scalars[idx] * factor;
     for (size_t i = (size_t)blockIdx.x * blockDim.x + threadIdx.x; i < n; i += (size_t)gridDim.x * blockDim.x) x[i] *= f;
+}
+
+__global__ __launch_bounds__(256) void scale_by_table_kernel(const float* __restrict__ src, float* __restrict__ dst, size_t per_sample,
+                                                             size_t n, cms_scale_table tb) {
+    const ScaleFactors sf = scale_table_load(tb);
+    for (size_t i = (size_t)blockIdx.x * blockDim.x + threadIdx.x; i < n; i += (size_t)gridDim.x * blockDim.x) {
+        float f;
+        const bool has = scale_table_pick(tb, sf, (int)(i / per_sample), f);
+        const float v = src[i];
+        dst[i] = has ? v * f : v;
+    }
 }
 
 struct CeArgs {
@@ -307,10 +357,14 @@
     store_partials<2>(acc, red, partials);
 }
 
+__device__ __forceinline__ void ce_finalize(const double* stats, float weight, float* out) {
+    out[0] = (float)(stats[0] / stats[1]);
+    out[1] = stats[1] > 0.0 ? (float)((double)weight / stats[1]) : 0.0f;
+}
+
 __global__ void ce_finalize_kernel(const double* __restrict__ stats, float weight, float* __restrict__ out) {
     if (threadIdx.x != 0 || blockIdx.x != 0) return;
-    out[0] = (float)(stats[0] / stats[1]);
-    out[1] = stats[1] > 0.0 ? (float)((double)weight / stats[1]) : 0.0f;
+    ce_finalize(stats, weight, out);
 }
 
 template <int CT>
@@ -359,10 +413,8 @@
 }
 
 template <int CT>
-__global__ __launch_bounds__(256) void ce_fused_tiled_kernel(CeArgs a, float* __restrict__ grad, float* __restrict__ partials) {
-    extern __shared__ __attribute__((aligned(16))) float smem[];
-    const Geo& g = a.g;
-    float acc[2] = {0.0f, 0.0f};
+__device__ __forceinline__ void ce_fused_tile(const CeArgs& a, float* __restrict__ grad, float* smem, float (&acc)[2]) {
+    const Geo& g = a.g;
     auto stage = [&](int n, const Patch& p, float* P) { ce_stage(a, n, p, P); };
     auto pixel_grad = [&](int n, int y, int x, const Tap& ty, const Tap& tx, const Patch& p, const float* P, auto emit) -> bool {
         const size_t pix = ((size_t)n * g.H + y) * g.W + x;
@@ -383,9 +435,41 @@
         return true;
     };
     tiled_scatter(g, stage, pixel_grad, grad, smem);
+}
+
+template <int CT>
+__global__ __launch_bounds__(256) void ce_fused_tiled_kernel(CeArgs a, float* __restrict__ grad, float* __restrict__ partials) {
+    extern __shared__ __attribute__((aligned(16))) float smem[];
+    float acc[2] = {0.0f, 0.0f};
+    ce_fused_tile<CT>(a, grad, smem, acc);
     __shared__ float red[2 * 16];
     store_partials<2>(acc, red, partials);
 }
+
+struct CeFin {
+    unsigned* ticket;
+    double* stats;
+    float* scalars;
+    float weight;
+};
+
+template <int CT>
+__global__ __launch_bounds__(256) void ce_fused_final_kernel(CeArgs a, float* __restrict__ grad, float* partials, CeFin fin) {
+    extern __shared__ __attribute__((aligned(16))) float smem[];
+    float acc[2] = {0.0f, 0.0f};
+    ce_fused_tile<CT>(a, grad, smem, acc);
+    __shared__ float red[2 * 16];
+    if (!store_partials_ticket<2>(acc, red, partials, fin.ticket)) return;
+    double st[2];
+    reduce_partials_block<2, true>(partials, (int)gridDim.x, reinterpret_cast<double*>(smem), st);
+    if (threadIdx.x == 0) {
+        fin.stats[0] = st[0];
+        fin.stats[1] = st[1];
+        ce_finalize(st, fin.weight, fin.scalars);
+        ticket_reset(fin.ticket);
+    }
+}
+
 
 static int g_loss_deterministic = -1;
 bool loss_deterministic() {
@@ -508,6 +592,58 @@
     return launch_status("cms_scale_by_scalar");
 }
 
+extern "C" int cms_consistency_fwd_bwd_final(const cms_consistency_desc* d, float grad_unit, float ramp_val, float cons_weight,
+                                             void* workspace, unsigned* ticket, double* stats_out, float* scalars_out,
+                                             float* grad_l_stu, void* stream) {
+    int rc = check_cons(d);
+    if (rc) return rc;
+    CMS_REQUIRE(workspace && ticket && stats_out && scalars_out && grad_l_stu,
+                "consistency_fwd_bwd_final: workspace / ticket / stats_out / scalars_out / grad NULL");
+    ConsArgs a = make_cons_args(d);
+    const int tiles = fused_tiles(a.g, 3);
+    CMS_REQUIRE(tiles > 0, "consistency_fwd_bwd_final: not available for this geometry / mode (ask cms_consistency_fused_supported)");
+    const int pstride = (int)patch_floats(d->c, a.g.sy, a.g.sx, TILE_H);
+    ConsFin fin;
+    fin.ticket = ticket;
+    fin.stats = stats_out;
+    fin.scalars = scalars_out;
+    fin.pixels = (double)((size_t)d->n * d->H * d->W);
+    fin.ramp = ramp_val;
+    fin.weight = cons_weight;
+    const size_t lds = std::max(tile_lds_bytes(d->c, a.g.sy, a.g.sx, 3), (size_t)3 * 256 * sizeof(double));
+    CMS_DISPATCH_C(d->c, {
+        auto kern = d->loss_fn == CMS_LOSS_VAR ? cons_fused_final_kernel<CT, LOSS_VAR> : cons_fused_final_kernel<CT, -1>;
+        allow_lds(kern, lds);
+        hipLaunchKernelGGL(kern, dim3(tiles), dim3(256), lds, (hipStream_t)stream, a, grad_unit, grad_l_stu, pstride,
+                           (float*)workspace, fin);
+    });
+    return launch_status("cms_consistency_fwd_bwd_final");
+}
+
+int cms::check_scale_table(const cms_scale_table* tb, const char* who) {
+    CMS_REQUIRE(tb != nullptr, "%s: NULL scale table", who);
+    CMS_REQUIRE(tb->n >= 0 && tb->n <= CMS_SCALE_ENTRIES, "%s: a scale table holds 0..%d entries", who, CMS_SCALE_ENTRIES);
+    for (int e = 0; e < tb->n; ++e) {
+        CMS_REQUIRE(tb->e[e].index >= 0, "%s: scale table entry %d: negative index", who, e);
+        CMS_REQUIRE(tb->e[e].first_sample >= (e ? tb->e[e - 1].first_sample : 0) && (e || tb->e[e].first_sample == 0),
+                    "%s: scale table entries start at sample 0 and ascend", who);
+    }
+    return CMS_OK;
+}
+
+extern "C" int cms_scale_by_table(const float* src, float* dst, int n, long long per_sample, const cms_scale_table* table,
+                                  void* stream) {
+    CMS_REQUIRE(src && dst && n >= 0 && per_sample > 0, "scale_by_table: bad argument");
+    const int rc = check_scale_table(table, "scale_by_table");
+    if (rc) return rc;
+    const long long total = (long long)n * per_sample;
+    if (total == 0) return CMS_OK;
+    const int grid = (int)std::min<long long>((total + 255) / 256, 1024);
+    hipLaunchKernelGGL(scale_by_table_kernel, dim3(grid), dim3(256), 0, (hipStream_t)stream, src, dst, (size_t)per_sample,
+                       (size_t)total, *table);
+    return launch_status("cms_scale_by_table");
+}
+
 extern "C" int cms_consistency_fwd(const cms_consistency_desc* d, void* workspace, double* stats_out, void* stream) {
     int rc = check_cons(d);
     if (rc) return rc;
@@ -569,6 +705,29 @@
     return launch_status("cms_ce_fwd_bwd");
 }
 
+extern "C" int cms_ce_fwd_bwd_final(const cms_ce_desc* d, float loss_weight, void* workspace, unsigned* ticket, double* stats_out,
+                                    float* scalars_out, float* grad_logits, void* stream) {
+    int rc = check_ce(d);
+    if (rc) return rc;
+    CMS_REQUIRE(workspace && ticket && stats_out && scalars_out && grad_logits,
+                "ce_fwd_bwd_final: workspace / ticket / stats_out / scalars_out / grad NULL");
+    const CeArgs a = make_ce_args(d);
+    const int tiles = fused_tiles(a.g, 1);
+    CMS_REQUIRE(tiles > 0, "ce_fwd_bwd_final: not available for this geometry / mode (ask cms_ce_fused_supported)");
+    CeFin fin;
+    fin.ticket = ticket;
+    fin.stats = stats_out;
+    fin.scalars = scalars_out;
+    fin.weight = loss_weight;
+    const size_t lds = std::max(tile_lds_bytes(d->c, a.g.sy, a.g.sx, 1), (size_t)2 * 256 * sizeof(double));
+    CMS_DISPATCH_C(d->c, {
+        allow_lds(ce_fused_final_kernel<CT>, lds);
+        hipLaunchKernelGGL(ce_fused_final_kernel<CT>, dim3(tiles), dim3(256), lds, (hipStream_t)stream, a, grad_logits,
+                           (float*)workspace, fin);
+    });
+    return launch_status("cms_ce_fwd_bwd_final");
+}
+
 extern "C" int cms_ce_fwd(const cms_ce_desc* d, void* workspace, double* stats_out, void* stream) {
     int rc = check_ce(d);
     if (rc) return rc;
diff --git a/cutmix-semisup-seg_amd/ops.py b/cutmix-semisup-seg_amd/ops.py
--- a/cutmix-semisup-seg_amd/ops.py
+++ b/cutmix-semisup-seg_amd/ops.py
@@ -175,7 +175,7 @@
 
 def _cons_scalars(stats, cfg, ramp_val, cons_weight, group, sync_conf_rate):
     stats_g = stats
-    if sync_conf_rate and cfg.conf_thresh > 0.0:
+    if sync_conf_rate and cfg.conf_thresh > 0.0 and _world(group) > 1:
         g = stats.clone()
         if _allreduce_sum(g, group):
             stats_g = g
@@ -211,14 +211,14 @@
 
 
 def consistency_fused(cfg, l_stu, l_tea0, l_tea1, out_size, grad_out, ranges=None, mask=None, um0=None, um1=None,
-                      ramp_val=1.0, cons_weight=1.0, group=None, sync_conf_rate=True):
+                      ramp_val=1.0, cons_weight=1.0, group=None, sync_conf_rate=True, defer_scale=False):
     d, keep = _cons_prepare('consistency_fused', cfg, l_stu, l_tea0, l_tea1, out_size, ranges, mask, um0, um1, grad_out)
     l_stu, l_tea0, l_tea1, ranges, mask, um0, um1 = keep[:7]
     if not fn['cms_consistency_fused_supported'](C.byref(d)):
         sc, cctx = consistency_forward(cfg, l_stu, l_tea0, l_tea1, out_size, ranges, mask, um0, um1, ramp_val, cons_weight, group,
                                        sync_conf_rate)
         consistency_backward(cctx, sc, grad_out)
-        return sc
+        return (sc, None) if defer_scale else sc
     dev = l_stu.device
     ws = _workspace('consistency', d, dev)
     stats = torch.empty(4, dtype=torch.float64, device=dev)
@@ -228,8 +228,68 @@
           'cms_consistency_fwd_bwd')
     scalars = _cons_scalars(stats, cfg, ramp_val, cons_weight, group, sync_conf_rate)
     if cfg.conf_thresh > 0.0 and not cfg.conf_per_pixel:
+        if defer_scale:
+            return scalars, (scalars, 1)
         check(fn['cms_scale_by_scalar'](_ptr(grad_out), grad_out.numel(), _ptr(scalars), 1, 1.0, _stream()), 'cms_scale_by_scalar')
-    return scalars
+    return (scalars, None) if defer_scale else scalars
+
+
+_TICKETS = {}
+
+
+def _ticket(kind, device):
+    key = (kind, str(device), torch.cuda.current_stream().cuda_stream)
+    t = _TICKETS.get(key)
+    if t is None:
+        t = _TICKETS[key] = torch.zeros(4, dtype=torch.int32, device=device)
+    return t
+
+
+def scale_table(entries):
+    if len(entries) > _lib.SCALE_ENTRIES:
+        raise ValueError('scale_table: at most {} ranges'.format(_lib.SCALE_ENTRIES))
+    tb = _lib.ScaleTable()
+    tb.n = len(entries)
+    for i, (first, scalars, index) in enumerate(entries):
+        if scalars is not None:
+            _need_cuda(scalars)
+            if scalars.dtype != torch.float32 or not 0 <= int(index) < scalars.numel():
+                raise ValueError('scale_table: fp32 scalars and an index inside them required')
+        tb.e[i].first_sample, tb.e[i].index = int(first), int(index)
+        tb.e[i].scalars = scalars.data_ptr() if scalars is not None else None
+    return tb
+
+
+def scale_by_table(src, table, out=None):
+    _need_cuda(src, out)
+    if src.dtype != torch.float32 or not src.is_contiguous():
+        raise TypeError('scale_by_table: contiguous fp32 tensor required')
+    if out is None:
+        out = torch.empty_like(src)
+    n = int(src.shape[0])
+    check(fn['cms_scale_by_table'](_ptr(src), _ptr(out), n, src.numel() // max(n, 1), C.byref(table), _stream()), 'cms_scale_by_table')
+    return out
+
+
+def consistency_fused_final(cfg, l_stu, l_tea0, l_tea1, out_size, grad_out, ranges=None, mask=None, um0=None, um1=None,
+                            ramp_val=1.0, cons_weight=1.0):
+    d, keep = _cons_prepare('consistency_fused_final', cfg, l_stu, l_tea0, l_tea1, out_size, ranges, mask, um0, um1, grad_out)
+    l_stu, l_tea0, l_tea1, ranges, mask, um0, um1 = keep[:7]
+    if not fn['cms_consistency_fused_supported'](C.byref(d)):
+        sc, cctx = consistency_forward(cfg, l_stu, l_tea0, l_tea1, out_size, ranges, mask, um0, um1, ramp_val, cons_weight, None, False)
+        consistency_backward(cctx, sc, grad_out)
+        return sc, None
+    dev = l_stu.device
+    ws = _workspace('consistency', d, dev)
+    stats = torch.empty(4, dtype=torch.float64, device=dev)
+    scalars = torch.empty(4, dtype=torch.float32, device=dev)
+    P = float(d.n) * float(d.H) * float(d.W)
+    grad_unit = float(ramp_val) * float(cons_weight) / P
+    check(fn['cms_consistency_fwd_bwd_final'](C.byref(d), grad_unit, float(ramp_val), float(cons_weight), _ptr(ws),
+                                              _ptr(_ticket('consistency', dev)), _ptr(stats), _ptr(scalars), _ptr(grad_out), _stream()),
+          'cms_consistency_fwd_bwd_final')
+    deferred = (scalars, 1) if (cfg.conf_thresh > 0.0 and not cfg.conf_per_pixel) else None
+    return scalars, deferred
 
 
 class _ConsistencyFn(torch.autograd.Function):
@@ -447,18 +507,35 @@
 
 
 def ce_fused(logits, labels, grad_out, out_size=None, ignore_index=255, align_corners=True, loss_weight=1.0, group=None,
-             sync_count=False):
+             sync_count=False, defer_scale=False):
     d, logits, labels = _ce_prepare(logits, labels, out_size, ignore_index, align_corners, grad_out)
     if not fn['cms_ce_fused_supported'](C.byref(d)):
         sc, cctx = ce_forward(logits, labels, out_size, ignore_index, align_corners, loss_weight, group, sync_count)
         ce_backward(cctx, sc, grad_out)
-        return sc
+        return (sc, None) if defer_scale else sc
     ws = _workspace('ce', d, logits.device)
     stats = torch.empty(2, dtype=torch.float64, device=logits.device)
     check(fn['cms_ce_fwd_bwd'](C.byref(d), _ptr(ws), _ptr(stats), _ptr(grad_out), _stream()), 'cms_ce_fwd_bwd')
     scalars, _ = _ce_scalars(stats, loss_weight, group, sync_count)
+    if defer_scale:
+        return scalars, (scalars, 1)
     check(fn['cms_scale_by_scalar'](_ptr(grad_out), grad_out.numel(), _ptr(scalars), 1, 1.0, _stream()), 'cms_scale_by_scalar')
     return scalars
+
+
+def ce_fused_final(logits, labels, grad_out, out_size=None, ignore_index=255, align_corners=True, loss_weight=1.0):
+    d, logits, labels = _ce_prepare(logits, labels, out_size, ignore_index, align_corners, grad_out)
+    if not fn['cms_ce_fused_supported'](C.byref(d)):
+        sc, cctx = ce_forward(logits, labels, out_size, ignore_index, align_corners, loss_weight)
+        ce_backward(cctx, sc, grad_out)
+        return sc, None
+    dev = logits.device
+    ws = _workspace('ce', d, dev)
+    stats = torch.empty(2, dtype=torch.float64, device=dev)
+    scalars = torch.empty(2, dtype=torch.float32, device=dev)
+    check(fn['cms_ce_fwd_bwd_final'](C.byref(d), float(loss_weight), _ptr(ws), _ptr(_ticket('ce', dev)), _ptr(stats), _ptr(scalars),
+                                     _ptr(grad_out), _stream()), 'cms_ce_fwd_bwd_final')
+    return scalars, (scalars, 1)
 
 
 def ce_backward(ctx, scalars, grad_out=None):
@@ -1908,6 +1985,23 @@
         return out
     check(fn['cms_aspp_spread_bwd'](_ptr(dlogits), _ptr(out), _dtype_code(out), dy, dx, nt, n, c, int(zc), h, w, _stream()),
           'cms_aspp_spread_bwd')
+    return out
+
+
+def aspp_spread_bwd_scaled(dlogits, table, taps, zc, dtype, out=None):
+    _need_cuda(dlogits, out)
+    if dlogits.dtype != torch.float32 or not dlogits.is_contiguous():
+        raise TypeError('aspp_spread_bwd_scaled: contiguous fp32 (N, C, h, w) gradient required')
+    if _REC is not None:
+        raise RuntimeError('aspp_spread_bwd_scaled: not a program op')
+    n, c, h, w = (int(v) for v in dlogits.shape)
+    if out is None:
+        out = torch.empty((n, h, w, int(zc)), dtype=dtype, device=dlogits.device)
+    elif tuple(out.shape) != (n, h, w, int(zc)) or not out.is_contiguous():
+        raise ValueError('aspp_spread_bwd_scaled: out must be a contiguous (N, h, w, zc) tensor')
+    dy, dx, nt = _tap_arrays(taps)
+    check(fn['cms_aspp_spread_bwd_scaled'](_ptr(dlogits), C.byref(table), _ptr(out), _dtype_code(out), dy, dx, nt, n, c, int(zc), h, w,
+                                           _stream()), 'cms_aspp_spread_bwd_scaled')
     return out
 
 
diff --git a/cutmix-semisup-seg_amd/step.py b/cutmix-semisup-seg_amd/step.py
--- a/cutmix-semisup-seg_amd/step.py
+++ b/cutmix-semisup-seg_amd/step.py
@@ -392,6 +392,10 @@
         if split:
             side.wait_stream(main)
         cons_vals = []
+        sex = self._student_executor()
+        final = (self.world <= 1 and sex is not None and getattr(sex, 'takes_dlogits_scale', False)
+                 and stu_lo.dtype == torch.float32 and len(unsup_batches) < ops._lib.SCALE_ENTRIES)
+        scale = []
 
         def consistency_branch():
             s_off, t_off = n_sup, 0
@@ -400,9 +404,15 @@
                 l0 = tea_lo[t_off:t_off + n]
                 l1 = tea_lo[t_off + n:t_off + 2 * n] if cfg.mix else None
                 t_off += 2 * n if cfg.mix else n
-                sc = ops.consistency_fused(cfg.cons, lo_det[s_off:s_off + n], l0, l1, out_size, grad_lo[s_off:s_off + n],
-                                           ranges=ub.ranges, mask=ub.mask, um0=ub.um0, um1=ub.um1, ramp_val=ramp,
-                                           cons_weight=cfg.cons_weight, group=self.group)
+                if final:
+                    sc, deferred = ops.consistency_fused(cfg.cons, lo_det[s_off:s_off + n], l0, l1, out_size,
+                                                         grad_lo[s_off:s_off + n], ranges=ub.ranges, mask=ub.mask, um0=ub.um0,
+                                                         um1=ub.um1, ramp_val=ramp, cons_weight=cfg.cons_weight, defer_scale=True)
+                    scale.append((s_off,) + (deferred or (None, 0)))
+                else:
+                    sc = ops.consistency_fused(cfg.cons, lo_det[s_off:s_off + n], l0, l1, out_size, grad_lo[s_off:s_off + n],
+                                               ranges=ub.ranges, mask=ub.mask, um0=ub.um0, um1=ub.um1, ramp_val=ramp,
+                                               cons_weight=cfg.cons_weight, group=self.group)
                 s_off += n
                 if split and isinstance(sc, torch.Tensor):
                     sc.record_stream(main)
@@ -410,8 +420,11 @@
         if split:
             with torch.cuda.stream(side):
                 consistency_branch()
-        ce_sc = ops.ce_fused(lo_det[:n_sup], sup_y, grad_lo[:n_sup], out_size, 255, self.align_corners, group=self.group)
-        sex = self._student_executor()
+        if final:
+            ce_sc, deferred = ops.ce_fused(lo_det[:n_sup], sup_y, grad_lo[:n_sup], out_size, 255, self.align_corners, defer_scale=True)
+            scale.insert(0, (0,) + (deferred or (None, 0)))
+        else:
+            ce_sc = ops.ce_fused(lo_det[:n_sup], sup_y, grad_lo[:n_sup], out_size, 255, self.align_corners, group=self.group)
         if split:
             if independent and groups is None and sex is not None and hasattr(sex, '_refresh_for_backward'):
                 sex._refresh_for_backward()
@@ -424,9 +437,13 @@
             dex.defer_wgrad_join = True
         if zev is not None:
             main.wait_event(zev)
+        if final:
+            sex.dlogits_scale = scale
         try:
             stu_lo.backward(grad_lo.to(stu_lo.dtype))
         finally:
+            if final:
+                sex.dlogits_scale = None
             if ex is not None:
                 ex.grad_hook = None
             if dex is not None:
diff --git a/include/cutmixseg.h b/include/cutmixseg.h
--- a/include/cutmixseg.h
+++ b/include/cutmixseg.h
@@ -77,6 +77,22 @@
                             float* grad_l_stu, void* stream);
 int cms_scale_by_scalar(float* x, long long n, const float* scalars, int index, float factor, void* stream);
 
+int cms_consistency_fwd_bwd_final(const cms_consistency_desc* d, float grad_unit, float ramp_val, float cons_weight,
+                                  void* workspace, unsigned* ticket, double* stats_out, float* scalars_out, float* grad_l_stu,
+                                  void* stream);
+
+#define CMS_SCALE_ENTRIES 4
+typedef struct {
+    int first_sample;
+    int index;
+    const float* scalars;
+} cms_scale_entry;
+typedef struct {
+    int n;
+    cms_scale_entry e[CMS_SCALE_ENTRIES];
+} cms_scale_table;
+int cms_scale_by_table(const float* src, float* dst, int n, long long per_sample, const cms_scale_table* table, void* stream);
+
 typedef struct cms_ce_desc {
     const float* logits;
     const void* labels;
@@ -91,6 +107,8 @@
 int cms_ce_bwd(const cms_ce_desc* d, const float* scalars, float* grad_logits, void* stream);
 int cms_ce_fused_supported(const cms_ce_desc* d);
 int cms_ce_fwd_bwd(const cms_ce_desc* d, void* workspace, double* stats_out, float* grad_logits, void* stream);
+int cms_ce_fwd_bwd_final(const cms_ce_desc* d, float loss_weight, void* workspace, unsigned* ticket, double* stats_out,
+                         float* scalars_out, float* grad_logits, void* stream);
 int cms_loss_set_deterministic(int on);
 
 
@@ -384,6 +402,8 @@
                         int n, int c, int zc, int h, int w, void* stream);
 int cms_aspp_spread_bwd(const float* dlogits, void* d_nhwc, int d_dtype, const int* tap_dy, const int* tap_dx, int n_taps,
                         int n, int c, int zc, int h, int w, void* stream);
+int cms_aspp_spread_bwd_scaled(const float* dlogits, const cms_scale_table* table, void* d_nhwc, int d_dtype, const int* tap_dy,
+                               const int* tap_dx, int n_taps, int n, int c, int zc, int h, int w, void* stream);
 
 int cms_stem_pack_weights(const void* w_khkwcoci, int w_dtype, float* w_packed, void* stream);
 int cms_stem_out_hw(int h, int w, int* ho, int* wo, int* hp, int* wp);
```

Result: no change. 640.9 images/sec (-0.1%).
